# zhiyuns/REHRSeg

Hardware: AMD Instinct MI355X
Metric: 3D patches/sec (fwd+bwd, 128^3 fp32) (higher is better)
Workload: dtype f32; 1 GPU; FLAVR UNet_3D_3D(1,'unet_18',128,4) fwd+bwd+Adam, 1x1x128^3 patch per GPU, random-init weights; patches_per_gpu=1, global_batch=1, parallelism=dp1 (patch-parallel, flat-bucket RCCL all-reduce), wgrad_stream=True

## Files before the change

include/rehrseg_hip.h:

```cpp
#ifndef REHRSEG_HIP_H
#define REHRSEG_HIP_H

#include <stdint.h>

#ifdef __cplusplus
extern "C" {
#endif

#define REHR_OK 0
#define REHR_EINVAL -1
#define REHR_ENOSUP -2
#define REHR_EHIP -3

#define REHR_ACT_NONE 0
#define REHR_ACT_RELU 1
#define REHR_ACT_LRELU 2

typedef struct {
  int32_t count, off0, offs, k0, ks;
} rehr_axis_taps;

typedef struct {
  const float* x1;
  const float* x2;
  int32_t c1, ldx1, ldx2;
  int32_t N, Di, Hi, Wi, Cin;
  int32_t Ld, Lh, Lw;
  int32_t sd, sh, sw, bd, bh, bw;
  rehr_axis_taps td, th, tw;
  int32_t KH, KW;
  const float* wp;
  int32_t Npad;
  float* y;
  int32_t Dy, Hy, Wy, Cout, ldy;
  int32_t osd, osh, osw, obd, obh, obw;
  const float* bias;
  int32_t act;
  float slope;
  double* stats;
  int32_t stats_mode;
  int32_t tile_d, tile_h, tile_w;
  float* wino_ws;
  int64_t wino_ws_bytes;
  int32_t flags;
  int32_t debug_flags;
} rehr_gather_gemm_desc;

#define REHR_GG_Y_F32 1
#define REHR_GG_WS_READY 2
#define REHR_GG_WS_ONLY 4

#define REHR_DBG_GG_NO_HALO 1
#define REHR_DBG_GG_NO_FLAT8 2
#define REHR_DBG_GG_FLAT8_HALF 4
#define REHR_DBG_GG_FLAT8_FULL 8
#define REHR_DBG_GG_W32P_TWO_PER_CU 16
#define REHR_DBG_GG_W32P_ONE_PER_CU 32
#define REHR_DBG_GG_INTERLEAVE 64
#define REHR_DBG_GG_NO_TCONV_KS 128
#define REHR_DBG_GG_SLICE_MAJOR 256

int64_t rehr_gather_gemm_wino_bytes(const rehr_gather_gemm_desc* d);
#define REHR_GG_ROUTE_NONE 0
#define REHR_GG_ROUTE_FLAT8 1
#define REHR_GG_ROUTE_W32P 2
#define REHR_GG_ROUTE_BIG8 3
#define REHR_GG_ROUTE_SMALL 4
#define REHR_GG_ROUTE_FLAT22 5
#define REHR_GG_ROUTE_REGION22 6
int rehr_gather_gemm_wino_route(const rehr_gather_gemm_desc* d);
int rehr_gather_gemm_f32(const rehr_gather_gemm_desc* d, void* stream);
int rehr_gather_gemm_multi_f32(const rehr_gather_gemm_desc* descs, int32_t count,
                               void* stream);
int rehr_gather_gemm_bf16(const rehr_gather_gemm_desc* d, void* stream);
int rehr_gather_gemm_multi_bf16(const rehr_gather_gemm_desc* descs, int32_t count, void* stream);
int rehr_pack_weights_bf16(const float* in, void* out, int32_t A, int32_t Apad, int32_t B, int32_t T,
                           int32_t transpose_ab, void* stream);

int rehr_sum_slabs_bias_act_f32(const float* slabs, int32_t S, int64_t slab_stride,
                                const float* bias, float* y, int64_t rows, int32_t C,
                                int32_t act, float slope, void* stream);

int rehr_sum_slabs_stats_f32(const float* slabs, int32_t S, int64_t slab_stride, const float* bias,
                             float* y, int32_t N, int64_t SV, int32_t C, int32_t act, float slope,
                             double* stats, void* stream);

int rehr_sum_slabs_bias_act_bf16(const float* slabs, int32_t S, int64_t slab_stride, const float* bias, void* y,
                                 int64_t rows, int32_t C, int32_t act, float slope, void* stream);
int rehr_sum_slabs_stats_bf16(const float* slabs, int32_t S, int64_t slab_stride, const float* bias, void* y,
                              int32_t N, int64_t SV, int32_t C, int32_t act, float slope, double* stats,
                              void* stream);

typedef struct {
  const float* l;
  int32_t ldl, Ca;
  const float* g;
  int32_t ldg, Cg;
  int32_t N, Ld, Lh, Lw;
  int32_t Dg, Hg, Wg;
  int32_t sd, sh, sw, bd, bh, bw;
  rehr_axis_taps td, th, tw;
  int32_t KH, KW;
  float* dst;
  int64_t dst_sa, dst_sc, dst_st;
  int32_t accumulate;
  float* workspace;
  int64_t workspace_bytes;
  float* dbias;
  int32_t flags;
  int32_t debug_flags;
} rehr_wgrad_desc;

#define REHR_DBG_WGRAD_DIRECT 1
#define REHR_DBG_WGRAD_NO_TAP_SKIP 2
#define REHR_DBG_WGRAD_NO_TAP_COLOCATE 4

int64_t rehr_wgrad_bf16_workspace_bytes(const rehr_wgrad_desc* d);
int rehr_wgrad_bf16(const rehr_wgrad_desc* d, void* stream);
int64_t rehr_wgrad_workspace_bytes(const rehr_wgrad_desc* d);
int rehr_wgrad_uses_winograd(const rehr_wgrad_desc* d);
int rehr_wgrad_f32(const rehr_wgrad_desc* d, void* stream);

int rehr_pack_weights_f32(const float* in, float* out, int32_t A, int32_t Apad,
                          int32_t B, int32_t T, int32_t transpose_ab,
                          void* stream);

typedef struct {
  const float* x;
  int32_t ldx, N, Di, Hi, Wi, Cin;
  const float* w;
  const float* bias;
  float* y;
  int32_t ldy, Do, Ho, Wo, Cout;
  int32_t KD, KH, KW, sd, sh, sw, pd, ph, pw;
  int32_t act;
  float slope;
  double* stats;
  int32_t stats_mode;
} rehr_direct_conv_desc;

int rehr_conv_small_cin_fwd_f32(const rehr_direct_conv_desc* d, void* stream);
int rehr_im2col_f32(const rehr_direct_conv_desc* d, float* out, int32_t Kpad,
                    void* stream);
int64_t rehr_conv_small_cin_wgrad_workspace_bytes(const rehr_direct_conv_desc* d);
int rehr_conv_small_cin_wgrad_on_mfma(const rehr_direct_conv_desc* d);
int rehr_conv_small_cin_fwd_on_mfma(const rehr_direct_conv_desc* d);
int rehr_conv_small_cin_fwd_ybf16(const rehr_direct_conv_desc* d, void* stream);
int rehr_conv_small_cin_wgrad_dybf16(const rehr_direct_conv_desc* d, float* dw, float* dbias, float* workspace,
                                     int64_t workspace_bytes, void* stream);
int rehr_conv_small_cin_wgrad_f32(const rehr_direct_conv_desc* d, float* dw,
                                  float* dbias, float* workspace,
                                  int64_t workspace_bytes, void* stream);

int rehr_conv_small_cout_fwd_f32(const rehr_direct_conv_desc* d, void* stream);
int rehr_conv_small_cout_dgrad_f32(const rehr_direct_conv_desc* d, float* dx,
                                   void* stream);
int64_t rehr_conv_small_cout_wgrad_workspace_bytes(const rehr_direct_conv_desc* d);
int rehr_conv_small_cout_wgrad_f32(const rehr_direct_conv_desc* d, float* dw,
                                   float* dbias, float* workspace,
                                   int64_t workspace_bytes, void* stream);

int rehr_se_gate_fwd_f32(const double* stats, const float* w, const float* b,
                         float* gate, float* mean, int32_t N, int32_t C,
                         int64_t S, void* stream);
int rehr_scale_res_act_fwd_f32(const float* x, int32_t ldx, const float* gate,
                               const float* res, int32_t ldr, float* y,
                               int32_t ldy, int32_t N, int64_t S, int32_t C,
                               int32_t act, float slope, void* stream);
int rehr_scale_res_act_bwd_f32(const float* dy, int32_t lddy, const float* y,
                               int32_t ldy, const float* x, int32_t ldx,
                               const float* gate, float* dx, int32_t lddx,
                               float* dres, int32_t lddr, double* dgate_acc,
                               int32_t N, int64_t S, int32_t C, int32_t act,
                               float slope, void* stream);
int rehr_se_gate_bwd_f32(const double* dgate_acc, const float* gate,
                         const float* mean, const float* w, float* dw,
                         float* db, float* kconst, int32_t N, int32_t C,
                         int64_t S, void* stream);
int rehr_add_channel_const_f32(float* x, int32_t ldx, const float* k, int32_t N,
                               int64_t S, int32_t C, void* stream);

int rehr_instnorm_act_fwd_f32(const float* x, int32_t ldx, const double* stats,
                              const float* gamma, const float* beta, float* y,
                              int32_t ldy, float* mean_rstd ,
                              int32_t N, int64_t S, int32_t C, float eps,
                              int32_t act, float slope, void* stream);
int rehr_instnorm_act_bwd_f32(const float* dy, int32_t lddy, const float* x,
                              int32_t ldx, const float* mean_rstd,
                              const float* gamma, const float* beta, float* dx,
                              int32_t lddx, float* dgamma, float* dbeta,
                              double* red, int32_t N, int64_t S, int32_t C,
                              int32_t act, float slope, void* stream);

int rehr_upsample_depth_fwd_f32(const float* x, float* y, int32_t N, int32_t Di,
                                int32_t Do, int64_t HW, int32_t C, void* stream);
int rehr_upsample_depth_bwd_f32(const float* dy, float* dx, int32_t N,
                                int32_t Di, int32_t Do, int64_t HW, int32_t C,
                                void* stream);

int rehr_upmix_depth_fwd_f32(const float* g, const float* bias, float* y, int32_t N,
                             int32_t Di, int32_t Do, int64_t HW, int32_t C, int32_t KD,
                             int32_t pd, int32_t act, float slope, void* stream);
int rehr_upmix_depth_bwd_f32(const float* dy, const float* y, float* dg, int32_t N,
                             int32_t Di, int32_t Do, int64_t HW, int32_t C, int32_t KD,
                             int32_t pd, int32_t act, float slope, void* stream);
int rehr_channel_sum_actgrad_f32(const float* dy, const float* y, int32_t ld, int64_t rows,
                                 int32_t C, int32_t act, float slope, float* out,
                                 double* scratch, void* stream);

int rehr_cosdist_stats_f32(const float* x1, const float* x2, double* stats, int32_t N,
                           int64_t S, int32_t C, void* stream);
int rehr_cosdist_bwd_f32(const float* x1, const float* x2, const double* stats, float* dx1,
                         int32_t N, int64_t S, int32_t C, float scale, void* stream);

int32_t rehr_uasr_mix_blocks(int32_t N, int32_t D, int64_t HW);
int rehr_uasr_mix_fwd_f32(const float* om, const float* ue, const float* wu, const float* bu, float* out,
                          float* unc, int32_t N, int32_t K, int32_t D, int64_t HW, void* stream);
int rehr_uasr_mix_bwd_f32(const float* om, const float* ue, const float* wu, const float* bu,
                          const float* gout, const float* gunc, float* dom, float* due, double* partial,
                          int32_t N, int32_t K, int32_t D, int64_t HW, void* stream);

int rehr_quad_maxpool_fwd_f32(const float* x, float* y, int32_t* idx, int64_t slices,
                              int32_t H, int32_t W, int32_t C, void* stream);
int rehr_quad_maxpool_bwd_f32(const float* dy, const int32_t* idx, float* dx, int64_t slices,
// ... 166 lines not shown
```

rehrseg_amd/csrc/gather_gemm.hip:

```cpp
#include "common.h"
#include "halo_conv.h"
#include "wino_shared.h"

namespace {

constexpr int BK = 32;
constexpr int LDS_LD = 36;
constexpr int NTHREADS = 256;

template <int BM, int BN, int WGM, int WGN, int LDSBUF>
__device__ __forceinline__ void gather_gemm_body(const GGParams& p, const int nblocks, const int logical_in = -1) {
  constexpr int WTM = BM / WGM, WTN = BN / WGN;
  constexpr int FM = WTM / 32, FN = WTN / 32;
  constexpr int AROWS = BM / 32, BROWS = BN / 32;
  static_assert(WGM * WGN == 4, "4 waves");
  const rehr_gather_gemm_desc& d = p.d;

  extern __shared__ __attribute__((aligned(16))) float smem[];
  float* As = smem;
  float* Bs = smem + LDSBUF * BM * LDS_LD;
  int* row_out = (int*)(Bs + LDSBUF * BN * LDS_LD);

  const int tid = threadIdx.x;
  const int lane = tid & 63, wave = tid >> 6;
// ... 152 lines not shown
  };
  auto commit_loads = [&](int buf, const f32x4 (&ra)[AROWS], const f32x4 (&rb)[BROWS]) {
    float* a = As + buf * BM * LDS_LD;
    float* b = Bs + buf * BN * LDS_LD;
#pragma unroll
    for (int i = 0; i < AROWS; ++i)
      *reinterpret_cast<f32x4*>(a + (r0 + 32 * i) * LDS_LD + q * 4) = ra[i];
#pragma unroll
    for (int i = 0; i < BROWS; ++i)
      *reinterpret_cast<f32x4*>(b + (r0 + 32 * i) * LDS_LD + q * 4) = rb[i];
  };

  const int arow = wm * WTM + (lane & 31);
  const int brow = wn * WTN + (lane & 31);
  const int koff = 4 * (lane >> 5);
  auto compute = [&](int buf) {
    const float* a = As + buf * BM * LDS_LD;
    const float* b = Bs + buf * BN * LDS_LD;
#pragma unroll
    for (int kk = 0; kk < BK / 8; ++kk) {
      f32x4 fa[FM], fb[FN];
#pragma unroll
      for (int i = 0; i < FM; ++i)
        fa[i] = *reinterpret_cast<const f32x4*>(a + (arow + 32 * i) * LDS_LD + kk * 8 + koff);
#pragma unroll
      for (int j = 0; j < FN; ++j)
        fb[j] = *reinterpret_cast<const f32x4*>(b + (brow + 32 * j) * LDS_LD + kk * 8 + koff);
#pragma unroll
      for (int e = 0; e < 4; ++e)
#pragma unroll
        for (int i = 0; i < FM; ++i)
#pragma unroll
          for (int j = 0; j < FN; ++j)
            acc[i][j] = __builtin_amdgcn_mfma_f32_32x32x2f32(fa[i][e], fb[j][e], acc[i][j], 0, 0, 0);
      if (kk == 0) __builtin_amdgcn_sched_barrier(0);
    }
  };

  if (nsteps > 0) {
    issue_loads(ra0, rb0);
    issue_loads(ra1, rb1);
    commit_loads(0, ra0, rb0);
  }
  __syncthreads();

  if (LDSBUF == 2) {
    for (int s = 0; s < nsteps; s += 2) {
      issue_loads(ra0, rb0);
      compute(0);
      commit_loads(1, ra1, rb1);
      __syncthreads();
      if (s + 1 >= nsteps) break;
      issue_loads(ra1, rb1);
      compute(1);
      commit_loads(0, ra0, rb0);
      __syncthreads();
    }
  } else {
    for (int s = 0; s < nsteps; s += 2) {
      issue_loads(ra0, rb0);
      compute(0);
      __syncthreads();
      commit_loads(0, ra1, rb1);
      __syncthreads();
      if (s + 1 >= nsteps) break;
      issue_loads(ra1, rb1);
      compute(0);
      __syncthreads();
      commit_loads(0, ra0, rb0);
      __syncthreads();
    }
  }

  const int chalf = lane >> 5;
#pragma unroll
  for (int j = 0; j < FN; ++j) {
    const int col = n0 + wn * WTN + j * 32 + (lane & 31);
    const bool colok = col < d.Cout;
    const float bv = (d.bias != nullptr && colok) ? d.bias[col] : 0.f;
    float s1 = 0.f, s2 = 0.f;
#pragma unroll
    for (int i = 0; i < FM; ++i) {
#pragma unroll
      for (int r = 0; r < 16; ++r) {
        const int row = wm * WTM + i * 32 + (r & 3) + 8 * (r >> 2) + 4 * chalf;
        const int off = row_out[row];
        float v = apply_act(acc[i][j][r] + bv, d.act, d.slope);
        if (off >= 0 && colok) {
          d.y[(int64_t)off * d.ldy + col] = v;
          s1 += v;
          s2 += v * v;
        }
      }
    }
    if (d.stats_mode != 0) {
      s1 += __shfl_xor(s1, 32, 64);
      s2 += __shfl_xor(s2, 32, 64);
      if (chalf == 0 && colok) {
        double* st = d.stats + ((int64_t)n_img * d.Cout + col) * 2;
        atomicAdd(st, (double)s1);
        if (d.stats_mode == 2) atomicAdd(st + 1, (double)s2);
      }
    }
  }
}

template <int BM, int BN, int WGM, int WGN, int LDSBUF>
__global__ __launch_bounds__(NTHREADS, (LDSBUF == 1 ? 3 : 2)) void gather_gemm_multi_kernel(const GGMulti pm) {
  int phase, logical;
  if (pm.interleave) {
    if (!interleaved_block((int)blockIdx.x, pm.ph[0].m_tiles, pm.ph[0].n_tiles, pm.count, phase, logical)) return;
  } else {
    phase = blockIdx.z;
    const int nb = pm.ph[phase].m_tiles * pm.ph[phase].n_tiles;
    if ((int)blockIdx.x >= nb) return;
    logical = xcd_remap(blockIdx.x, nb);
  }
  phase = __builtin_amdgcn_readfirstlane(phase);
  logical = __builtin_amdgcn_readfirstlane(logical);
  gather_gemm_body<BM, BN, WGM, WGN, LDSBUF>(pm.ph[phase], 0, logical);
}
template <int BM, int BN, int WGM, int WGN, int LDSBUF>
__global__ __launch_bounds__(NTHREADS, (LDSBUF == 1 ? 3 : 2)) void gather_gemm_kernel(const GGParams p) {
  gather_gemm_body<BM, BN, WGM, WGN, LDSBUF>(p, (int)gridDim.x);
}

template <int BM, int BN, int WGM, int WGN, int LDSBUF>
int launch_gg(const GGMulti& pm, int count, hipStream_t stream) {
  constexpr size_t smem = (size_t)LDSBUF * (BM + BN) * LDS_LD * sizeof(float) + BM * sizeof(int);
  return gg_launch<gather_gemm_kernel<BM, BN, WGM, WGN, LDSBUF>, gather_gemm_multi_kernel<BM, BN, WGM, WGN, LDSBUF>,
                   NTHREADS, smem>(pm, count, stream);
}

int validate(const rehr_gather_gemm_desc& d) { return gg_validate(d, 4); }

int launch_generic(const GGMulti& pm, int count, hipStream_t st) {
  const int npad = pm.ph[0].d.Npad;
  if (npad % 128 == 0) return launch_gg<128, 128, 2, 2, 2>(pm, count, st);
  if (npad % 64 == 0) return launch_gg<128, 64, 2, 2, 1>(pm, count, st);
  return launch_gg<128, 32, 4, 1, 1>(pm, count, st);
}

}

WinoRoute wino_route(const rehr_gather_gemm_desc& d, WinoPlan& plan) {
  if (!(d.debug_flags & REHR_DBG_GG_NO_FLAT8) && wino_flat8_plan(d, plan)) return WINO_FLAT8;
  if (const WinoRoute r = wino_region_plan(d, plan)) return r;
  if (wino22_flat_plan(d, plan, 1)) return WINO_FLAT22;
  if (wino22_region_plan(d, plan)) return WINO_REGION22;
  plan.bytes = 0;
  return WINO_NONE;
}

static int wino_run(WinoRoute r, const rehr_gather_gemm_desc* ds, int count, const WinoPlan& plan, hipStream_t st) {
  for (int i = 0; i < count; ++i) {
    const int rc = r >= WINO_FLAT22 ? wino22_weights_launch(ds[i], plan, st) : wino_weights_launch(r, ds[i], plan, st);
    if (rc != REHR_OK) return rc;
  }
  if (ds[0].flags & REHR_GG_WS_ONLY) return REHR_OK;
  switch (r) {
    case WINO_FLAT8: return wino_flat8_launch(ds[0], plan, st);
    case WINO_W32P: case WINO_BIG8: case WINO_SMALL: return wino_region_launch(r, ds, count, plan, st);
    default: return wino22_launch(r, ds, count, plan, st);
  }
}

extern "C" int rehr_gather_gemm_multi_f32(const rehr_gather_gemm_desc* descs, int32_t count, void* stream) {
  if (descs == nullptr || count < 1 || count > MAX_PHASES) return REHR_EINVAL;
  for (int i = 0; i < count; ++i) {
    const int rc = validate(descs[i]);
    if (rc != REHR_OK) return rc;
    if (descs[i].Npad != descs[0].Npad || descs[i].N != descs[0].N || descs[i].wp != descs[0].wp ||
        descs[i].x1 != descs[0].x1)
      return REHR_EINVAL;
  }
  hipStream_t st = (hipStream_t)stream;
  const bool ws_only = (descs[0].flags & REHR_GG_WS_ONLY) != 0;
  for (int i = 1; i < count; ++i)
    if ((descs[i].flags ^ descs[0].flags) & (REHR_GG_WS_ONLY | REHR_GG_WS_READY)) return REHR_EINVAL;
  if (count > 1 && !ws_only) {
    const int trc = tconv_ks_try(descs, count, false, st);
    if (trc != REHR_ENOSUP) return trc;
  }
  WinoPlan plan{};
  if (count > 1 && descs[0].wino_ws != nullptr) {
    const int taps = descs[0].td.count;
    if ((taps > 3 || taps == 1) && wino_split_plan(descs, count, plan)) return wino_run(WINO_BIG8, descs, count, plan, st);
    if (taps <= 3 && wino22_flat_multi_plan(descs, count, plan)) return wino_run(WINO_FLAT22, descs, count, plan, st);
  }
  GGMulti pm;
  pm.interleave = 0;
  pm.count = 0;
  pm.no_interleave = (descs[0].debug_flags & REHR_DBG_GG_INTERLEAVE) ? 0 : 1;
  int n = 0;
  for (int i = 0; i < count; ++i) {
    if (descs[i].wino_ws != nullptr && !(count > 1 && descs[i].td.count > 3)) {
      const WinoRoute r = wino_route(descs[i], plan);
      if (r != WINO_NONE && wino_ws_ok(descs[i], plan.bytes)) {
        const int wrc = wino_run(r, &descs[i], 1, plan, st);
        if (wrc != REHR_OK) return wrc;
        continue;
      }
    }
    if (ws_only) continue;
    if (descs[i].tile_d >= 0) {
      const int hrc = halo_conv_try(descs[i], st);
      if (hrc == REHR_OK) continue;
      if (hrc != REHR_ENOSUP) return hrc;
    }
    const int rc = gg_plan(descs[i], pm.ph[n], 4, BK);
    if (rc != REHR_OK) return rc;
    ++n;
  }
  if (n == 0) return REHR_OK;
  return launch_generic(pm, n, st);
}

extern "C" int64_t rehr_gather_gemm_wino_bytes(const rehr_gather_gemm_desc* dp) {
  WinoPlan plan{};
  if (dp == nullptr || validate(*dp) != REHR_OK || wino_route(*dp, plan) == WINO_NONE) return 0;
  return plan.bytes;
}

extern "C" int rehr_gather_gemm_wino_route(const rehr_gather_gemm_desc* dp) {
  WinoPlan plan{};
  if (dp == nullptr || validate(*dp) != REHR_OK) return REHR_GG_ROUTE_NONE;
  const WinoRoute r = wino_route(*dp, plan);
  return r == WINO_NONE ? REHR_GG_ROUTE_NONE : (int)r | (plan.variant << 8);
}

extern "C" int rehr_gather_gemm_f32(const rehr_gather_gemm_desc* dp, void* stream) {
  if (dp == nullptr) return REHR_EINVAL;
  return rehr_gather_gemm_multi_f32(dp, 1, stream);
}
```

rehrseg_amd/csrc/gg_shared.h:

```cpp
#pragma once
#include "common.h"
#include "taps.h"

struct GGParams {
  rehr_gather_gemm_desc d;
  int tiles_d, tiles_h, tiles_w, m_tiles, n_tiles;
  int kchunks;
  int64_t wp_bytes;
};

constexpr int MAX_PHASES = 8;
struct GGMulti {
  GGParams ph[MAX_PHASES];
  int interleave, count, no_interleave;
};

__device__ __forceinline__ bool interleaved_block(int b, int m_tiles, int n_tiles, int count, int& phase, int& logical) {
  const int xcd = b & 7, j = b >> 3, per = count * n_tiles;
  const int mt = (j / per) * 8 + xcd, rem = j % per;
  phase = rem / n_tiles;
  logical = mt * n_tiles + (rem - phase * n_tiles);
  return mt < m_tiles;
}

constexpr int64_t GG_BUF_LIMIT = BUF_LIMIT;

inline int64_t gg_wp_bytes(const rehr_gather_gemm_desc& d, int es) {
  const int64_t kd_max = d.td.k0 + (int64_t)d.td.ks * (d.td.count - 1);
  const int64_t kh_max = d.th.k0 + (int64_t)d.th.ks * (d.th.count - 1);
  const int64_t kw_max = d.tw.k0 + (int64_t)d.tw.ks * (d.tw.count - 1);
  return (((kd_max * d.KH) + kh_max) * d.KW + kw_max + 1) * d.Npad * d.Cin * es;
}

inline bool gg_src_fits(const rehr_gather_gemm_desc& d, int64_t vox, int es) {
  const int64_t b = vox * es;
  return b * d.ldx1 < GG_BUF_LIMIT && (!d.x2 || b * d.ldx2 < GG_BUF_LIMIT);
}

inline int gg_validate(const rehr_gather_gemm_desc& d, int es) {
  const int row = 16 / es;
  if (!d.x1 || !d.wp || !d.y) return REHR_EINVAL;
  if (d.N < 1 || d.Cin < 16 || d.Cin % 16 || d.c1 < 1 || d.c1 > d.Cin) return REHR_EINVAL;
  if (d.c1 < d.Cin && (d.c1 % 32 || !d.x2)) return REHR_EINVAL;
  if (d.ldx1 % row || (d.x2 && d.ldx2 % row)) return REHR_EINVAL;
  if (((uintptr_t)d.x1 | (uintptr_t)d.wp | (uintptr_t)(d.x2 ? d.x2 : d.x1)) & 15) return REHR_EINVAL;
  if (d.Npad % 32 || d.Npad < d.Cout || d.Cout < 1) return REHR_EINVAL;
  if (d.Ld < 1 || d.Lh < 1 || d.Lw < 1) return REHR_EINVAL;
  if (d.td.count < 1 || d.th.count < 1 || d.tw.count < 1) return REHR_EINVAL;
  if (d.tile_d != 0 && (d.tile_d < 1 || d.tile_h < 1 || d.tile_w < 1 || d.tile_d * d.tile_h * d.tile_w != 128))
    return REHR_EINVAL;
  if (d.stats_mode != 0 && !d.stats) return REHR_EINVAL;
  if (d.N > 65535) return REHR_EINVAL;
  const int64_t yd = (int64_t)(d.Ld - 1) * d.osd + d.obd, yh = (int64_t)(d.Lh - 1) * d.osh + d.obh,
                yw = (int64_t)(d.Lw - 1) * d.osw + d.obw;
  if (d.obd < 0 || d.obh < 0 || d.obw < 0 || yd >= d.Dy || yh >= d.Hy || yw >= d.Wy) return REHR_EINVAL;
  if (d.ldy < d.Cout) return REHR_EINVAL;
  if ((int64_t)d.N * d.Dy * d.Hy * d.Wy >= (1ll << 31)) return REHR_EINVAL;
  return REHR_OK;
}

inline int gg_plan(const rehr_gather_gemm_desc& d, GGParams& p, int es, int bk) {
  p.d = d;
  if (d.tile_d == 0) {
    p.tiles_d = p.tiles_h = 1;
    p.tiles_w = (int)(((int64_t)d.Ld * d.Lh * d.Lw + 127) / 128);
    p.m_tiles = p.tiles_w;
  } else {
    p.tiles_d = (d.Ld + d.tile_d - 1) / d.tile_d;
    p.tiles_h = (d.Lh + d.tile_h - 1) / d.tile_h;
    p.tiles_w = (d.Lw + d.tile_w - 1) / d.tile_w;
    p.m_tiles = p.tiles_d * p.tiles_h * p.tiles_w;
  }
  p.kchunks = (d.Cin + bk - 1) / bk;
  p.wp_bytes = gg_wp_bytes(d, es);
  if (p.wp_bytes >= GG_BUF_LIMIT || !gg_src_fits(d, (int64_t)d.Di * d.Hi * d.Wi, es)) return REHR_ENOSUP;
  p.n_tiles = d.Npad / (d.Npad % 128 == 0 ? 128 : (d.Npad % 64 == 0 ? 64 : 32));
  return REHR_OK;
}

template <void (*KERN1)(GGParams), void (*KERNM)(GGMulti), int NT, size_t SMEM>
int gg_launch(const GGMulti& pm, int count, hipStream_t stream) {
  static bool attr_set = false;
  if (!attr_set) {
    if (hipFuncSetAttribute(reinterpret_cast<const void*>(KERN1), hipFuncAttributeMaxDynamicSharedMemorySize,
                            (int)SMEM) != hipSuccess ||
        hipFuncSetAttribute(reinterpret_cast<const void*>(KERNM), hipFuncAttributeMaxDynamicSharedMemorySize,
                            (int)SMEM) != hipSuccess)
      return REHR_EHIP;
    attr_set = true;
  }
  if (count == 1) {
    const GGParams& p = pm.ph[0];
    hipLaunchKernelGGL(KERN1, dim3(p.m_tiles * p.n_tiles, p.d.N, 1), dim3(NT), SMEM, stream, p);
  } else {
    int nb = 0;
    bool uniform = true;
    for (int i = 0; i < count; ++i) {
      const int n = pm.ph[i].m_tiles * pm.ph[i].n_tiles;
      nb = n > nb ? n : nb;
      uniform = uniform && pm.ph[i].m_tiles == pm.ph[0].m_tiles && pm.ph[i].n_tiles == pm.ph[0].n_tiles;
    }
    GGMulti pmi = pm;
    pmi.count = count;
    const int64_t gx = (int64_t)((pm.ph[0].m_tiles + 7) / 8) * 8 * count * pm.ph[0].n_tiles;
    pmi.interleave = (uniform && !pm.no_interleave && gx < (1ll << 31)) ? 1 : 0;
    if (pmi.interleave) hipLaunchKernelGGL(KERNM, dim3((unsigned)gx, pm.ph[0].d.N, 1), dim3(NT), SMEM, stream, pmi);
    else hipLaunchKernelGGL(KERNM, dim3(nb, pm.ph[0].d.N, count), dim3(NT), SMEM, stream, pmi);
  }
  REHR_LAUNCH_CHECK();
  return REHR_OK;
}

int tconv_ks_try(const rehr_gather_gemm_desc* ds, int count, bool bf16, hipStream_t stream);
```

rehrseg_amd/csrc/tconv_ks.hip:

```cpp
#include "common.h"

namespace {

constexpr int TK_BM = 128, TK_BK = 32, TK_LD = 36, TK_THREADS = 256, TK_MAXPH = 8;

struct TconvKsParams {
  const void* x;
  const void* wp;
  const float* bias;
  void* y;
  int ldx, ldy, Cin, Cout, Npad;
  int N, Di, Hi, Wi, Do, Ho, Wo;
  int sd, sh, sw;
  int nph;
  int tap[TK_MAXPH];
  int yoff[TK_MAXPH];
  int64_t vox_total;
  int lda;
};

template <int NT>
__global__ __launch_bounds__(TK_THREADS, 2) void tconv_ks_f32_kernel(const TconvKsParams p) {
  extern __shared__ __attribute__((aligned(16))) float smem[];
  float* As = smem;
// ... 132 lines not shown
      const int row = r0 + 64 * i;
      const int64_t v = v0 + row;
      tk_bf16x8 a;
#pragma unroll
      for (int e = 0; e < 8; ++e) a[e] = (__bf16)0.f;
      if (v < p.vox_total) a = *reinterpret_cast<const tk_bf16x8*>(x + v * p.ldx + c * TK_BK + q * 8);
      *reinterpret_cast<tk_bf16x8*>(As + row * p.lda + c * TK_BK + q * 8) = a;
    }

  constexpr int NBR = (NT * 32 + 63) / 64;
  tk_bf16x8 rb[NBR];
  auto fetch_b = [&](int ph, int c) {
    const __bf16* w = wp + ((int64_t)p.tap[ph] * p.Npad) * p.Cin + c * TK_BK + q * 8;
#pragma unroll
    for (int j = 0; j < NBR; ++j) {
      const int row = r0 + 64 * j;
      if (row < NT * 32) rb[j] = *reinterpret_cast<const tk_bf16x8*>(w + (int64_t)row * p.Cin);
    }
  };
  auto commit_b = [&](int buf) {
    __bf16* b = Bs + buf * NT * 32 * TK_LDH;
#pragma unroll
    for (int j = 0; j < NBR; ++j) {
      const int row = r0 + 64 * j;
      if (row < NT * 32) *reinterpret_cast<tk_bf16x8*>(b + row * TK_LDH + q * 8) = rb[j];
    }
  };

  const int arow = wave * 32 + (lane & 31), koff = 8 * (lane >> 5), chalf = lane >> 5;
  const int steps = p.nph * kchunks;
  fetch_b(0, 0);
  commit_b(0);
  __syncthreads();

  f32x16 acc[NT];
  int ph = 0, c = 0;
  for (int s = 0; s < steps; ++s) {
    if (c == 0) {
#pragma unroll
      for (int j = 0; j < NT; ++j)
#pragma unroll
        for (int r = 0; r < 16; ++r) acc[j][r] = 0.f;
    }
    int nph_ = ph, nc = c + 1;
    if (nc == kchunks) { nc = 0; ++nph_; }
    const bool more = s + 1 < steps;
    if (more) fetch_b(nph_, nc);
    const __bf16* a = As + arow * p.lda + c * TK_BK + koff;
    const __bf16* b = Bs + (s & 1) * NT * 32 * TK_LDH + (lane & 31) * TK_LDH + koff;
#pragma unroll
    for (int kk = 0; kk < TK_BK / 16; ++kk) {
      const tk_bf16x8 fa = *reinterpret_cast<const tk_bf16x8*>(a + kk * 16);
#pragma unroll
      for (int j = 0; j < NT; ++j) {
        const tk_bf16x8 fb = *reinterpret_cast<const tk_bf16x8*>(b + j * 32 * TK_LDH + kk * 16);
        acc[j] = __builtin_amdgcn_mfma_f32_32x32x16_bf16(fa, fb, acc[j], 0, 0, 0);
      }
    }
    if (more) commit_b((s + 1) & 1);
    if (c == kchunks - 1) {
      const int yo = p.yoff[ph];
#pragma unroll
      for (int j = 0; j < NT; ++j) {
        const int col = j * 32 + (lane & 31);
        const bool colok = col < p.Cout;
        const float bv = (p.bias != nullptr && colok) ? p.bias[col] : 0.f;
#pragma unroll
        for (int r = 0; r < 16; ++r) {
          const int row = wave * 32 + (r & 3) + 8 * (r >> 2) + 4 * chalf;
          const int off = row_out[row];
          if (off >= 0 && colok) y[(int64_t)(off + yo) * p.ldy + col] = (__bf16)(acc[j][r] + bv);
        }
      }
    }
    __syncthreads();
    ph = nph_;
    c = nc;
  }
}


bool tconv_ks_match(const rehr_gather_gemm_desc* ds, int count, bool bf16, TconvKsParams& p) {
  if (count < 2 || count > TK_MAXPH) return false;
  const rehr_gather_gemm_desc& d0 = ds[0];
  if (d0.x2 != nullptr || d0.c1 != d0.Cin || d0.Cin % TK_BK || d0.Cin > 128 || d0.Npad % 32 || d0.Npad > 128) return false;
  if (d0.act != REHR_ACT_NONE || d0.stats_mode != 0 || (d0.flags & REHR_GG_Y_F32)) return false;
  if (d0.osd * d0.osh * d0.osw != count) return false;
  if (d0.Dy != d0.Di * d0.osd || d0.Hy != d0.Hi * d0.osh || d0.Wy != d0.Wi * d0.osw) return false;
  if ((int64_t)d0.N * d0.Dy * d0.Hy * d0.Wy >= (1ll << 31)) return false;
  if (d0.KH != d0.osh || d0.KW != d0.osw) return false;
  unsigned seen = 0;
  for (int i = 0; i < count; ++i) {
    const rehr_gather_gemm_desc& d = ds[i];
    if (d.x1 != d0.x1 || d.wp != d0.wp || d.y != d0.y || d.bias != d0.bias || d.x2 != nullptr || d.Cin != d0.Cin ||
        d.ldx1 != d0.ldx1 || d.ldy != d0.ldy || d.Cout != d0.Cout || d.Npad != d0.Npad || d.N != d0.N)
      return false;
    if (d.td.count != 1 || d.th.count != 1 || d.tw.count != 1 || d.td.off0 || d.th.off0 || d.tw.off0) return false;
    if (d.sd != 1 || d.sh != 1 || d.sw != 1 || d.bd || d.bh || d.bw) return false;
    if (d.Ld != d0.Di || d.Lh != d0.Hi || d.Lw != d0.Wi || d.Di != d0.Di || d.Hi != d0.Hi || d.Wi != d0.Wi) return false;
    if (d.osd != d0.osd || d.osh != d0.osh || d.osw != d0.osw || d.Dy != d0.Dy || d.Hy != d0.Hy || d.Wy != d0.Wy) return false;
    if (d.obd != d.td.k0 || d.obh != d.th.k0 || d.obw != d.tw.k0) return false;
    if (d.obd < 0 || d.obd >= d.osd || d.obh < 0 || d.obh >= d.osh || d.obw < 0 || d.obw >= d.osw) return false;
    if (d.act != REHR_ACT_NONE || d.stats_mode != 0 || d.flags != d0.flags) return false;
    const int id = (d.obd * d.osh + d.obh) * d.osw + d.obw;
    if (seen & (1u << id)) return false;
    seen |= 1u << id;
    p.tap[i] = (d.td.k0 * d.KH + d.th.k0) * d.KW + d.tw.k0;
    p.yoff[i] = (d.obd * d.Hy + d.obh) * d.Wy + d.obw;
  }
  const int align = bf16 ? 15 : 15;
  if (((uintptr_t)d0.x1 | (uintptr_t)d0.wp) & align) return false;
  if (bf16 ? (d0.ldx1 % 8 || d0.ldy % 2) : (d0.ldx1 % 4)) return false;
  p.x = d0.x1; p.wp = d0.wp; p.bias = d0.bias; p.y = d0.y;
  p.ldx = d0.ldx1; p.ldy = d0.ldy; p.Cin = d0.Cin; p.Cout = d0.Cout; p.Npad = d0.Npad;
  p.N = d0.N; p.Di = d0.Di; p.Hi = d0.Hi; p.Wi = d0.Wi; p.Do = d0.Dy; p.Ho = d0.Hy; p.Wo = d0.Wy;
  p.sd = d0.osd; p.sh = d0.osh; p.sw = d0.osw;
  p.nph = count;
  p.vox_total = (int64_t)d0.N * d0.Di * d0.Hi * d0.Wi;
  p.lda = bf16 ? d0.Cin + 8 : d0.Cin + 4;
  return true;
}

template <int NT>
int tconv_launch(const TconvKsParams& p, bool bf16, hipStream_t stream) {
  const int64_t blocks = (p.vox_total + TK_BM - 1) / TK_BM;
  if (blocks >= (1ll << 31)) return REHR_ENOSUP;
  if (!bf16 && p.Cin > 64) return REHR_ENOSUP;
  if (bf16) {
    const size_t smem = ((size_t)TK_BM * p.lda + 2 * NT * 32 * TK_LDH) * 2 + TK_BM * sizeof(int);
    static bool attr = false;
    if (!attr) {
      if (hipFuncSetAttribute((const void*)tconv_ks_bf16_kernel<NT>, hipFuncAttributeMaxDynamicSharedMemorySize, 72 * 1024) !=
          hipSuccess)
        return REHR_EHIP;
      attr = true;
    }
    hipLaunchKernelGGL(tconv_ks_bf16_kernel<NT>, dim3((unsigned)blocks), dim3(TK_THREADS), smem, stream, p);
  } else {
    const size_t smem = ((size_t)TK_BM * p.lda + 2 * NT * 32 * TK_LD) * sizeof(float) + TK_BM * sizeof(int);
    static bool attr = false;
    if (!attr) {
      if (hipFuncSetAttribute((const void*)tconv_ks_f32_kernel<NT>, hipFuncAttributeMaxDynamicSharedMemorySize, 112 * 1024) !=
          hipSuccess)
        return REHR_EHIP;
      attr = true;
    }
    hipLaunchKernelGGL(tconv_ks_f32_kernel<NT>, dim3((unsigned)blocks), dim3(TK_THREADS), smem, stream, p);
  }
  return REHR_OK;
}

}

int tconv_ks_try(const rehr_gather_gemm_desc* ds, int count, bool bf16, hipStream_t stream) {
  if (ds[0].debug_flags & REHR_DBG_GG_NO_TCONV_KS) return REHR_ENOSUP;
  TconvKsParams p;
  if (!tconv_ks_match(ds, count, bf16, p)) return REHR_ENOSUP;
  int rc;
  switch (p.Npad / 32) {
    case 1: rc = tconv_launch<1>(p, bf16, stream); break;
    case 2: rc = tconv_launch<2>(p, bf16, stream); break;
    case 3: rc = tconv_launch<3>(p, bf16, stream); break;
    default: rc = tconv_launch<4>(p, bf16, stream); break;
  }
  if (rc != REHR_OK) return rc;
  REHR_LAUNCH_CHECK();
  return REHR_OK;
}
```

rehrseg_amd/csrc/wino22_conv.hip:

```cpp
#include "common.h"
#include "wino_shared.h"
#include <cstdlib>

namespace {

constexpr int LD = WINO_LDX;
constexpr int PW = 17;
constexpr int RP = PW * LD + 12;
constexpr int BUF = PW * RP;
constexpr int PVOX = PW * PW;
constexpr int NT_ = 768;
constexpr int NX = (PVOX * 8 + NT_ - 1) / NT_;
constexpr int MAXPH = WINO_MAXPH;

struct W22Params {
  rehr_gather_gemm_desc d;
  int nb_h, nb_w, kchunks, nphase;
  Phase phase[MAXPH];
  const float* up;
  uint32_t up_bytes;
};

__global__ void w22_weights_kernel(const rehr_gather_gemm_desc d, float* __restrict__ up, int kchunks) {
  AxisPlan ah, aw;
  plan_axis(d.th, d.sh, d.bh, ah);
  plan_axis(d.tw, d.sw, d.bw, aw);
  const int nphase = ah.nph * aw.nph;
  const int cpad = kchunks * 32;
  const int64_t per = (int64_t)d.Npad * cpad;
  const int64_t per_src = (int64_t)d.Npad * d.Cin;
  const int64_t total = (int64_t)nphase * d.td.count * per;
  const int NT = d.Npad / 32;
  for (int64_t i = (int64_t)blockIdx.x * blockDim.x + threadIdx.x; i < total; i += (int64_t)gridDim.x * blockDim.x) {
    const int pj = (int)(i / per);
    const int p = pj / d.td.count, jd = pj - p * d.td.count;
    const int p_h = p / aw.nph, p_w = p - p_h * aw.nph;
    const int64_t rem = i - (int64_t)pj * per;
    const int n = (int)(rem / cpad), ci = (int)(rem - (int64_t)n * cpad);
    float g[2][2];
#pragma unroll
    for (int a = 0; a < 2; ++a)
#pragma unroll
      for (int b = 0; b < 2; ++b) {
        const int wt = ((d.td.k0 + d.td.ks * jd) * d.KH + ah.kidx[p_h][a]) * d.KW + aw.kidx[p_w][b];
        g[a][b] = ci < d.Cin ? d.wp[(int64_t)wt * per_src + (int64_t)n * d.Cin + ci] : 0.f;
      }
    float u[9];
    u[0] = g[0][0];              u[1] = g[0][0] + g[0][1];                     u[2] = g[0][1];
    u[3] = g[0][0] + g[1][0];    u[4] = g[0][0] + g[0][1] + g[1][0] + g[1][1]; u[5] = g[0][1] + g[1][1];
    u[6] = g[1][0];              u[7] = g[1][0] + g[1][1];                     u[8] = g[1][1];
    const int nt = n >> 5, col = n & 31, chunk = ci >> 5, kk = (ci >> 3) & 3, half = (ci >> 2) & 1, e = ci & 3;
#pragma unroll
    for (int x = 0; x < 9; ++x) {
      const int64_t o = (((((int64_t)pj * 9 + x) * NT + nt) * kchunks + chunk) * 4 + kk) * 256 + (half * 32 + col) * 4 + e;
      up[o] = u[x];
    }
  }
}

__global__ __launch_bounds__(NT_) void wino22_conv_kernel(const W22Params p) {
  const rehr_gather_gemm_desc& d = p.d;
  extern __shared__ __attribute__((aligned(16))) float smem[];
  float* Xs = smem;

  const int tid = threadIdx.x, lane = tid & 63;
  const int wv = __builtin_amdgcn_readfirstlane(tid >> 6);
  const int r = wv % 3, fm = (wv / 3) & 1, fn = wv / 6;
  const int half = lane >> 5, col = lane & 31;
  const int n_img = blockIdx.z;
  const int nt0 = blockIdx.y * 2 + fn, n0 = blockIdx.y * 64;
  int b = xcd_remap(blockIdx.x, gridDim.x);
  const int bw_ = b % p.nb_w; b /= p.nb_w;
  const int bh_ = b % p.nb_h;
  const int od = b / p.nb_h;
  const int oh0 = bh_ * 16, ow0 = bw_ * 16;

  const int ia = r;
  const int th_ = fm * 4 + (col >> 3), tw_ = col & 7;
  const float* xa = Xs + (2 * th_ + ia) * RP + tw_ * LD + 4 * half;
  const float* xb = Xs + (2 * th_ + 1) * RP + tw_ * LD + 4 * half;

  int prow[NX], pcol[NX];
#pragma unroll
  for (int i = 0; i < NX; ++i) {
    const int piece = tid + NT_ * i;
    const int v = piece >> 3;
    const int ph = (v * 3856) >> 16;
    const int slot = v - ph * PW;
    prow[i] = ph;
    pcol[i] = slot < 9 ? 2 * slot : 2 * (slot - 9) + 1;
  }
  const int pq = tid & 7;
  const uint32_t img_elems = (uint32_t)d.Di * d.Hi * d.Wi;
  int jd_lo = d.td.count, jd_hi = -1;
  for (int j = 0; j < d.td.count; ++j) {
    const int id = od + d.bd + d.td.off0 + d.td.offs * j;
    if ((unsigned)id < (unsigned)d.Di) { jd_lo = min(jd_lo, j); jd_hi = max(jd_hi, j); }
  }
  const int items = p.nphase * p.kchunks * max(0, jd_hi - jd_lo + 1);
  f32x4 rx[NX];
  struct Item { int ph, chunk, jd; };
  auto advance = [&](Item& t) {
    if (++t.jd > jd_hi) {
      t.jd = jd_lo;
      if (++t.chunk == p.kchunks) { t.chunk = 0; ++t.ph; }
    }
  };
  auto fetch = [&](const Item& t) {
    const bool live = t.ph < p.nphase;
    const int ph_i = live ? t.ph : 0;
    const int jd = t.jd;
    const int cc = t.chunk * 32;
    const Phase& P = p.phase[ph_i];
    const int id = od + d.bd + d.td.off0 + d.td.offs * jd;
    const bool first = cc < d.c1;
    const float* src = first ? d.x1 : d.x2;
    const uint32_t ld = (uint32_t)(first ? d.ldx1 : d.ldx2);
    const int coff = first ? cc : cc - d.c1;
    const uint32_t nrec = img_elems * ld * 4u;
    const __amdgpu_buffer_rsrc_t rs = __builtin_amdgcn_make_buffer_rsrc(
        const_cast<float*>(src) + (int64_t)n_img * img_elems * ld, 0, nrec, 0x00020000);
    const bool dok = live & ((unsigned)id < (unsigned)d.Di) & ((cc + pq * 4) < d.Cin);
    const uint32_t base = (uint32_t)(id * d.Hi * d.Wi) * ld * 4u + (uint32_t)(coff + pq * 4) * 4u;
#pragma unroll
    for (int i = 0; i < NX; ++i) {
      const int piece = tid + NT_ * i;
      const int ih = (oh0 + P.dh0 + prow[i]) * P.sh + P.ph, iw = (ow0 + P.dw0 + pcol[i]) * P.sw + P.pw;
      const bool ok = dok & (piece < PVOX * 8) & ((unsigned)ih < (unsigned)d.Hi) & ((unsigned)iw < (unsigned)d.Wi);
      const uint32_t off = base + (uint32_t)(ih * d.Wi + iw) * ld * 4u;
      rx[i] = __builtin_bit_cast(f32x4, __builtin_amdgcn_raw_buffer_load_b128(rs, ok ? off : nrec, 0, 0));
    }
  };
  auto stage = [&](int buf) {
#pragma unroll
    for (int i = 0; i < NX; ++i) {
      const int piece = tid + NT_ * i;
      const int v = piece >> 3;
      if (piece < PVOX * 8) *reinterpret_cast<f32x4*>(Xs + buf + v * LD + prow[i] * 12 + pq * 4) = rx[i];
    }
  };

  const __amdgpu_buffer_rsrc_t rsu =
      __builtin_amdgcn_make_buffer_rsrc(const_cast<float*>(p.up), 0, p.up_bytes, 0x00020000);
  const int NT = d.Npad / 32;
  const uint32_t xi_stride = (uint32_t)NT * p.kchunks * 4096u, nt_stride = (uint32_t)p.kchunks * 4096u;
  const uint32_t ulane = (uint32_t)(r * 3) * xi_stride + (uint32_t)nt0 * nt_stride + (uint32_t)lane * 16u;
  auto load_u = [&](const Item& t, int kk, f32x4 (&ub)[3]) {
    const int ph_i = t.ph < p.nphase ? t.ph : 0;
#ifdef W22_DBG_SAMEW
    const uint32_t base = ulane + 0u * (uint32_t)(ph_i + kk);
#else
    const uint32_t base = (uint32_t)((ph_i * d.td.count + t.jd) * 9) * xi_stride + (uint32_t)(t.chunk * 4 + kk) * 1024u + ulane;
#endif
#pragma unroll
    for (int c = 0; c < 3; ++c)
      ub[c] = __builtin_bit_cast(f32x4, __builtin_amdgcn_raw_buffer_load_b128(rsu, base + c * xi_stride, 0, 0));
  };

  f32x16 acc[3];
#pragma unroll
  for (int c = 0; c < 3; ++c)
#pragma unroll
    for (int q = 0; q < 16; ++q) acc[c][q] = 0.f;

  auto read_a = [&](int buf, const int kk, f32x4 (&v)[3]) {
    f32x4 R[3];
#ifdef W22_DBG_NOLDS
    R[0] = R[1] = R[2] = f32x4{1.f, 2.f, 3.f, 4.f};
#else
#pragma unroll
    for (int j = 0; j < 3; ++j) R[j] = *reinterpret_cast<const f32x4*>(xa + buf + ((j & 1) * 9 + (j >> 1)) * LD + kk * 8);
    if (r != 1) {
#pragma unroll
      for (int j = 0; j < 3; ++j) R[j] -= *reinterpret_cast<const f32x4*>(xb + buf + ((j & 1) * 9 + (j >> 1)) * LD + kk * 8);
    }
#endif
    v[0] = R[0] - R[1];
    v[1] = R[1];
    v[2] = R[2] - R[1];
  };
  auto mma = [&](const f32x4 (&v)[3], const f32x4 (&ub)[3]) {
#pragma unroll
    for (int e = 0; e < 4; ++e)
#pragma unroll
      for (int c = 0; c < 3; ++c) acc[c] = __builtin_amdgcn_mfma_f32_32x32x2f32(v[c][e], ub[c][e], acc[c], 0, 0, 0);
  };

#ifdef W22_STAMPS
  const long long st0 = __builtin_readcyclecounter();
#endif
  f32x4 u0[3], u1[3], va[3], vb[3];
  Item cur_i = {0, 0, min(jd_lo, d.td.count - 1)}, nxt_i = cur_i, fet_i;
  fetch(cur_i);
  load_u(cur_i, 0, u0);
  stage(0);
  advance(nxt_i);
  fetch(nxt_i);
  fet_i = nxt_i;
  __syncthreads();
  read_a(0, 0, va);
#ifdef W22_STAMPS
  const long long st1 = __builtin_readcyclecounter();
  long long st_stage = 0, st_bar = 0;
#endif
  for (int it = 0; it < items; ++it) {
    const int cur = (it & 1) * BUF, nxt = cur ^ BUF;
    load_u(cur_i, 1, u1);
    read_a(cur, 1, vb);
    __builtin_amdgcn_s_setprio(2);
// ... 284 lines not shown
  Item cur_i = {0, 0, min(jd_lo, d.td.count - 1)}, nxt_i = cur_i;
  fetch(cur_i);
  load_u(cur_i, 0, u0);
  stage(0);
  __syncthreads();
  for (int it = 0; it < items; ++it) {
    const int cur = (it & 1) * FBUF, nxt = cur ^ FBUF;
    advance(nxt_i);
    fetch(nxt_i);
    load_u(cur_i, 1, u1);
    kstep(cur, 0, u0);
    load_u(cur_i, 2, u0);
    kstep(cur, 1, u1);
    load_u(cur_i, 3, u1);
    kstep(cur, 2, u0);
    load_u(nxt_i, 0, u0);
    kstep(cur, 3, u1);
    stage(nxt);
    cur_i = nxt_i;
    __syncthreads();
  }

  float* ex = smem;
  {
    const f32x16 T0v = acc[0] + acc[1];
    const f32x16 T1v = acc[1] + acc[2];
    float* e0 = ex + (((fm * 2 + fn) * 3 + r) * 2) * 16 * 64 + lane;
#pragma unroll
    for (int q = 0; q < 16; ++q) {
      e0[q * 64] = T0v[q];
      e0[(16 + q) * 64] = T1v[q];
    }
  }
  __syncthreads();
  const float neg_slope = d.act == REHR_ACT_NONE ? 1.f : (d.act == REHR_ACT_RELU ? 0.f : d.slope);
  const int col_n = n0 + fn * 32 + col;
  const bool colok = col_n < d.Cout;
  const float bv = (d.bias != nullptr && colok) ? d.bias[col_n] : 0.f;
  float ssum[F22_MAXSLOT][2];
#pragma unroll
  for (int s = 0; s < F22_MAXSLOT; ++s) ssum[s][0] = ssum[s][1] = 0.f;
  for (int pos = r; pos < 4; pos += 3) {
    const int ro = pos >> 1, co = pos & 1;
    const float k0 = ro == 0 ? 1.f : 0.f, k2 = ro == 0 ? 0.f : 1.f;
    const float* e0 = ex + ((fm * 2 + fn) * 3 * 2 + co) * 16 * 64 + lane;
    float t[3][16];
#pragma unroll
    for (int rr = 0; rr < 3; ++rr)
#pragma unroll
      for (int q = 0; q < 16; ++q) t[rr][q] = e0[(rr * 32 + q) * 64];
#pragma unroll
    for (int q = 0; q < 16; ++q) {
      const float yv = k0 * t[0][q] + t[1][q] + k2 * t[2][q] + bv;
      const float v = fmaxf(yv, 0.f) + neg_slope * fminf(yv, 0.f);
      const int m = fm * 32 + 8 * (q >> 2) + 4 * half + (q & 3);
      const int tv = tab[m], hwp = tab[2 * TB + m], sl = tab[TB + m];
      const int oh = 2 * (hwp >> 16) + ro, ow = 2 * (hwp & 0xffff) + co;
      const bool ok = colok & (tv >= 0) & (oh < d.Lh) & (ow < d.Lw);
      if (ok) d.y[((int64_t)tv + (int64_t)ro * d.osh * d.Wy + co * d.osw) * d.ldy + col_n] = v;
      if (d.stats_mode != 0) {
        const float vs = ok ? v : 0.f;
#pragma unroll
        for (int s = 0; s < F22_MAXSLOT; ++s) {
          ssum[s][0] += (s == sl) ? vs : 0.f;
          ssum[s][1] += (s == sl) ? vs * vs : 0.f;
        }
      }
    }
  }
  if (d.stats_mode != 0) {
    __syncthreads();
    float* red = smem;
    const int nslot = min(sl_ - s0 + 1, F22_MAXSLOT);
#pragma unroll
    for (int s = 0; s < F22_MAXSLOT; ++s)
      if (s < nslot) {
        float* rp = red + (((s * 12 + wv) * 2 + half) * 2) * 32 + col;
        rp[0] = ssum[s][0];
        rp[32] = ssum[s][1];
      }
    __syncthreads();
    for (int task = tid; task < nslot * 64; task += NT_) {
      const int s = task >> 6, fq = (task >> 5) & 1, c = task & 31;
      const int cn = n0 + fq * 32 + c;
      const int slice = s0 + s, od = slice / d.N, n = slice - od * d.N;
      if (cn < d.Cout && od < d.Ld) {
        float a1 = 0.f, a2 = 0.f;
        for (int w6 = 0; w6 < 6; ++w6)
          for (int h = 0; h < 2; ++h) {
            const float* rp = red + (((s * 12 + fq * 6 + w6) * 2 + h) * 2) * 32 + c;
            a1 += rp[0];
            a2 += rp[32];
          }
        double* st = d.stats + ((int64_t)n * d.Cout + cn) * 2;
        atomicAdd(st, (double)a1);
        if (d.stats_mode == 2) atomicAdd(st + 1, (double)a2);
      }
    }
  }
}

constexpr FlatConsts F22_CONSTS = {1, 64, F22_NX * NT_, 256, (int64_t)4 * 3 * 2 * 16 * 64,
                                   (int64_t)F22_MAXSLOT * 12 * 2 * 2 * 32, 160 * 1024};

bool plan22_taps(const rehr_gather_gemm_desc& d, WinoPlan& plan) {
  if (d.sd != 1) return false;
  AxisPlan ah, aw;
  if (!plan_axis(d.th, d.sh, d.bh, ah) || !plan_axis(d.tw, d.sw, d.bw, aw)) return false;
  if (ah.nph != aw.nph) return false;
  if (ah.nph == 2 && (d.osh != 1 || d.osw != 1 || d.obh || d.obw)) return false;
  if (d.td.count < 1 || d.td.count > 3 || d.Npad % 64) return false;
  plan.variant = 0;
  plan.kchunks = (d.Cin + 31) / 32;
  plan.nphase = fill_phases(ah, aw, plan.phase);
  plan.bytes = wino_scratch_bytes(d, 9 * plan.nphase);
  return plan.bytes != 0;
}

}

bool wino22_flat_plan(const rehr_gather_gemm_desc& d, WinoPlan& plan, int parts) {
  if (d.debug_flags & REHR_DBG_GG_NO_FLAT8) return false;
  if (!plan22_taps(d, plan) || d.Lh > 2048 || d.Ld > 127) return false;
  return plan_flat_geom(d, F22_CONSTS, parts, plan.flat);
}

bool wino22_region_plan(const rehr_gather_gemm_desc& d, WinoPlan& plan) {
  if (!plan22_taps(d, plan) || d.Lh < 12 || d.Lw < 12) return false;
  plan.nb_h = (d.Lh + 15) / 16;
  plan.nb_w = (d.Lw + 15) / 16;
  const int64_t padded = (int64_t)plan.nb_h * 16 * plan.nb_w * 16, exact = (int64_t)d.Lh * d.Lw;
  if (padded * 10 > exact * 13) {
    if (padded * 100 > exact * 178 || (int64_t)plan.nb_h * plan.nb_w * d.Ld * d.N * (d.Npad / 64) < 256) return false;
  }
  if (!gg_src_fits(d, (int64_t)d.Di * d.Hi * d.Wi, 4)) return false;
  return (int64_t)plan.nb_h * plan.nb_w * d.Ld < (1ll << 31) && d.Npad / 64 <= 65535 && d.N <= 65535;
}

bool wino22_flat_multi_plan(const rehr_gather_gemm_desc* ds, int count, WinoPlan& plan) {
  if (count < 2 || count > WINO_MAXPH) return false;
  if (!wino22_flat_plan(ds[0], plan, count) || plan.nphase != 1) return false;
  for (int i = 0; i < count; ++i) {
    WinoPlan q;
    if (!wino22_flat_plan(ds[i], q, count) || q.nphase != 1 || q.bytes != plan.bytes || !wino_ws_ok(ds[i], q.bytes))
      return false;
    if (!gg_same_layer(ds[i], ds[0], SAME_DEPTH_TAPS | SAME_DEST) || q.phase[0].sh != plan.phase[0].sh ||
        q.phase[0].sw != plan.phase[0].sw)
      return false;
    plan.phase[i] = q.phase[0];
  }
  return true;
}

int wino22_weights_launch(const rehr_gather_gemm_desc& d, const WinoPlan& plan, hipStream_t stream) {
  const int64_t total = (int64_t)plan.nphase * d.td.count * d.Npad * plan.kchunks * 32;
  return wino_transform_launch<w22_weights_kernel>(d, total, 8192, stream, plan.kchunks);
}

int wino22_launch(WinoRoute r, const rehr_gather_gemm_desc* ds, int count, const WinoPlan& plan, hipStream_t stream) {
  const rehr_gather_gemm_desc& d = ds[0];
  if (r == WINO_FLAT22) {
    F22Params p;
    p.d = d;
    flat_fill(p, plan.flat);
    p.kchunks = plan.kchunks;
    p.nphase = plan.nphase;
    for (int i = 0; i < WINO_MAXPH; ++i) p.phase[i] = plan.phase[i];
    p.up_bytes = (uint32_t)plan.bytes;
    p.parts = count;
    p.up = count == 1 ? d.wino_ws : nullptr;
    for (int i = 0; i < count; ++i) {
      p.s_up[i] = ds[i].wino_ws;
      p.s_obh[i] = ds[i].obh;
      p.s_obw[i] = ds[i].obw;
    }
    const size_t smem = flat_lds_bytes(plan.flat, 64);
    const int rc = grow_dyn_lds<wino22_flat_conv_kernel>(smem);
    if (rc != REHR_OK) return rc;
    dim3 grid((unsigned)((p.ntiles + 63) / 64), d.Npad / 64, count);
    hipLaunchKernelGGL(wino22_flat_conv_kernel, grid, dim3(NT_), smem, stream, p);
  } else {
    W22Params p;
    p.d = d;
    p.nb_h = plan.nb_h;
    p.nb_w = plan.nb_w;
    p.kchunks = plan.kchunks;
    p.nphase = plan.nphase;
    for (int i = 0; i < WINO_MAXPH; ++i) p.phase[i] = plan.phase[i];
    p.up = d.wino_ws;
    p.up_bytes = (uint32_t)plan.bytes;
    constexpr size_t smem_x = (size_t)2 * BUF * sizeof(float), smem_e = (size_t)4 * 3 * 2 * 16 * 64 * sizeof(float);
    constexpr size_t smem = smem_x > smem_e ? smem_x : smem_e;
    const int rc = set_dyn_lds_once<wino22_conv_kernel>((int)smem);
    if (rc != REHR_OK) return rc;
    dim3 grid((unsigned)((int64_t)p.nb_h * p.nb_w * d.Ld), d.Npad / 64, d.N);
    hipLaunchKernelGGL(wino22_conv_kernel, grid, dim3(NT_), smem, stream, p);
  }
  REHR_LAUNCH_CHECK();
  return REHR_OK;
}
```

rehrseg_amd/csrc/wino_conv.hip:

```cpp
#include "common.h"
#include "wino_shared.h"
#include <cstdlib>

namespace {

constexpr int TH = 4, TW = 8;
constexpr int PH = 2 * TH + 2, PW = 2 * TW + 2;
constexpr int PVOX = PH * PW;
constexpr int LDX = 36;
constexpr int NX = (PVOX * 8 + 255) / 256;

struct WinoParams {
  rehr_gather_gemm_desc d;
  int nb_h, nb_w;
  int band_major;
  int kchunks;
  int dh0, dw0;
  const float* up;
  uint32_t up_bytes;
  int nsplit;
  rehr_axis_taps s_td[8];
  const float* s_up[8];
  uint32_t s_up_bytes[8];
  float* s_y[8];
// ... 119 lines not shown
    }
  };
  auto load_u = [&](int it, int kk, f32x4 (&ub)[4]) {
    const int jd = it % d.td.count;
    const int cc = (it / d.td.count) * 32;
    const uint32_t base = (uint32_t)(jd * 16 + r * 4) * per_b + (uint32_t)(cc + kk * 8) * 4u + ulane;
#pragma unroll
    for (int c = 0; c < 4; ++c)
      ub[c] = __builtin_bit_cast(f32x4, __builtin_amdgcn_raw_buffer_load_b128(rsu, base + c * per_b, 0, 0));
  };
  auto compute = [&](const f32x4 (&R)[4], const f32x4 (&ub)[4]) {
    f32x4 v[4];
    v[0] = R[0] - R[2];
    v[1] = R[1] + R[2];
    v[2] = R[1] - R[2];
    v[3] = R[1] - R[3];
#pragma unroll
    for (int e = 0; e < 4; ++e)
#pragma unroll
      for (int c = 0; c < 4; ++c)
        acc[c] = __builtin_amdgcn_mfma_f32_32x32x2f32(v[c][e], ub[c][e], acc[c], 0, 0, 0);
  };

  fetch(0);
  stage(0);
  fetch(1);
  f32x4 Ra[4], Rb[4], ua[4], ubb[4];
  load_u(0, 0, ua);
  __syncthreads();

  for (int it = 0; it < items; ++it) {
    const int cur = (it & 1) * (PVOX * LDX);
    read_r(cur, 0, Ra);
    read_r(cur, 1, Rb);
    load_u(it, 1, ubb);
    stage(cur ^ (PVOX * LDX));
    __builtin_amdgcn_sched_barrier(0);
    compute(Ra, ua);
    __builtin_amdgcn_sched_barrier(0);
    read_r(cur, 2, Ra);
    load_u(it, 2, ua);
    fetch(it + 2);
    __builtin_amdgcn_sched_barrier(0);
    compute(Rb, ubb);
    __builtin_amdgcn_sched_barrier(0);
    read_r(cur, 3, Rb);
    load_u(it, 3, ubb);
    __builtin_amdgcn_sched_barrier(0);
    compute(Ra, ua);
    __builtin_amdgcn_sched_barrier(0);
    load_u(it + 1 < items ? it + 1 : it, 0, ua);
    __builtin_amdgcn_sched_barrier(0);
    compute(Rb, ubb);
    __builtin_amdgcn_sched_barrier(0);
    __syncthreads();
  }

  f32x16 T0 = (acc[0] + acc[1] - acc[2]) * rsign;
  f32x16 T1 = (acc[1] + acc[2] - acc[3]) * rsign;
  float* ex = smem;
#pragma unroll
  for (int q = 0; q < 16; ++q) {
    ex[((r * 2 + 0) * 16 + q) * 64 + lane] = T0[q];
    ex[((r * 2 + 1) * 16 + q) * 64 + lane] = T1[q];
  }
  __syncthreads();
  const int ro = r >> 1, co = r & 1;
  const float k0 = ro == 0 ? 1.f : 0.f, k2 = ro == 0 ? 1.f : -1.f, k3 = ro == 0 ? 0.f : -1.f;
  const float neg_slope = d.act == REHR_ACT_NONE ? 1.f : (d.act == REHR_ACT_RELU ? 0.f : d.slope);
  const int col_n = n0 + col;
  const bool colok = col_n < d.Cout;
  const float bv = (d.bias != nullptr && colok) ? d.bias[col_n] : 0.f;
  float s1_ = 0.f, s2_ = 0.f;
  float t[4][16];
#pragma unroll
  for (int rr = 0; rr < 4; ++rr)
#pragma unroll
    for (int q = 0; q < 16; ++q) t[rr][q] = ex[((rr * 2 + co) * 16 + q) * 64 + lane];
#pragma unroll
  for (int q = 0; q < 16; ++q) {
    const float yv = k0 * t[0][q] + t[1][q] + k2 * t[2][q] + k3 * t[3][q] + bv;
    const float v = fmaxf(yv, 0.f) + neg_slope * fminf(yv, 0.f);
    const int tile = (q & 3) + 8 * (q >> 2) + 4 * half;
    const int oh = oh0 + 2 * (tile / TW) + ro, ow = ow0 + 2 * (tile % TW) + co;
    const bool ok = colok & (oh < d.Lh) & (ow < d.Lw);
    if (ok) d.y[((((int64_t)n_img * d.Dy + od) * d.Hy + oh) * d.Wy + ow) * d.ldy + col_n] = v;
    s1_ += ok ? v : 0.f;
    s2_ += ok ? v * v : 0.f;
  }
  if (d.stats_mode != 0) {
    s1_ += __shfl_xor(s1_, 32, 64);
    s2_ += __shfl_xor(s2_, 32, 64);
    __syncthreads();
    float* red = smem;
    if (half == 0) {
      red[(r * 2 + 0) * 32 + col] = s1_;
      red[(r * 2 + 1) * 32 + col] = s2_;
    }
    __syncthreads();
    if (r == 0 && half == 0 && colok) {
      const float a1 = red[col] + red[64 + col] + red[128 + col] + red[192 + col];
      const float a2 = red[32 + col] + red[96 + col] + red[160 + col] + red[224 + col];
      double* st = d.stats + ((int64_t)n_img * d.Cout + col_n) * 2;
      atomicAdd(st, (double)a1);
      if (d.stats_mode == 2) atomicAdd(st + 1, (double)a2);
    }
  }
}

constexpr int PW2 = 18, PVOX2 = 18 * 18;
constexpr int RP2 = PW2 * LDX + 8;
constexpr int BUF2 = PW2 * RP2;

__global__ void wino_weights_frag_kernel(const rehr_gather_gemm_desc d, float* __restrict__ up, int kchunks) {
  const float G[4][3] = {{1.f, 0.f, 0.f}, {.5f, .5f, .5f}, {.5f, -.5f, .5f}, {0.f, 0.f, 1.f}};
  const int cpad = kchunks * 32;
  const int64_t per = (int64_t)d.Npad * cpad;
  const int64_t per_src = (int64_t)d.Npad * d.Cin;
  const int64_t total = (int64_t)d.td.count * per;
  const int NT = d.Npad / 32;
  for (int64_t i = (int64_t)blockIdx.x * blockDim.x + threadIdx.x; i < total; i += (int64_t)gridDim.x * blockDim.x) {
    const int jd = (int)(i / per);
    const int64_t rem = i - (int64_t)jd * per;
    const int n = (int)(rem / cpad), ci = (int)(rem - (int64_t)n * cpad);
    float g[3][3];
#pragma unroll
    for (int jh = 0; jh < 3; ++jh)
#pragma unroll
      for (int jw = 0; jw < 3; ++jw) {
        const int a = d.bh + d.th.off0 + d.th.offs * jh + 1;
        const int b = d.bw + d.tw.off0 + d.tw.offs * jw + 1;
        const int wt = ((d.td.k0 + d.td.ks * jd) * d.KH + (d.th.k0 + d.th.ks * jh)) * d.KW + (d.tw.k0 + d.tw.ks * jw);
        const float v = ci < d.Cin ? d.wp[(int64_t)wt * per_src + (int64_t)n * d.Cin + ci] : 0.f;
#pragma unroll
        for (int aa = 0; aa < 3; ++aa)
#pragma unroll
          for (int bb = 0; bb < 3; ++bb)
            if (aa == a && bb == b) g[aa][bb] = v;
      }
    float t[4][3];
#pragma unroll
    for (int r = 0; r < 4; ++r)
#pragma unroll
      for (int b = 0; b < 3; ++b) t[r][b] = G[r][0] * g[0][b] + G[r][1] * g[1][b] + G[r][2] * g[2][b];
    const int nt = n >> 5, col = n & 31, chunk = ci >> 5, kk = (ci >> 3) & 3, half = (ci >> 2) & 1, e = ci & 3;
#pragma unroll
    for (int r = 0; r < 4; ++r)
#pragma unroll
      for (int c = 0; c < 4; ++c) {
        const int64_t o = (((((int64_t)jd * 16 + r * 4 + c) * NT + nt) * kchunks + chunk) * 4 + kk) * 256 +
                          (half * 32 + col) * 4 + e;
        up[o] = t[r][0] * G[c][0] + t[r][1] * G[c][1] + t[r][2] * G[c][2];
      }
  }
}

constexpr int NX8 = (PVOX2 * 8 + 511) / 512;

__global__ __launch_bounds__(512) void wino_conv_big8_kernel(const WinoParams p) {
  const rehr_gather_gemm_desc& d = p.d;
  extern __shared__ __attribute__((aligned(16))) float smem[];
  float* Xs = smem;
  constexpr int BUF = BUF2;

  const int tid = threadIdx.x, lane = tid & 63;
  const int wv = __builtin_amdgcn_readfirstlane(tid >> 6);
  const int r = wv & 3, fm = wv >> 2;
  const int half = lane >> 5, col = lane & 31;
  const int part = (p.nsplit > 1) ? (int)(blockIdx.z % p.nsplit) : 0;
  const int n_img = (p.nsplit > 1) ? (int)(blockIdx.z / p.nsplit) : (int)blockIdx.z;
  const rehr_axis_taps td = (p.nsplit > 1) ? p.s_td[part] : p.d.td;
  const float* const up = (p.nsplit > 1) ? p.s_up[part] : p.up;
  const uint32_t up_bytes = (p.nsplit > 1) ? p.s_up_bytes[part] : p.up_bytes;
  float* const yout = (p.nsplit > 1) ? p.s_y[part] : p.d.y;
  const int nt0 = blockIdx.y * 2, n0 = blockIdx.y * 64;
  int b = xcd_remap(blockIdx.x, gridDim.x);
  const int bw_ = b % p.nb_w; b /= p.nb_w;
  const int bh_ = p.band_major ? b / p.d.Ld : b % p.nb_h;
  const int od = p.band_major ? b % p.d.Ld : b / p.nb_h;
  const int oh0 = bh_ * 16, ow0 = bw_ * 16;

  const int i1 = (r == 0) ? 0 : 1, i2 = (r == 3) ? 3 : 2;
  const float s2 = (r == 1) ? 1.f : -1.f;
  const float rsign = (r == 2) ? -1.f : 1.f;
  const int th_ = fm * 4 + (col >> 3), tw_ = col & 7;
  const float* xa = Xs + (2 * th_ + i1) * RP2 + tw_ * LDX + 4 * half;
  const float* xb = Xs + (2 * th_ + i2) * RP2 + tw_ * LDX + 4 * half;

  int pvx[NX8];
  uint32_t pok = 0;
#pragma unroll
  for (int i = 0; i < NX8; ++i) {
    const int piece = tid + 512 * i;
    const int v = piece >> 3;
    const int ph = v / PW2, slot = v - ph * PW2;
    const int pw_ = slot < 9 ? 2 * slot : 2 * (slot - 9) + 1;
    const int ih = oh0 + p.dh0 + ph, iw = ow0 + p.dw0 + pw_;
    const bool ok = (piece < PVOX2 * 8) & ((unsigned)ih < (unsigned)d.Hi) & ((unsigned)iw < (unsigned)d.Wi);
    pvx[i] = ok ? ih * d.Wi + iw : 0;
    pok |= (ok ? 1u : 0u) << i;
  }
  const int pq = tid & 7;
  const uint32_t img_elems = (uint32_t)d.Di * d.Hi * d.Wi;
  constexpr int NXH = NX8 / 2;
  f32x4 rx[NXH];
  int jd_lo = td.count, jd_hi = -1;
  for (int j = 0; j < td.count; ++j) {
    const int id = od + d.bd + td.off0 + td.offs * j;
    if ((unsigned)id < (unsigned)d.Di) { jd_lo = min(jd_lo, j); jd_hi = max(jd_hi, j); }
  }
  const int items = p.kchunks * max(0, jd_hi - jd_lo + 1);
  struct Item { int chunk, jd; };
  auto advance = [&](Item& t) {
    if (++t.jd > jd_hi) { t.jd = jd_lo; ++t.chunk; }
  };
  auto fetch_to = [&](f32x4 (&rx)[NXH], const Item& t, const int lo) {
    const bool live = (t.chunk < p.kchunks) & (items > 0);
    const int jd = t.jd;
    const int cc = (live ? t.chunk : 0) * 32;
    const int id = od + d.bd + td.off0 + td.offs * jd;
    const bool first = cc < d.c1;
    const float* src = first ? d.x1 : d.x2;
    const uint32_t ld = (uint32_t)(first ? d.ldx1 : d.ldx2);
    const int coff = first ? cc : cc - d.c1;
    const uint32_t nrec = img_elems * ld * 4u;
    const __amdgpu_buffer_rsrc_t rs = __builtin_amdgcn_make_buffer_rsrc(
        const_cast<float*>(src) + (int64_t)n_img * img_elems * ld, 0, nrec, 0x00020000);
    const bool dok = live & ((unsigned)id < (unsigned)d.Di) & ((cc + pq * 4) < d.Cin);
    const uint32_t base = (uint32_t)(id * d.Hi * d.Wi) * ld * 4u + (uint32_t)(coff + pq * 4) * 4u;
#pragma unroll
    for (int i = 0; i < NXH; ++i) {
      const bool ok = dok & ((pok >> (lo + i)) & 1u);
      const uint32_t off = base + (uint32_t)pvx[lo + i] * ld * 4u;
      rx[i] = __builtin_bit_cast(f32x4, __builtin_amdgcn_raw_buffer_load_b128(rs, ok ? off : nrec, 0, 0));
    }
  };
  auto stage_from = [&](const f32x4 (&rx)[NXH], int buf, const int lo) {
#pragma unroll
    for (int i = 0; i < NXH; ++i) {
      const int piece = tid + 512 * (lo + i);
      const int v = piece >> 3, row = (v * 3641) >> 16;
      if (piece < PVOX2 * 8) *reinterpret_cast<f32x4*>(Xs + buf + v * LDX + row * 8 + pq * 4) = rx[i];
    }
  };
  auto fetch = [&](const Item& t, const int lo) { fetch_to(rx, t, lo); };
  auto stage = [&](int buf, const int lo) { stage_from(rx, buf, lo); };

  const __amdgpu_buffer_rsrc_t rsu =
      __builtin_amdgcn_make_buffer_rsrc(const_cast<float*>(up), 0, up_bytes, 0x00020000);
  const int NT = d.Npad / 32;
  const uint32_t xi_stride = (uint32_t)NT * p.kchunks * 4096u, nt_stride = (uint32_t)p.kchunks * 4096u;
  const uint32_t ulane = (uint32_t)lane * 16u;
  const uint32_t ubase = (uint32_t)(r * 4) * xi_stride + (uint32_t)nt0 * nt_stride;
  auto load_u = [&](const Item& t, const int kk, const int fn, f32x4 (&ub)[4]) {
    const int chunk = t.chunk < p.kchunks ? t.chunk : 0;
    const uint32_t base = ubase + (uint32_t)(t.jd * 16) * xi_stride + (uint32_t)(chunk * 4 + kk) * 1024u + fn * nt_stride;
#pragma unroll
    for (int c = 0; c < 4; ++c)
      ub[c] = __builtin_bit_cast(f32x4, __builtin_amdgcn_raw_buffer_load_b128(rsu, ulane, base + c * xi_stride, 0));
  };

  f32x16 acc[2][4];
#pragma unroll
  for (int fn = 0; fn < 2; ++fn)
#pragma unroll
    for (int c = 0; c < 4; ++c)
#pragma unroll
      for (int q = 0; q < 16; ++q) acc[fn][c][q] = 0.f;

  f32x4 ra[4], rb[4];
  auto issue_reads = [&](int buf, const int kk) {
#pragma unroll
    for (int j = 0; j < 4; ++j) {
      ra[j] = *reinterpret_cast<const f32x4*>(xa + buf + ((j & 1) * 9 + (j >> 1)) * LDX + kk * 8);
      rb[j] = *reinterpret_cast<const f32x4*>(xb + buf + ((j & 1) * 9 + (j >> 1)) * LDX + kk * 8);
    }
  };
  typedef float f32x2 __attribute__((ext_vector_type(2)));
  struct VFrag { f32x2 p[4][2]; };
  const f32x2 s2v = {s2, s2};
  auto combine = [&](VFrag& v) {
#pragma unroll
    for (int h = 0; h < 2; ++h) {
      f32x2 R[4];
#pragma unroll
      for (int j = 0; j < 4; ++j) {
        const f32x2 a = h ? ra[j].hi : ra[j].lo, bq = h ? rb[j].hi : rb[j].lo;
        R[j] = __builtin_elementwise_fma(bq, s2v, a);
      }
      v.p[0][h] = R[0] - R[2];
      v.p[1][h] = R[1] + R[2];
      v.p[2][h] = R[1] - R[2];
      v.p[3][h] = R[1] - R[3];
    }
  };
  auto mfmas = [&](const int fn, const VFrag& v, const f32x4 (&ub)[4]) {
#pragma unroll
    for (int e = 0; e < 4; ++e)
#pragma unroll
      for (int c = 0; c < 4; ++c)
        acc[fn][c] = __builtin_amdgcn_mfma_f32_32x32x2f32(v.p[c][e >> 1][e & 1], ub[c][e], acc[fn][c], 0, 0, 0);
  };

  VFrag VA, VB;
  f32x4 u0[4], u1[4];
  Item ci = {0, min(jd_lo, td.count - 1)}, ni = ci;
// ... 356 lines not shown
    W3P_FENCE();
    load_u(ni, 1, u1);
    ci = ni;
  }
#undef W3P_FENCE
  __syncthreads();

  float* ex = smem;
#pragma unroll
  for (int m = 0; m < 2; ++m) {
    const f32x16 T0 = (acc[m][0] + acc[m][1] - acc[m][2]) * rsign;
    const f32x16 T1 = (acc[m][1] + acc[m][2] - acc[m][3]) * rsign;
    float* e0 = ex + (((2 * g + m) * 4 + r) * 2) * 16 * 64 + lane;
#pragma unroll
    for (int q = 0; q < 16; ++q) {
      e0[q * 64] = T0[q];
      e0[(16 + q) * 64] = T1[q];
    }
  }
  __syncthreads();
  const int ro = r >> 1, co = r & 1;
  const float k0 = ro == 0 ? 1.f : 0.f, k2 = ro == 0 ? 1.f : -1.f, k3 = ro == 0 ? 0.f : -1.f;
  const float neg_slope = d.act == REHR_ACT_NONE ? 1.f : (d.act == REHR_ACT_RELU ? 0.f : d.slope);
  float* ybase = d.y + ((((int64_t)n_img * d.Dy + od) * d.Hy + (oh0 + ro)) * d.Wy + (ow0 + co + 8 * half)) * d.ldy +
                 n0 + col;
  const int64_t rowstep = 2 * (int64_t)d.Wy * d.ldy, colstep = 2 * (int64_t)d.ldy;
  const bool interior = (oh0 + 16 * G <= d.Lh) & (ow0 + 16 <= d.Lw) & (n0 + 32 <= d.Cout);
  const int col_n = n0 + col;
  const bool colok = col_n < d.Cout;
  const float bv = (d.bias != nullptr && colok) ? d.bias[col_n] : 0.f;
  double s1_ = 0.0, s2_ = 0.0;
#pragma unroll
  for (int m = 0; m < 2; ++m) {
    const int fm = 2 * g + m;
    const float* e0 = ex + (fm * 4 * 2 + co) * 16 * 64 + lane;
    float t[4][16];
#pragma unroll
    for (int rr = 0; rr < 4; ++rr)
#pragma unroll
      for (int q = 0; q < 16; ++q) t[rr][q] = e0[(rr * 32 + q) * 64];
    float v[16];
#pragma unroll
    for (int q = 0; q < 16; ++q) {
      const float yv = k0 * t[0][q] + t[1][q] + k2 * t[2][q] + k3 * t[3][q] + bv;
      v[q] = fmaxf(yv, 0.f) + neg_slope * fminf(yv, 0.f);
    }
    float* yb = ybase + (fm * 4) * rowstep;
    if (interior) {
#pragma unroll
      for (int q = 0; q < 16; ++q) {
        yb[(q >> 2) * rowstep + (q & 3) * colstep] = v[q];
        s1_ += (double)v[q];
        s2_ += (double)v[q] * (double)v[q];
      }
    } else {
#pragma unroll
      for (int q = 0; q < 16; ++q) {
        const int oh = oh0 + 2 * (fm * 4 + (q >> 2)) + ro, ow = ow0 + 2 * ((q & 3) + 4 * half) + co;
        const bool ok = colok & (oh < d.Lh) & (ow < d.Lw);
        if (ok) yb[(q >> 2) * rowstep + (q & 3) * colstep] = v[q];
        s1_ += ok ? (double)v[q] : 0.0;
        s2_ += ok ? (double)v[q] * (double)v[q] : 0.0;
      }
    }
  }
  if (d.stats_mode != 0) {
    s1_ += __shfl_xor(s1_, 32, 64);
    s2_ += __shfl_xor(s2_, 32, 64);
    __syncthreads();
    double* red = reinterpret_cast<double*>(smem);
    if (half == 0) {
      red[(wv * 2 + 0) * 32 + col] = s1_;
      red[(wv * 2 + 1) * 32 + col] = s2_;
    }
    __syncthreads();
    if (wv == 0 && half == 0 && colok) {
      double a1 = 0.0, a2 = 0.0;
#pragma unroll
      for (int w = 0; w < 4 * G; ++w) {
        a1 += red[(w * 2 + 0) * 32 + col];
        a2 += red[(w * 2 + 1) * 32 + col];
      }
      double* st = d.stats + ((int64_t)n_img * d.Cout + col_n) * 2;
      atomicAdd(st, a1);
      if (d.stats_mode == 2) atomicAdd(st + 1, a2);
    }
  }
}

bool regions16_ok(const rehr_gather_gemm_desc& d) {
  if (d.Lh < 16 || d.Lw < 16) return false;
  const int64_t nb_h = (d.Lh + 15) / 16, nb_w = (d.Lw + 15) / 16;
  return nb_h * 16 * nb_w * 16 * 10 <= (int64_t)d.Lh * d.Lw * 13;
}
int w32_groups(const rehr_gather_gemm_desc& d) {
  const int64_t nb_h = (d.Lh + 31) / 32, nb_w = (d.Lw + 15) / 16;
  if (d.Lh >= 32 && nb_h * 32 * nb_w * 16 * 10 <= (int64_t)d.Lh * d.Lw * 13) return 4;
  return 2;
}

template <int G>
int launch_w32p(const WinoParams& p, hipStream_t stream) {
  constexpr size_t smem_x = (size_t)2 * (W3<2 * G>::BUF + 32) * sizeof(float);
  constexpr size_t smem_e = (size_t)2 * G * 4 * 2 * 16 * 64 * sizeof(float);
  constexpr size_t smem = smem_x > smem_e ? smem_x : smem_e;
  const int rc = set_dyn_lds_once<wino_conv_w32p_kernel<G>>((int)smem);
  if (rc != REHR_OK) return rc;
  dim3 grid((unsigned)((int64_t)p.nb_h * p.nb_w * p.d.Ld), p.d.Npad / 32, p.d.N);
  hipLaunchKernelGGL(wino_conv_w32p_kernel<G>, grid, dim3(256 * G), smem, stream, p);
  return REHR_OK;
}

}

WinoRoute wino_region_plan(const rehr_gather_gemm_desc& d, WinoPlan& plan) {
  if (d.sd != 1 || d.sh != 1 || d.sw != 1) return WINO_NONE;
  if (d.osd != 1 || d.osh != 1 || d.osw != 1 || d.obd || d.obh || d.obw) return WINO_NONE;
  if (d.Ld != d.Dy || d.Lh != d.Hy || d.Lw != d.Wy) return WINO_NONE;
  if (!three_taps(d.th, d.bh) || !three_taps(d.tw, d.bw)) return WINO_NONE;
  if (d.td.count < 1 || d.td.count > 256) return WINO_NONE;
  if (d.Lh < 8 || d.Lw < 8) return WINO_NONE;
  const WinoRoute r = !regions16_ok(d) ? WINO_SMALL : d.Npad % 64 ? WINO_W32P : WINO_BIG8;
  const int64_t nb_h = (d.Lh + 2 * TH - 1) / (2 * TH), nb_w = (d.Lw + 2 * TW - 1) / (2 * TW);
  if (r == WINO_SMALL && nb_h * 2 * TH * nb_w * 2 * TW * 100 > (int64_t)d.Lh * d.Lw * 134) return WINO_NONE;
  plan.bytes = wino_scratch_bytes(d, 16);
  if (plan.bytes == 0) return WINO_NONE;
  if (!gg_src_fits(d, (int64_t)d.Di * d.Hi * d.Wi, 4)) return WINO_NONE;
  if (nb_h * nb_w * d.Ld >= (1ll << 31) || d.Npad / 32 > 65535 || d.N > 65535) return WINO_NONE;
  plan.kchunks = (d.Cin + 31) / 32;
  plan.variant = 0;
  plan.nb_h = r == WINO_SMALL ? (int)nb_h : (d.Lh + 15) / 16;
  plan.nb_w = r == WINO_SMALL ? (int)nb_w : (d.Lw + 15) / 16;
  if (r == WINO_W32P) {
    const bool two = (d.debug_flags & REHR_DBG_GG_W32P_TWO_PER_CU) ? true
                     : (d.debug_flags & REHR_DBG_GG_W32P_ONE_PER_CU) ? false : d.Cin * d.td.count <= 96;
    plan.variant = (w32_groups(d) == 4 && !two) ? 2 : 1;
    plan.nb_h = (d.Lh + 16 * plan.variant - 1) / (16 * plan.variant);
  }
  return r;
}

bool wino_split_plan(const rehr_gather_gemm_desc* ds, int count, WinoPlan& plan) {
  if (count < 2 || count > 8 || (int64_t)ds[0].N * count > 65535) return false;
  if (wino_region_plan(ds[0], plan) != WINO_BIG8) return false;
  for (int i = 0; i < count; ++i) {
    const rehr_gather_gemm_desc& d = ds[i];
    WinoPlan q{};
    if (wino_region_plan(d, q) == WINO_NONE || !wino_ws_ok(d, q.bytes)) return false;
    if (d.bias || d.stats_mode || d.act != REHR_ACT_NONE || !gg_same_layer(d, ds[0], SAME_HW_TAPS)) return false;
  }
  return true;
}

int wino_weights_launch(WinoRoute r, const rehr_gather_gemm_desc& d, const WinoPlan& plan, hipStream_t stream) {
  if (r == WINO_SMALL)
    return wino_transform_launch<wino_weights_kernel>(d, (int64_t)d.td.count * d.Npad * d.Cin, 4096, stream);
  return wino_transform_launch<wino_weights_frag_kernel>(d, (int64_t)d.td.count * d.Npad * plan.kchunks * 32, 8192, stream,
                                                         plan.kchunks);
}

int wino_region_launch(WinoRoute r, const rehr_gather_gemm_desc* ds, int count, const WinoPlan& plan, hipStream_t stream) {
  const rehr_gather_gemm_desc& d = ds[0];
  WinoParams p;
  p.d = d;
  p.kchunks = plan.kchunks;
  p.dh0 = -1;
  p.dw0 = -1;
  p.nb_h = plan.nb_h;
  p.nb_w = plan.nb_w;
  p.band_major = (d.debug_flags & REHR_DBG_GG_SLICE_MAJOR) ? 0 : 1;
  p.nsplit = count > 1 ? count : 0;
  p.up = count > 1 ? nullptr : d.wino_ws;
  p.up_bytes = count > 1 ? 0 : (uint32_t)plan.bytes;
  for (int i = 0; count > 1 && i < count; ++i) {
    p.s_td[i] = ds[i].td;
    p.s_up[i] = ds[i].wino_ws;
    p.s_up_bytes[i] = (uint32_t)wino_scratch_bytes(ds[i], 16);
    p.s_y[i] = ds[i].y;
  }
  if (r == WINO_W32P) {
    const int rc = plan.variant == 2 ? launch_w32p<2>(p, stream) : launch_w32p<1>(p, stream);
    if (rc != REHR_OK) return rc;
  } else if (r == WINO_BIG8) {
    constexpr size_t smem_x = (size_t)2 * BUF2 * sizeof(float), smem_e = (size_t)4 * 4 * 2 * 16 * 64 * sizeof(float);
    constexpr size_t smem = smem_x > smem_e ? smem_x : smem_e;
    const int rc = set_dyn_lds_once<wino_conv_big8_kernel>((int)smem);
    if (rc != REHR_OK) return rc;
    dim3 grid((unsigned)((int64_t)p.nb_h * p.nb_w * d.Ld), d.Npad / 64, d.N * count);
    hipLaunchKernelGGL(wino_conv_big8_kernel, grid, dim3(512), smem, stream, p);
  } else {
    constexpr size_t smem_x = (size_t)2 * PVOX * LDX * sizeof(float), smem_e = (size_t)4 * 2 * 16 * 64 * sizeof(float);
    constexpr size_t smem = smem_x > smem_e ? smem_x : smem_e;
    static_assert(smem <= 64 * 1024, "wino_conv_kernel: dynamic LDS beyond the default limit");
    dim3 grid((unsigned)((int64_t)p.nb_h * p.nb_w * d.Ld), d.Npad / 32, d.N);
    hipLaunchKernelGGL(wino_conv_kernel, grid, dim3(256), smem, stream, p);
  }
  REHR_LAUNCH_CHECK();
  return REHR_OK;
}
```

rehrseg_amd/csrc/wino_shared.h:

```cpp
#pragma once
#include "common.h"
#include "gg_shared.h"
#include "wino22_shared.h"

enum WinoRoute {
  WINO_NONE = REHR_GG_ROUTE_NONE,
  WINO_FLAT8 = REHR_GG_ROUTE_FLAT8,
  WINO_W32P = REHR_GG_ROUTE_W32P,
  WINO_BIG8 = REHR_GG_ROUTE_BIG8,
  WINO_SMALL = REHR_GG_ROUTE_SMALL,
  WINO_FLAT22 = REHR_GG_ROUTE_FLAT22,
  WINO_REGION22 = REHR_GG_ROUTE_REGION22,
};

constexpr int WINO_LDX = 36;
constexpr int WINO_MAXPH = 4;

struct Phase {
  int sh, sw;
  int ph, pw;
  int dh0, dw0;
};

struct FlatGeom {
  int nth, ntw, tps;
  int ntiles;
  int PH;
  int PWs, nev;
  int RP, rowpad;
  int rows;
  int rowmagic;
  int tab_off;
};
struct FlatConsts {
  int border;
  int tiles;
  int pieces;
  int fill_min;
  int64_t efl, rfl;
  int lds_cap;
};
constexpr int FLAT_MAXSLOT = 8;

struct WinoPlan {
  int64_t bytes;
  int variant;
  int kchunks;
  int nb_h, nb_w;
  FlatGeom flat;
  int nphase;
  Phase phase[WINO_MAXPH];
};

inline int64_t wino_scratch_bytes(const rehr_gather_gemm_desc& d, int xforms) {
  const int64_t need = (int64_t)xforms * d.td.count * d.Npad * ((d.Cin + 31) / 32) * 32 * (int64_t)sizeof(float);
  return need >= (1ll << 32) - 64 ? 0 : need;
}
inline bool wino_ws_ok(const rehr_gather_gemm_desc& d, int64_t need) {
  return d.wino_ws && d.wino_ws_bytes >= need && !((uintptr_t)d.wino_ws & 15);
}

inline int flat_conflicts(int ntw, int RP) {
  int worst = 0;
  for (int a = 0; a < ntw; ++a) {
    int cnt[16] = {0};
    for (int l = 0; l < 16; ++l) {
      const int t = a + l, th = t / ntw, tw = t - th * ntw;
      const int unit = ((tw * WINO_LDX + th * 2 * RP) / 4) & 15;
      if (++cnt[unit] > worst) worst = cnt[unit];
    }
  }
  return worst;
}

inline bool plan_flat_geom(const rehr_gather_gemm_desc& d, const FlatConsts& c, int parts, FlatGeom& g) {
  if (d.td.count < 1 || d.td.count > 3) return false;
  if (d.Npad % 64 || d.Lh < 6 || d.Lw < 6 || d.Lw > 64) return false;
  if (d.Lh % 16 == 0 && d.Lw % 16 == 0) return false;
  g.nth = (d.Lh + 1) / 2;
  g.ntw = (d.Lw + 1) / 2;
  g.tps = g.nth * g.ntw;
  if ((int64_t)g.nth * 2 * g.ntw * 2 * 10 > (int64_t)d.Lh * d.Lw * 13) return false;
  const int64_t ntiles = (int64_t)d.N * d.Ld * g.tps;
  if (ntiles >= (1ll << 30) || ntiles < c.tiles) return false;
  g.ntiles = (int)ntiles;
  if ((ntiles + 63) / 64 * (d.Npad / 64) * parts < c.fill_min) return false;
  if ((c.tiles - 2) / g.tps + 2 > FLAT_MAXSLOT) return false;
  g.PH = 2 * g.nth + c.border;
  g.nev = g.ntw + 1;
  g.PWs = 2 * g.ntw + c.border;
  const int trr = (c.tiles - 2) / g.ntw + 2, sdiff = (c.tiles - 2) / g.tps + 1;
  g.rows = 2 * (trr - 1) + c.border * (sdiff + 1) + 2;
  if ((int64_t)g.rows * g.PWs * 8 > c.pieces) return false;
  g.rowmagic = 65536 / g.PWs + 1;
  for (int v = 0; v <= g.rows * g.PWs; ++v)
    if (((v * g.rowmagic) >> 16) != v / g.PWs) return false;
  int best = 1 << 30;
  for (int pad = 4; pad <= 64; pad += 4) {
    const int cf = flat_conflicts(g.ntw, g.PWs * WINO_LDX + pad);
    if (cf < best) { best = cf; g.rowpad = pad; }
  }
  g.RP = g.PWs * WINO_LDX + g.rowpad;
  if (!gg_src_fits(d, (int64_t)d.N * d.Di * d.Hi * d.Wi, 4)) return false;
  if ((int64_t)d.N * d.Dy * d.Hy * d.Wy >= (1ll << 31) || d.Npad / 64 > 65535) return false;
  int64_t fl = (int64_t)2 * (g.rows * g.RP + WINO_LDX + 4);
  if (c.efl > fl) fl = c.efl;
  if (c.rfl > fl) fl = c.rfl;
  g.tab_off = (int)fl;
  return (fl + 3 * c.tiles) * 4 <= c.lds_cap;
}
template <typename P>
inline void flat_fill(P& p, const FlatGeom& g) {
  p.nth = g.nth; p.ntw = g.ntw; p.tps = g.tps; p.ntiles = g.ntiles;
  p.PH = g.PH; p.PWs = g.PWs; p.nev = g.nev; p.RP = g.RP; p.rowpad = g.rowpad;
  p.rows = g.rows; p.rowmagic = g.rowmagic; p.tab_off = g.tab_off;
}
inline size_t flat_lds_bytes(const FlatGeom& g, int tiles) { return (size_t)(g.tab_off + 3 * tiles) * sizeof(float); }

inline int fill_phases(const AxisPlan& ah, const AxisPlan& aw, Phase* phase) {
  for (int i = 0; i < ah.nph; ++i)
    for (int j = 0; j < aw.nph; ++j) {
      Phase& P = phase[i * aw.nph + j];
      P.sh = ah.stride; P.sw = aw.stride;
      P.ph = ah.par[i]; P.pw = aw.par[j];
      P.dh0 = ah.dmin[i]; P.dw0 = aw.dmin[j];
    }
  return ah.nph * aw.nph;
}

enum { SAME_HW_TAPS = 1, SAME_DEPTH_TAPS = 2, SAME_DEST = 4 };
inline bool gg_same_layer(const rehr_gather_gemm_desc& d, const rehr_gather_gemm_desc& d0, unsigned groups) {
  if (d.x2 != d0.x2 || d.Cin != d0.Cin || d.c1 != d0.c1 || d.ldx1 != d0.ldx1 || d.ldx2 != d0.ldx2 || d.Cout != d0.Cout ||
      d.ldy != d0.ldy || d.Ld != d0.Ld || d.Lh != d0.Lh || d.Lw != d0.Lw || d.Di != d0.Di || d.Hi != d0.Hi ||
      d.Wi != d0.Wi || d.bd != d0.bd)
    return false;
  auto same_axis = [](const rehr_axis_taps& a, const rehr_axis_taps& b) {
    return a.count == b.count && a.off0 == b.off0 && a.offs == b.offs && a.k0 == b.k0 && a.ks == b.ks;
  };
  if ((groups & SAME_HW_TAPS) && (d.bh != d0.bh || d.bw != d0.bw || d.KH != d0.KH || d.KW != d0.KW ||
                                  !same_axis(d.th, d0.th) || !same_axis(d.tw, d0.tw)))
    return false;
  if ((groups & SAME_DEPTH_TAPS) && (d.td.count != d0.td.count || d.td.off0 != d0.td.off0 || d.td.offs != d0.td.offs))
    return false;
  if ((groups & SAME_DEST) &&
      (d.y != d0.y || d.Dy != d0.Dy || d.Hy != d0.Hy || d.Wy != d0.Wy || d.osd != d0.osd || d.osh != d0.osh ||
       d.osw != d0.osw || d.obd != d0.obd || d.bias != d0.bias || d.act != d0.act || d.slope != d0.slope ||
       d.stats != d0.stats || d.stats_mode != d0.stats_mode))
    return false;
  return true;
}

template <auto KERN, typename... Args>
static int wino_transform_launch(const rehr_gather_gemm_desc& d, int64_t total, int cap, hipStream_t stream, Args... args) {
  if (d.flags & REHR_GG_WS_READY) return REHR_OK;
  int64_t blocks = (total + 255) / 256;
  if (blocks > cap) blocks = cap;
  hipLaunchKernelGGL(KERN, dim3((unsigned)blocks), dim3(256), 0, stream, d, d.wino_ws, args...);
  REHR_LAUNCH_CHECK();
  return REHR_OK;
}

WinoRoute wino_region_plan(const rehr_gather_gemm_desc& d, WinoPlan& plan);
bool wino_split_plan(const rehr_gather_gemm_desc* ds, int count, WinoPlan& plan);
int wino_weights_launch(WinoRoute r, const rehr_gather_gemm_desc& d, const WinoPlan& plan, hipStream_t stream);
int wino_region_launch(WinoRoute r, const rehr_gather_gemm_desc* ds, int count, const WinoPlan& plan, hipStream_t stream);
bool wino_flat8_plan(const rehr_gather_gemm_desc& d, WinoPlan& plan);
int wino_flat8_launch(const rehr_gather_gemm_desc& d, const WinoPlan& plan, hipStream_t stream);
bool wino22_flat_plan(const rehr_gather_gemm_desc& d, WinoPlan& plan, int parts);
bool wino22_region_plan(const rehr_gather_gemm_desc& d, WinoPlan& plan);
bool wino22_flat_multi_plan(const rehr_gather_gemm_desc* ds, int count, WinoPlan& plan);
int wino22_weights_launch(const rehr_gather_gemm_desc& d, const WinoPlan& plan, hipStream_t stream);
int wino22_launch(WinoRoute r, const rehr_gather_gemm_desc* ds, int count, const WinoPlan& plan, hipStream_t stream);
```

rehrseg_amd/hip_backend.py:

```python
from __future__ import annotations

import ctypes as C
import os
import functools
import weakref

import torch
from torch.optim.optimizer import register_optimizer_step_post_hook as _register_step_hook

from . import lib as L

name = "hip"


def _stream():
    return C.c_void_p(torch.cuda.current_stream().cuda_stream)


_prof = None


def profile_start():
    global _prof
    _prof = []
# ... 65 lines not shown
            continue
        if not t.is_cuda:
            raise L.RehrsegHipError("librehrseg_hip.so needs device tensors (no CPU fallback)")
        if t.dtype not in (torch.float32, torch.bfloat16):
            raise L.RehrsegHipError(f"unsupported dtype {t.dtype} (the kernels read float32, the mixed-precision "
                                    "variants bfloat16)")
    for t in f64:
        if t is None:
            continue
        if not t.is_cuda or t.dtype != torch.float64:
            raise L.RehrsegHipError("statistics buffers are float64 device tensors")


def _fn(base, t):
    name = base + ("_bf16" if t.dtype == torch.bfloat16 else "_f32")
    return getattr(L.load(), name), name


def _same_dtype(*ts):
    dts = {t.dtype for t in ts if t is not None}
    if len(dts) > 1:
        raise L.RehrsegHipError(f"activation operands of one call must share a dtype, got {sorted(map(str, dts))}")


_zero_pool = {}
_ZERO_CHUNK = 1 << 16


def zeros_f64(shape, device):
    n = 1
    for s in shape:
        n *= int(s)
    n_al = (n + 1) & ~1
    if n_al > _ZERO_CHUNK // 4:
        return torch.zeros(shape, dtype=torch.float64, device=device)
    key = (device.type, device.index, torch.cuda.current_stream(device).cuda_stream if device.type == "cuda" else 0)
    ent = _zero_pool.get(key)
    if ent is None or ent[1] + n_al > _ZERO_CHUNK:
        ent = [torch.zeros(_ZERO_CHUNK, dtype=torch.float64, device=device), 0]
        _zero_pool[key] = ent
    out = ent[0][ent[1]:ent[1] + n].view(shape)
    ent[1] += n_al
    return out


def new_act(N, Cc, D, H, W, like, zero=False, dtype=None):
    dt = dtype if dtype is not None else (like.dtype if like.dtype == torch.bfloat16 else torch.float32)
    t = torch.empty((N, Cc, D, H, W), dtype=dt, device=like.device, memory_format=torch.channels_last_3d)
    return t.zero_() if zero else t


WEIGHT_FORM_CACHE = True


def _after_optimizer_step(opt, args, kwargs):
    for g in opt.param_groups:
        for p in g["params"]:
            p._rehr_stamp = getattr(p, "_rehr_stamp", 0) + 1


_register_step_hook(_after_optimizer_step)


def _ver(p):
    return (p._version, getattr(p, "_rehr_stamp", 0))


keep_forms = False


def _keeps_forms(w):
    return WEIGHT_FORM_CACHE and keep_forms and isinstance(w, torch.nn.Parameter)


class _Form:
    __slots__ = ("param", "version", "out", "make", "stream", "readers", "dep", "__weakref__")

    def __init__(self, key, param, make, dep=None):
        self.param = weakref.ref(param, lambda _r, k=key: _drop_form(k))
        self.version = None
        self.out = None
        self.make = make
        self.stream = None
        self.readers = set()
        self.dep = dep


_forms = {}
_form_of_panel = {}
form_rebuilds = 0


def _drop_form(key):
    f = _forms.pop(key, None)
    if f is not None and key[0] == "pack":
        _form_of_panel.pop(id(f.out), None)


def invalidate_weight_forms():
    _forms.clear()
    _form_of_panel.clear()


def _form_ready(f, p):
    global form_rebuilds
    cur = torch.cuda.current_stream(p.device)
    v = _ver(p)
    if f.version != v:
        if f.dep is not None:
            _form_ready(f.dep, p)
        for r in f.readers:
            if r != cur:
                cur.wait_stream(r)
        if f.stream is not None and f.stream != cur:
            cur.wait_stream(f.stream)
        f.make(p)
        form_rebuilds += 1
        f.version, f.stream, f.readers = v, cur, set()
    if f.stream != cur and cur not in f.readers:
        cur.wait_stream(f.stream)
    f.readers.add(cur)


def _pack_launch(src, out, A, Apad, B, T, transpose):
    if out.dtype == torch.bfloat16:
        L.check(L.load().rehr_pack_weights_bf16(_ptr(src), _ptr(out), A, Apad, B, T, int(transpose), _stream()),
                "rehr_pack_weights_bf16")
    else:
        L.check(L.load().rehr_pack_weights_f32(_ptr(src), _ptr(out), A, Apad, B, T, int(transpose), _stream()),
                "rehr_pack_weights_f32")


def pack_weights(w, A, Apad, B, T, transpose, dtype=torch.float32, part=None):
    _chk_dev(w)
    if w.dtype != torch.float32:
        raise L.RehrsegHipError("master weights are float32")

    def src(p):
        return (p if part is None else p.narrow(*part)).contiguous()

    if not _keeps_forms(w):
        out = torch.empty((T, Apad, B), dtype=dtype, device=w.device)
        _pack_launch(src(w), out, A, Apad, B, T, transpose)
        return out
    key = ("pack", id(w), tuple(w.shape), part, A, Apad, B, T, bool(transpose), dtype)
    f = _forms.get(key)
    if f is None or f.param() is not w:
        out = torch.empty((T, Apad, B), dtype=dtype, device=w.device)
        f = _forms[key] = _Form(key, w, lambda p: _pack_launch(src(p), out, A, Apad, B, T, transpose))
        f.out = out
        _form_of_panel[id(out)] = f
    _form_ready(f, w)
    return f.out


USE_WINOGRAD = True
USE_WINOGRAD_WGRAD = True
USE_HALO_BF16 = True
WGRAD_TAP_COLOCATE = True
USE_WGRAD_TAP_SKIP = True
W32P_BLOCKS = 0
PHASE_INTERLEAVE = False
WINO_BAND_MAJOR = True
USE_TCONV_KS = True
USE_WINO_FLAT8 = True
WINO_FLAT8_TILES = 0
wino_wgrad_launches = 0
wino_launches = 0


def _gg_desc(d, x1, x2, c1, src_dims, Cin, lattice, s, b, taps, KH, KW, wp, Npad, y, y_dims, Cout,
             os_, ob, bias, act, slope, stats, stats_mode, tile):
    _chk_dev(x1, x2, wp, y, bias, f64=(stats,))
    d.x1, d.x2, d.c1 = _ptr(x1), _ptr(x2), c1
    d.ldx1 = x1.shape[1]
    d.ldx2 = x2.shape[1] if x2 is not None else 0
    d.N = x1.shape[0]
    d.Di, d.Hi, d.Wi = src_dims
    d.Cin = Cin
    d.Ld, d.Lh, d.Lw = lattice
    d.sd, d.sh, d.sw = s
    d.bd, d.bh, d.bw = b
    d.td, d.th, d.tw = _taps(taps[0]), _taps(taps[1]), _taps(taps[2])
    d.KH, d.KW = KH, KW
    d.wp, d.Npad = _ptr(wp), Npad
    d.y = _ptr(y)
    d.Dy, d.Hy, d.Wy = y_dims
    d.Cout, d.ldy = Cout, y.shape[1]
    d.osd, d.osh, d.osw = os_
    d.obd, d.obh, d.obw = ob
    d.bias, d.act, d.slope = _ptr(bias), act, slope
    d.stats, d.stats_mode = _ptr(stats), stats_mode
    d.tile_d, d.tile_h, d.tile_w = tile
    d.wino_ws, d.wino_ws_bytes = None, 0
    d.flags = 0
    d.debug_flags = 0
    need = 0
    if x1.dtype == torch.bfloat16:
        if wp.dtype != torch.bfloat16 or (x2 is not None and x2.dtype != torch.bfloat16):
            raise L.RehrsegHipError("mixed-precision gather-GEMM: x1, x2 and the packed weights must all be bfloat16")
        if bias is not None and bias.dtype != torch.float32:
            raise L.RehrsegHipError("bias stays float32")
        d.flags = L.GG_Y_F32 if y.dtype == torch.float32 else 0
        d.debug_flags = (0 if USE_HALO_BF16 else L.DBG_GG_NO_HALO)
    elif wp.dtype != torch.float32 or y.dtype != torch.float32 or (x2 is not None and x2.dtype != torch.float32):
        raise L.RehrsegHipError("fp32 gather-GEMM: every operand must be float32")
    elif USE_WINOGRAD and tile[0] >= 0:
        d.debug_flags = ((0 if USE_WINO_FLAT8 else L.DBG_GG_NO_FLAT8) |
                         {1: L.DBG_GG_W32P_TWO_PER_CU, 2: L.DBG_GG_W32P_ONE_PER_CU}.get(W32P_BLOCKS, 0) |
                         {1: L.DBG_GG_FLAT8_HALF, 2: L.DBG_GG_FLAT8_FULL}.get(WINO_FLAT8_TILES, 0))
        need = L.load().rehr_gather_gemm_wino_bytes(C.byref(d))
    if PHASE_INTERLEAVE:
        d.debug_flags |= L.DBG_GG_INTERLEAVE
    if not USE_TCONV_KS:
        d.debug_flags |= L.DBG_GG_NO_TCONV_KS
    if not WINO_BAND_MAJOR:
        d.debug_flags |= L.DBG_GG_SLICE_MAJOR
    _gg_desc.need = need
    _gg_desc.sig = (c1, x1.shape[1], x2.shape[1] if x2 is not None else 0, x1.shape[0], tuple(src_dims), Cin,
                    tuple(lattice), tuple(s), tuple(b), tuple(tuple(t) for t in taps), KH, KW, Npad, tuple(y_dims), Cout,
                    y.shape[1], tuple(os_), tuple(ob), bias is not None, act, stats_mode, tuple(tile), d.debug_flags)
    return _algo_flops(d.N, lattice, s, b, taps, src_dims, Cin, Cout) if _prof is not None else 0.0


def _attach_ws(descs, n, needs, sigs, wp):
    if not any(needs):
        return None
    global wino_launches
    wino_launches += sum(1 for nb in needs if nb)
    dev = wp.device
    pf = _form_of_panel.get(id(wp)) if WEIGHT_FORM_CACHE else None
    p = pf.param() if pf is not None else None
    if p is None or not _keeps_forms(p):
        keeps = [torch.empty(nb // 4, dtype=torch.float32, device=dev) if nb else None for nb in needs]
        for i in range(n):
            if needs[i]:
                descs[i].wino_ws, descs[i].wino_ws_bytes = _ptr(keeps[i]), needs[i]
        return keeps
    key = ("ws", id(p), id(pf), tuple(sigs))
    f = _forms.get(key)
    if f is None or f.param() is not p or f.dep is not pf:
        outs = [torch.empty(nb // 4, dtype=torch.float32, device=dev) if nb else None for nb in needs]
        cp = (L.GatherGemmDesc * n)()
        for i in range(n):
            C.memmove(C.byref(cp[i]), C.byref(descs[i]), C.sizeof(L.GatherGemmDesc))
            if needs[i]:
                cp[i].wino_ws, cp[i].wino_ws_bytes = _ptr(outs[i]), needs[i]
            cp[i].flags |= L.GG_WS_ONLY

        def make(_p, cp=cp, n=n):
            L.check(L.load().rehr_gather_gemm_multi_f32(cp, n, _stream()), "rehr_gather_gemm_multi_f32 (weight forms)")

        f = _forms[key] = _Form(key, p, make, dep=pf)
        f.out = outs
    _form_ready(f, p)
    for i in range(n):
        if needs[i]:
            descs[i].wino_ws, descs[i].wino_ws_bytes = _ptr(f.out[i]), needs[i]
        descs[i].flags |= L.GG_WS_READY
    return f.out


def _gg_tag(d):
    return (f"N{d.N} {d.Cin}->{d.Cout} lattice {d.Ld}x{d.Lh}x{d.Lw} stride {d.sd}{d.sh}{d.sw} "
            f"taps {d.td.count}x{d.th.count}x{d.tw.count}" + (" +x2" if d.x2 else "") +
            (" [" + _ROUTE_NAMES.get(wino_route(d)[0], "direct") + "]" if d.wino_ws else ""))


_ROUTE_NAMES = {L.GG_ROUTE_FLAT8: "flat8", L.GG_ROUTE_W32P: "w32p", L.GG_ROUTE_BIG8: "big8", L.GG_ROUTE_SMALL: "small",
                L.GG_ROUTE_FLAT22: "flat22", L.GG_ROUTE_REGION22: "region22"}


def wino_route(d):
    r = int(L.load().rehr_gather_gemm_wino_route(C.byref(d)))
    return r & 255, (r >> 8) & 255


def _gg_family(d):
    if _prof is None:
        return None
    if not d.wino_ws:
        return "gather_gemm"
    route = wino_route(d)[0]
    if route == L.GG_ROUTE_NONE:
        return "gather_gemm"
    return "wino22_conv" if route in (L.GG_ROUTE_FLAT22, L.GG_ROUTE_REGION22) else "wino_conv"


def gather_gemm(*args):
    d = L.GatherGemmDesc()
    flops = _gg_desc(d, *args)
    if args[0].dtype == torch.bfloat16:
        with _timed("gather_gemm_bf16", flops, lambda: _gg_tag(d)):
            L.check(L.load().rehr_gather_gemm_bf16(C.byref(d), _stream()), "rehr_gather_gemm_bf16")
        return
    arr = (L.GatherGemmDesc * 1)(d)
    keep = _attach_ws(arr, 1, [_gg_desc.need], [_gg_desc.sig], args[11])
    with _timed(_gg_family(arr[0]), flops, lambda: _gg_tag(arr[0])):
        L.check(L.load().rehr_gather_gemm_multi_f32(arr, 1, _stream()), "rehr_gather_gemm_f32")
    del keep


def gather_gemm_multi(calls):
    if len(calls) == 1:
        return gather_gemm(*calls[0])
    arr = (L.GatherGemmDesc * len(calls))()
    flops, needs, sigs = 0.0, [], []
    for i, a in enumerate(calls):
        flops += _gg_desc(arr[i], *a)
        needs.append(_gg_desc.need)
        sigs.append(_gg_desc.sig)
    if calls[0][0].dtype == torch.bfloat16:
        with _timed("gather_gemm_bf16", flops, lambda: f"{len(calls)} parts of " + _gg_tag(arr[0])):
            L.check(L.load().rehr_gather_gemm_multi_bf16(arr, len(calls), _stream()), "rehr_gather_gemm_multi_bf16")
        return
    keep = _attach_ws(arr, len(calls), needs, sigs, calls[0][11])
    with _timed(_gg_family(arr[0]) if all(arr[i].wino_ws for i in range(len(calls))) else "gather_gemm", flops,
                lambda: f"{len(calls)} parts of " + _gg_tag(arr[0])):
        L.check(L.load().rehr_gather_gemm_multi_f32(arr, len(calls), _stream()), "rehr_gather_gemm_multi_f32")
    del keep


def sum_slabs_bias_act(slabs, S, bias, act, slope, stats=None, out_dtype=None):
    _chk_dev(slabs, bias, f64=(stats,))
    if slabs.dtype != torch.float32:
        raise L.RehrsegHipError("split-K slabs are float32")
    SN, Cc, D, H, W = slabs.shape
    N = SN // S
    bf = out_dtype == torch.bfloat16
    y = new_act(N, Cc, D, H, W, like=slabs, dtype=torch.bfloat16 if bf else torch.float32)
    rows = N * D * H * W
    lib = L.load()
    if stats is not None:
        fn = lib.rehr_sum_slabs_stats_bf16 if bf else lib.rehr_sum_slabs_stats_f32
        L.check(fn(_ptr(slabs), S, rows * Cc, _ptr(bias), _ptr(y), N, D * H * W, Cc, act, slope, _ptr(stats), _stream()),
                "rehr_sum_slabs_stats")
        return y
    fn = lib.rehr_sum_slabs_bias_act_bf16 if bf else lib.rehr_sum_slabs_bias_act_f32
    L.check(fn(_ptr(slabs), S, rows * Cc, _ptr(bias), _ptr(y), rows, Cc, act, slope, _stream()), "rehr_sum_slabs_bias_act")
    return y


def wgrad(l, Ca, g, Cg, N, lattice, g_dims, s, b, taps, KH, KW, dst, dst_off, dst_strides, accumulate, dbias):
    _chk_dev(l, g, dst, dbias)
    bf16 = l.dtype == torch.bfloat16
    if (g.dtype == torch.bfloat16) != bf16 or dst.dtype != torch.float32:
        raise L.RehrsegHipError("weight gradient: l and g share one dtype (fp32 or bf16), dst is float32")
    d = L.WgradDesc()
    d.l, d.ldl, d.Ca = _ptr(l), l.shape[1], Ca
    d.g, d.ldg, d.Cg = _ptr(g), g.shape[1], Cg
    d.N = N
    d.Ld, d.Lh, d.Lw = lattice
    d.Dg, d.Hg, d.Wg = g_dims
    d.sd, d.sh, d.sw = s
    d.bd, d.bh, d.bw = b
    d.td, d.th, d.tw = _taps(taps[0]), _taps(taps[1]), _taps(taps[2])
    d.KH, d.KW = KH, KW
    d.dst = C.c_void_p(dst.data_ptr() + 4 * dst_off)
    d.dst_sa, d.dst_sc, d.dst_st = dst_strides
    d.accumulate = int(accumulate)
    d.dbias = _ptr(dbias)
    d.flags = 0
    d.debug_flags = ((0 if USE_WINOGRAD_WGRAD else L.DBG_WGRAD_DIRECT) | (0 if USE_WGRAD_TAP_SKIP else L.DBG_WGRAD_NO_TAP_SKIP) |
                     (0 if WGRAD_TAP_COLOCATE else L.DBG_WGRAD_NO_TAP_COLOCATE))
    lib = L.load()
    flops = _algo_flops(N, lattice, s, b, taps, g_dims, Ca, Cg) if _prof is not None else 0.0
    if bf16:
        if dbias is not None:
            raise L.RehrsegHipError("mixed-precision weight gradient has no fused bias gradient (use channel_sum)")
        nbytes = lib.rehr_wgrad_bf16_workspace_bytes(C.byref(d))
        if nbytes < 0:
            L.check(int(nbytes), "rehr_wgrad_bf16_workspace_bytes")
        ws = torch.empty((nbytes + 3) // 4, dtype=torch.float32, device=l.device)
        d.workspace, d.workspace_bytes = _ptr(ws), nbytes
        with _timed("wgrad_bf16", flops, lambda: f"N{N} {Ca}x{Cg} lattice {tuple(lattice)} stride {tuple(s)} "
                                             f"taps {taps[0][0]}x{taps[1][0]}x{taps[2][0]}"):
            L.check(lib.rehr_wgrad_bf16(C.byref(d), _stream()), "rehr_wgrad_bf16")
        return
    nbytes = lib.rehr_wgrad_workspace_bytes(C.byref(d))
    if nbytes < 0:
        L.check(int(nbytes), "rehr_wgrad_workspace_bytes")
    global wino_wgrad_launches
    wino = int(lib.rehr_wgrad_uses_winograd(C.byref(d)))
    wino_wgrad_launches += wino
    ws = torch.empty((nbytes + 3) // 4, dtype=torch.float32, device=l.device)
    d.workspace, d.workspace_bytes = _ptr(ws), nbytes
    with _timed(("wino_wgrad" if d.th.count == 3 else "wino22_wgrad") if wino else "wgrad", flops,
                lambda: f"N{N} {Ca}x{Cg} lattice {tuple(lattice)} stride {tuple(s)} taps {taps[0][0]}x{taps[1][0]}x{taps[2][0]}"):
        L.check(lib.rehr_wgrad_f32(C.byref(d), _stream()), "rehr_wgrad_f32")


def _direct_desc(x, w, bias, y, stride, pad, act, slope, stats, stats_mode):
    d = L.DirectConvDesc()
    N, Cin, Di, Hi, Wi = x.shape
    Cout, _, KD, KH, KW = w.shape
    _, _, Do, Ho, Wo = y.shape
    d.x, d.ldx, d.N, d.Di, d.Hi, d.Wi, d.Cin = _ptr(x), Cin, N, Di, Hi, Wi, Cin
    d.w, d.bias = _ptr(w), _ptr(bias)
    d.y, d.ldy, d.Do, d.Ho, d.Wo, d.Cout = _ptr(y), Cout, Do, Ho, Wo, Cout
    d.KD, d.KH, d.KW = KD, KH, KW
    d.sd, d.sh, d.sw = stride
    d.pd, d.ph, d.pw = pad
    d.act, d.slope = act, slope
    d.stats, d.stats_mode = _ptr(stats), stats_mode
    return d


def _shape_desc(x_shape, w_shape, stride, pad):
    d = L.DirectConvDesc()
    d.N, d.Cin, d.Di, d.Hi, d.Wi = x_shape
    d.Cout, _, d.KD, d.KH, d.KW = w_shape
    d.ldx, d.ldy = d.Cin, d.Cout
    d.sd, d.sh, d.sw = stride
    d.pd, d.ph, d.pw = pad
    d.Do, d.Ho, d.Wo = ((i + 2 * p - k) // s + 1 for i, k, s, p in zip(x_shape[2:], w_shape[2:], stride, pad))
    return d


@functools.lru_cache(maxsize=None)
def small_cin_bf16_out_ok(x_shape, w_shape, stride, pad):
    return bool(L.load().rehr_conv_small_cin_fwd_on_mfma(C.byref(_shape_desc(x_shape, w_shape, stride, pad))))


def small_cin_fwd(x, w, bias, y, stride, pad, act, slope, stats, stats_mode):
    _chk_dev(x, w, bias, y, f64=(stats,))
    if x.dtype != torch.float32:
        raise L.RehrsegHipError("thin-input conv: the input stays float32")
    d = _direct_desc(x, w.contiguous(), bias, y, stride, pad, act, slope, stats, stats_mode)
    if y.dtype == torch.bfloat16:
        L.check(L.load().rehr_conv_small_cin_fwd_ybf16(C.byref(d), _stream()), "rehr_conv_small_cin_fwd_ybf16")
        return
    L.check(L.load().rehr_conv_small_cin_fwd_f32(C.byref(d), _stream()), "rehr_conv_small_cin_fwd_f32")


def im2col(x, w, out_dims, stride, pad, Kpad):
    _chk_dev(x, w)
    N = x.shape[0]
    col = new_act(N, Kpad, *out_dims, like=x)
    d = _direct_desc(x, w, None, col, stride, pad, 0, 0.0, None, 0)
    d.Cout, d.ldy = w.shape[0], Kpad
    L.check(L.load().rehr_im2col_f32(C.byref(d), _ptr(col), Kpad, _stream()), "rehr_im2col_f32")
    return col


def small_cin_wgrad_on_mfma(x, w, dy, stride, pad):
    d = _direct_desc(x, w.contiguous(), None, dy, stride, pad, 0, 0.0, None, 0)
    return bool(L.load().rehr_conv_small_cin_wgrad_on_mfma(C.byref(d)))


def small_cin_wgrad(x, w, dy, stride, pad, want_bias):
    _chk_dev(x, w, dy)
    lib = L.load()
    d = _direct_desc(x, w.contiguous(), None, dy, stride, pad, 0, 0.0, None, 0)
    if dy.dtype == torch.bfloat16 and not lib.rehr_conv_small_cin_wgrad_on_mfma(C.byref(d)):
        dy = dy.float()
        d.y = _ptr(dy)
    nbytes = lib.rehr_conv_small_cin_wgrad_workspace_bytes(C.byref(d))
    ws = torch.empty((nbytes + 3) // 4, dtype=torch.float32, device=x.device)
    dw = torch.empty_like(w, memory_format=torch.contiguous_format)
    db = torch.empty(w.shape[0], dtype=torch.float32, device=x.device) if want_bias else None
    fn = lib.rehr_conv_small_cin_wgrad_dybf16 if dy.dtype == torch.bfloat16 else lib.rehr_conv_small_cin_wgrad_f32
    L.check(fn(C.byref(d), _ptr(dw), _ptr(db), _ptr(ws), nbytes, _stream()), "rehr_conv_small_cin_wgrad")
    return dw, db


def small_cout_fwd(x, w, bias, y, pad, act, slope):
    _chk_dev(x, w, bias, y)
    d = _direct_desc(x, w.contiguous(), bias, y, (1, 1, 1), pad, act, slope, None, 0)
    L.check(L.load().rehr_conv_small_cout_fwd_f32(C.byref(d), _stream()), "rehr_conv_small_cout_fwd_f32")


# ... 715 lines not shown
```

rehrseg_amd/lib.py:

```python
from __future__ import annotations

import ctypes as C
import os
import re
from typing import Optional

_HERE = os.path.dirname(os.path.abspath(__file__))
LIB_PATH = os.environ.get("REHRSEG_HIP_LIB") or os.path.join(_HERE, "librehrseg_hip.so")
HEADER_PATH = os.path.join(os.path.dirname(_HERE), "include", "rehrseg_hip.h")

ACT_NONE, ACT_RELU, ACT_LRELU = 0, 1, 2
ABI_VERSION = 6
GG_Y_F32 = 1
GG_WS_READY = 2
GG_WS_ONLY = 4
DBG_WGRAD_DIRECT = 1
DBG_WGRAD_NO_TAP_SKIP = 2
DBG_WGRAD_NO_TAP_COLOCATE = 4
DBG_GG_NO_HALO = 1
DBG_GG_NO_FLAT8 = 2
DBG_GG_FLAT8_HALF = 4
DBG_GG_FLAT8_FULL = 8
DBG_GG_W32P_TWO_PER_CU = 16
DBG_GG_W32P_ONE_PER_CU = 32
DBG_GG_INTERLEAVE = 64
DBG_GG_NO_TCONV_KS = 128
DBG_GG_SLICE_MAJOR = 256
GG_ROUTE_NONE, GG_ROUTE_FLAT8, GG_ROUTE_W32P, GG_ROUTE_BIG8 = 0, 1, 2, 3
GG_ROUTE_SMALL, GG_ROUTE_FLAT22, GG_ROUTE_REGION22 = 4, 5, 6

_i32, _i64, _f32 = C.c_int32, C.c_int64, C.c_float
_vp = C.c_void_p


class AxisTaps(C.Structure):
    _fields_ = [("count", _i32), ("off0", _i32), ("offs", _i32), ("k0", _i32), ("ks", _i32)]

    def __init__(self, count=1, off0=0, offs=1, k0=0, ks=1):
        super().__init__(count, off0, offs, k0, ks)

    def astuple(self):
        return (self.count, self.off0, self.offs, self.k0, self.ks)


class GatherGemmDesc(C.Structure):
    _fields_ = [
        ("x1", _vp), ("x2", _vp), ("c1", _i32), ("ldx1", _i32), ("ldx2", _i32),
        ("N", _i32), ("Di", _i32), ("Hi", _i32), ("Wi", _i32), ("Cin", _i32),
        ("Ld", _i32), ("Lh", _i32), ("Lw", _i32),
        ("sd", _i32), ("sh", _i32), ("sw", _i32), ("bd", _i32), ("bh", _i32), ("bw", _i32),
        ("td", AxisTaps), ("th", AxisTaps), ("tw", AxisTaps), ("KH", _i32), ("KW", _i32),
        ("wp", _vp), ("Npad", _i32),
        ("y", _vp), ("Dy", _i32), ("Hy", _i32), ("Wy", _i32), ("Cout", _i32), ("ldy", _i32),
        ("osd", _i32), ("osh", _i32), ("osw", _i32), ("obd", _i32), ("obh", _i32), ("obw", _i32),
        ("bias", _vp), ("act", _i32), ("slope", _f32),
        ("stats", _vp), ("stats_mode", _i32),
        ("tile_d", _i32), ("tile_h", _i32), ("tile_w", _i32),
        ("wino_ws", _vp), ("wino_ws_bytes", _i64),
        ("flags", _i32), ("debug_flags", _i32),
    ]


class WgradDesc(C.Structure):
    _fields_ = [
        ("l", _vp), ("ldl", _i32), ("Ca", _i32),
        ("g", _vp), ("ldg", _i32), ("Cg", _i32),
        ("N", _i32), ("Ld", _i32), ("Lh", _i32), ("Lw", _i32),
        ("Dg", _i32), ("Hg", _i32), ("Wg", _i32),
        ("sd", _i32), ("sh", _i32), ("sw", _i32), ("bd", _i32), ("bh", _i32), ("bw", _i32),
        ("td", AxisTaps), ("th", AxisTaps), ("tw", AxisTaps), ("KH", _i32), ("KW", _i32),
        ("dst", _vp), ("dst_sa", _i64), ("dst_sc", _i64), ("dst_st", _i64),
        ("accumulate", _i32),
        ("workspace", _vp), ("workspace_bytes", _i64),
        ("dbias", _vp),
        ("flags", _i32), ("debug_flags", _i32),
    ]


class DirectConvDesc(C.Structure):
    _fields_ = [
        ("x", _vp), ("ldx", _i32), ("N", _i32), ("Di", _i32), ("Hi", _i32), ("Wi", _i32), ("Cin", _i32),
        ("w", _vp), ("bias", _vp),
        ("y", _vp), ("ldy", _i32), ("Do", _i32), ("Ho", _i32), ("Wo", _i32), ("Cout", _i32),
        ("KD", _i32), ("KH", _i32), ("KW", _i32), ("sd", _i32), ("sh", _i32), ("sw", _i32),
        ("pd", _i32), ("ph", _i32), ("pw", _i32),
        ("act", _i32), ("slope", _f32), ("stats", _vp), ("stats_mode", _i32),
    ]


PATCH_F32, PATCH_U8, PATCH_MAX_ITEMS = 0, 1, 16


class PatchItem(C.Structure):
    _fields_ = [("src", _vp), ("base", _i64), ("stride", _i64 * 4), ("lo", _i32 * 4), ("hi", _i32 * 4)]


class PatchGatherDesc(C.Structure):
    _fields_ = [("n_items", _i32), ("dims", _i32 * 4), ("src_dtype", _i32), ("scale", _f32), ("bias", _f32),
                ("dst", _vp), ("dst_item_stride", _i64)]


_P_GG, _P_WG, _P_DC = C.POINTER(GatherGemmDesc), C.POINTER(WgradDesc), C.POINTER(DirectConvDesc)

PROTOTYPES = {
    "rehr_gather_gemm_wino_bytes": (_i64, [_P_GG]),
    "rehr_gather_gemm_wino_route": (C.c_int, [_P_GG]),
    "rehr_gather_gemm_f32": (C.c_int, [_P_GG, _vp]),
    "rehr_gather_gemm_multi_f32": (C.c_int, [_P_GG, _i32, _vp]),
    "rehr_gather_gemm_bf16": (C.c_int, [_P_GG, _vp]),
    "rehr_gather_gemm_multi_bf16": (C.c_int, [_P_GG, _i32, _vp]),
    "rehr_pack_weights_bf16": (C.c_int, [_vp, _vp, _i32, _i32, _i32, _i32, _i32, _vp]),
    "rehr_sum_slabs_bias_act_f32": (C.c_int, [_vp, _i32, _i64, _vp, _vp, _i64, _i32, _i32, _f32, _vp]),
    "rehr_sum_slabs_stats_f32": (C.c_int, [_vp, _i32, _i64, _vp, _vp, _i32, _i64, _i32, _i32, _f32, _vp, _vp]),
    "rehr_sum_slabs_bias_act_bf16": (C.c_int, [_vp, _i32, _i64, _vp, _vp, _i64, _i32, _i32, _f32, _vp]),
    "rehr_sum_slabs_stats_bf16": (C.c_int, [_vp, _i32, _i64, _vp, _vp, _i32, _i64, _i32, _i32, _f32, _vp, _vp]),
    "rehr_wgrad_workspace_bytes": (_i64, [_P_WG]),
    "rehr_wgrad_uses_winograd": (C.c_int, [_P_WG]),
    "rehr_wgrad_f32": (C.c_int, [_P_WG, _vp]),
    "rehr_wgrad_bf16_workspace_bytes": (_i64, [_P_WG]),
    "rehr_wgrad_bf16": (C.c_int, [_P_WG, _vp]),
    "rehr_pack_weights_f32": (C.c_int, [_vp, _vp, _i32, _i32, _i32, _i32, _i32, _vp]),
    "rehr_conv_small_cin_fwd_f32": (C.c_int, [_P_DC, _vp]),
    "rehr_im2col_f32": (C.c_int, [_P_DC, _vp, _i32, _vp]),
    "rehr_conv_small_cin_wgrad_workspace_bytes": (_i64, [_P_DC]),
    "rehr_conv_small_cin_wgrad_on_mfma": (C.c_int, [_P_DC]),
    "rehr_conv_small_cin_fwd_on_mfma": (C.c_int, [_P_DC]),
    "rehr_conv_small_cin_fwd_ybf16": (C.c_int, [_P_DC, _vp]),
    "rehr_conv_small_cin_wgrad_dybf16": (C.c_int, [_P_DC, _vp, _vp, _vp, _i64, _vp]),
    "rehr_conv_small_cin_wgrad_f32": (C.c_int, [_P_DC, _vp, _vp, _vp, _i64, _vp]),
    "rehr_conv_small_cout_fwd_f32": (C.c_int, [_P_DC, _vp]),
    "rehr_conv_small_cout_dgrad_f32": (C.c_int, [_P_DC, _vp, _vp]),
    "rehr_conv_small_cout_wgrad_workspace_bytes": (_i64, [_P_DC]),
    "rehr_conv_small_cout_wgrad_f32": (C.c_int, [_P_DC, _vp, _vp, _vp, _i64, _vp]),
    "rehr_se_gate_fwd_f32": (C.c_int, [_vp, _vp, _vp, _vp, _vp, _i32, _i32, _i64, _vp]),
    "rehr_scale_res_act_fwd_f32": (C.c_int, [_vp, _i32, _vp, _vp, _i32, _vp, _i32, _i32, _i64, _i32, _i32, _f32, _vp]),
    "rehr_scale_res_act_bwd_f32": (C.c_int, [_vp, _i32, _vp, _i32, _vp, _i32, _vp, _vp, _i32, _vp, _i32, _vp,
                                             _i32, _i64, _i32, _i32, _f32, _vp]),
    "rehr_se_gate_bwd_f32": (C.c_int, [_vp, _vp, _vp, _vp, _vp, _vp, _vp, _i32, _i32, _i64, _vp]),
    "rehr_add_channel_const_f32": (C.c_int, [_vp, _i32, _vp, _i32, _i64, _i32, _vp]),
    "rehr_instnorm_act_fwd_f32": (C.c_int, [_vp, _i32, _vp, _vp, _vp, _vp, _i32, _vp, _i32, _i64, _i32, _f32,
                                            _i32, _f32, _vp]),
    "rehr_instnorm_act_bwd_f32": (C.c_int, [_vp, _i32, _vp, _i32, _vp, _vp, _vp, _vp, _i32, _vp, _vp, _vp,
                                            _i32, _i64, _i32, _i32, _f32, _vp]),
    "rehr_upsample_depth_fwd_f32": (C.c_int, [_vp, _vp, _i32, _i32, _i32, _i64, _i32, _vp]),
    "rehr_upsample_depth_bwd_f32": (C.c_int, [_vp, _vp, _i32, _i32, _i32, _i64, _i32, _vp]),
    "rehr_upmix_depth_fwd_f32": (C.c_int, [_vp, _vp, _vp, _i32, _i32, _i32, _i64, _i32, _i32, _i32, _i32, C.c_float, _vp]),
    "rehr_upmix_depth_bwd_f32": (C.c_int, [_vp, _vp, _vp, _i32, _i32, _i32, _i64, _i32, _i32, _i32, _i32, C.c_float, _vp]),
    "rehr_channel_sum_actgrad_f32": (C.c_int, [_vp, _vp, _i32, _i64, _i32, _i32, C.c_float, _vp, _vp, _vp]),
    "rehr_cosdist_stats_f32": (C.c_int, [_vp, _vp, _vp, _i32, _i64, _i32, _vp]),
    "rehr_cosdist_bwd_f32": (C.c_int, [_vp, _vp, _vp, _vp, _i32, _i64, _i32, C.c_float, _vp]),
    "rehr_uasr_mix_blocks": (_i32, [_i32, _i32, _i64]),
    "rehr_uasr_mix_fwd_f32": (C.c_int, [_vp, _vp, _vp, _vp, _vp, _vp, _i32, _i32, _i32, _i64, _vp]),
    "rehr_uasr_mix_bwd_f32": (C.c_int, [_vp, _vp, _vp, _vp, _vp, _vp, _vp, _vp, _vp, _i32, _i32, _i32, _i64, _vp]),
    "rehr_quad_maxpool_fwd_f32": (C.c_int, [_vp, _vp, _vp, _i64, _i32, _i32, _i32, _vp]),
    "rehr_quad_maxpool_bwd_f32": (C.c_int, [_vp, _vp, _vp, _i64, _i32, _i32, _i32, _vp]),
    "rehr_window_stem_assemble_f32": (C.c_int, [_vp, _vp, _vp, _vp, _vp, _vp, _i32, _i32, _i32, _i64, _i32, _i32, C.c_float, _vp]),
    "rehr_window_stem_assemble_bf16": (C.c_int, [_vp, _vp, _vp, _vp, _vp, _vp, _i32, _i32, _i32, _i64, _i32, _i32, C.c_float, _vp]),
    "rehr_conv5_thin_f32_workspace_bytes": (_i64, [_P_DC]),
    "rehr_conv5_thin_f32_supported": (C.c_int, [_P_DC]),
    "rehr_conv5_thin_fwd_f32": (C.c_int, [_P_DC, _vp, _i64, _vp]),
    "rehr_conv5_thin_dgrad_f32": (C.c_int, [_P_DC, _vp, _i32, _vp, _i64, _vp]),
    "rehr_conv5_thin_wgrad_f32": (C.c_int, [_P_DC, _vp, _vp, _vp, _i64, _vp]),
    "rehr_conv5_thin_workspace_bytes": (_i64, [_P_DC]),
    "rehr_conv5_thin_dgrad_bf16": (C.c_int, [_P_DC, _vp, _i32, _vp, _i64, _vp]),
    "rehr_conv5_thin_wgrad_bf16": (C.c_int, [_P_DC, _vp, _vp, _vp, _i64, _vp]),
    "rehr_upmix_depth_fwd_bf16": (C.c_int, [_vp, _vp, _vp, _i32, _i32, _i32, _i64, _i32, _i32, _i32, _i32, C.c_float, _vp]),
    "rehr_upmix_depth_bwd_bf16": (C.c_int, [_vp, _vp, _vp, _i32, _i32, _i32, _i64, _i32, _i32, _i32, _i32, C.c_float, _vp]),
    "rehr_channel_sum_actgrad_bf16": (C.c_int, [_vp, _vp, _i32, _i64, _i32, _i32, C.c_float, _vp, _vp, _vp]),
    "rehr_conv5_thin_supported": (C.c_int, [_P_DC]),
    "rehr_conv5_thin_fwd_bf16": (C.c_int, [_P_DC, _vp, _i64, _vp]),
    "rehr_patch_gather": (C.c_int, [C.POINTER(PatchGatherDesc), C.POINTER(PatchItem), _vp]),
    "rehr_axis_resample_f32": (C.c_int, [_vp, _vp, _vp, _vp, _i64, _i32, _i32, _i64, _i32, _vp]),
    "rehr_aug_warp2d_f32": (C.c_int, [_vp, _vp, _vp, _i32, _i32, _i32, _i32, _i32, _i32, _i32, _vp]),
    "rehr_aug_stats_f32": (C.c_int, [_vp, _i32, _i64, _vp, _vp, _vp]),
    "rehr_aug_pointwise_f32": (C.c_int, [_vp, _i32, _i64, _i32, _vp, _vp, _vp, _vp]),
    "rehr_tta_gather_f32": (C.c_int, [_vp, _vp] + [_i32] * 12 + [_vp]),
    "rehr_tta_blend_f16acc": (C.c_int, [_vp, _vp, _i32, _i32, _i32, _i32, _vp, _vp, _vp] + [_i32] * 6 + [_vp]),
    "rehr_seg_eval_finalize_f16": (C.c_int, [_vp, _vp] + [_i32] * 9 + [_vp, _vp, _vp, _vp]),
    "rehr_minmax_f32": (C.c_int, [_vp, _i64, _vp, _vp]),
    "rehr_sr_window_gather_f32": (C.c_int, [_vp, _vp] + [_i32] * 8 + [_vp]),
    "rehr_sr_volume_scatter_f32": (C.c_int, [_vp, _vp] + [_i32] * 7 + [_vp, _vp, _vp, _vp, _vp]),
    "rehr_stage2_prep_f32": (C.c_int, [_vp, _vp, _vp, _i32, _vp, _i32, _i64, _vp]),
    "rehr_stage2_unc_u8_f32": (C.c_int, [_vp, _vp, _vp, _i64, _vp]),
    "rehr_zoom_depth_f32": (C.c_int, [_vp, _i64, _i32, _i32, _vp, _vp, _vp, _i32, _vp, _vp, _vp]),
    "rehr_bspline_prefilter_axis_f64acc_f32": (C.c_int, [_vp, _vp, _i64, _i32, _i64, _vp]),
    "rehr_blur_to_slices_f32": (C.c_int, [_vp, _vp, _i32, _vp, _i32, _i32, _i32, _i32, _vp]),
    "rehr_sr_metrics_workspace_bytes": (_i64, [_i32] * 4),
    "rehr_sr_metrics_f32": (C.c_int, [_vp] * 8 + [_i32] * 4 + [_f32, _vp, _vp, _i64, _vp]),
    "rehr_sr_metrics_bf16": (C.c_int, [_vp] * 8 + [_i32] * 4 + [_f32, _vp, _vp, _i64, _vp]),
    "rehr_seg_loss_fwd_f32": (C.c_int, [_vp, _i32, _vp, _vp, _i32, _i32, _i64, _vp, _vp]),
    "rehr_seg_loss_bwd_f32": (C.c_int, [_vp, _i32, _vp, _vp, _i32, _i32, _i64, _vp, _f32, _f32, _f32, _i32, _vp,
                                        _vp, _i32, _vp]),
    "rehr_bce_dice_fwd_f32": (C.c_int, [_vp, _vp, _i32, _i32, _i64, _vp, _vp]),
    "rehr_bce_dice_bwd_f32": (C.c_int, [_vp, _vp, _i32, _i32, _i64, _vp, _f32, _f32, _vp, _vp, _vp]),
    "rehr_act_fwd_f32": (C.c_int, [_vp, _vp, _i64, _i32, _f32, _vp]),
    "rehr_act_bwd_f32": (C.c_int, [_vp, _vp, _vp, _i64, _i32, _f32, _vp]),
    "rehr_channel_sum_f32": (C.c_int, [_vp, _i32, _i64, _i32, _vp, _i32, _vp, _vp]),
    "rehr_copy_channels_f32": (C.c_int, [_vp, _i32, _vp, _i32, _i64, _i32, _vp]),
    "rehr_nchw_to_nhwc_f32": (C.c_int, [_vp, _vp, _i32, _i32, _i64, _vp]),
    "rehr_nhwc_to_nchw_f32": (C.c_int, [_vp, _vp, _i32, _i32, _i64, _vp]),
    "rehr_scale_res_act_fwd_bf16": (C.c_int, [_vp, _i32, _vp, _vp, _i32, _vp, _i32, _i32, _i64, _i32, _i32, _f32, _vp]),
    "rehr_scale_res_act_bwd_bf16": (C.c_int, [_vp, _i32, _vp, _i32, _vp, _i32, _vp, _vp, _i32, _vp, _i32, _vp,
                                              _i32, _i64, _i32, _i32, _f32, _vp]),
    "rehr_add_channel_const_bf16": (C.c_int, [_vp, _i32, _vp, _i32, _i64, _i32, _vp]),
    "rehr_instnorm_act_fwd_bf16": (C.c_int, [_vp, _i32, _vp, _vp, _vp, _vp, _i32, _vp, _i32, _i64, _i32, _f32,
                                             _i32, _f32, _vp]),
    "rehr_instnorm_act_bwd_bf16": (C.c_int, [_vp, _i32, _vp, _i32, _vp, _vp, _vp, _vp, _i32, _vp, _vp, _vp,
                                             _i32, _i64, _i32, _i32, _f32, _vp]),
    "rehr_instnorm_act_bwd_dbias_bf16": (C.c_int, [_vp, _i32, _vp, _i32, _vp, _vp, _vp, _vp, _i32, _vp, _vp, _vp,
                                                   _i32, _i64, _i32, _i32, _f32, _vp, _vp, _vp]),
    "rehr_channel_sum_bf16": (C.c_int, [_vp, _i32, _i64, _i32, _vp, _i32, _vp, _vp]),
    "rehr_act_bwd_bf16": (C.c_int, [_vp, _vp, _vp, _i64, _i32, _f32, _vp]),
    "rehr_abi_version": (C.c_int, []),
    "rehr_last_hip_error": (C.c_char_p, []),
}

_ERR = {-1: "REHR_EINVAL (malformed descriptor)", -2: "REHR_ENOSUP (unsupported shape)",
        -3: "REHR_EHIP (hip launch error)"}


class RehrsegHipError(RuntimeError):
    pass


def declared_symbols(header_path: str = HEADER_PATH):
    text = open(header_path).read()
    text = re.sub(r"/\*.*?\*/", "", text, flags=re.S)
    return sorted(set(re.findall(r"\b(rehr_[a-z0-9_]+)\s*\(", text)))


_lib: Optional[C.CDLL] = None


def load() -> C.CDLL:
    global _lib
    if _lib is not None:
        return _lib
    if not os.path.exists(LIB_PATH):
        raise RehrsegHipError(
            f"{LIB_PATH} not found: build it with `python -c 'import __graft_entry__ as g; g.build()'` "
            "(hipcc --offload-arch=gfx950).  There is no CPU fallback for the product path.")
    import torch
    if torch.cuda.is_available():
        torch.cuda.init()
    lib = C.CDLL(LIB_PATH)
    for name, (res, args) in PROTOTYPES.items():
        fn = getattr(lib, name)
        fn.restype = res
        fn.argtypes = args
    ver = lib.rehr_abi_version()
    if ver != ABI_VERSION:
        raise RehrsegHipError(f"ABI version mismatch: library {ver}, binding {ABI_VERSION}")
    _lib = lib
    return lib


def check(rc: int, what: str):
    if rc != 0:
        detail = ""
        if rc == -3 and _lib is not None:
            detail = f": {_lib.rehr_last_hip_error().decode()}"
        raise RehrsegHipError(f"{what} failed: {_ERR.get(rc, rc)}{detail}")
```

rehrseg_amd/ops.py:

```python
from __future__ import annotations

import functools
import itertools
import weakref
from dataclasses import dataclass
from typing import Optional, Tuple

import torch

from . import hip_backend

ACT_NONE, ACT_RELU, ACT_LRELU = 0, 1, 2

_backend = hip_backend


def get_backend():
    return _backend


def set_backend(b):
    global _backend
    old = _backend
    _backend = b
    return old


_mixed = False


class mixed_precision:

    def __init__(self, enabled=True):
        self.enabled = bool(enabled)

    def __enter__(self):
        global _mixed
        self.prev, _mixed = _mixed, self.enabled
        return self

    def __exit__(self, *exc):
        global _mixed
        _mixed = self.prev
        return False


def is_mixed_precision():
    return _mixed


def to_cl(x: torch.Tensor) -> torch.Tensor:
    if x.dim() != 5:
        raise ValueError(f"expected a 5-D (N,C,D,H,W) tensor, got {tuple(x.shape)}")
    if x.dtype not in (torch.float32, torch.bfloat16, torch.float64):
        x = x.float()
    if x.permute(0, 2, 3, 4, 1).is_contiguous():
        return x
    return x.permute(0, 2, 3, 4, 1).contiguous().permute(0, 4, 1, 2, 3)


def _triple(v):
    if isinstance(v, int):
        return (v, v, v)
    v = tuple(int(a) for a in v)
    if len(v) != 3:
        raise ValueError(f"expected 3 values, got {v}")
    return v


def conv_out_dim(i, k, s, p):
    return (i + 2 * p - k) // s + 1


def phase_taps(K, s, p, phase):
    k0 = (phase + p) % s
    if k0 >= K:
        return None
    count = (K - k0 + s - 1) // s
    off0 = (phase + p - k0) // s
    return (count, off0, -1, k0, s)


def full_taps(K):
    return (K, 0, 1, 0, 1)


@functools.lru_cache(maxsize=None)
def choose_tile(lattice, thin=(False, False, False)):
    Ld, Lh, Lw = lattice
    best = None
    for td in (1, 2, 4, 8, 16, 32, 64, 128):
        for th in (1, 2, 4, 8, 16, 32, 64, 128):
            if 128 % (td * th):
                continue
            tw = 128 // (td * th)
            if (thin[0] and td > 1) or (thin[1] and th > 1) or (thin[2] and tw > 1):
                continue
            vol = (-(-Ld // td) * td) * (-(-Lh // th) * th) * (-(-Lw // tw) * tw)
            halo = (td + 2) * (th + 2) * (tw + 2)
            key = (vol, halo, -tw)
            if best is None or key < best[0]:
                best = (key, (td, th, tw))
    lin = -(-(Ld * Lh * Lw) // 128) * 128
    if best is None or (best[0][0] > 1.10 * lin and not any(thin)):
        return (0, 0, 0)
    return best[1]


def pad_rows(a):
    if a % 128 == 0 or a % 64 == 0:
        return a
    return -(-a // 32) * 32


@dataclass(frozen=True)
class ConvCfg:
    stride: Tuple[int, int, int]
    pad: Tuple[int, int, int]
    transposed: bool = False
    act: int = ACT_NONE
    slope: float = 0.0
    mode: str = "plain"
    eps: float = 1e-5
    y_fp32: bool = False


def _spatial(x):
    return tuple(x.shape[2:])


def _out_dims(in_dims, w_shape, cfg: ConvCfg):
    K = tuple(w_shape[2:])
    if cfg.transposed:
        return tuple((i - 1) * s - 2 * p + k for i, k, s, p in zip(in_dims, K, cfg.stride, cfg.pad))
    return tuple(conv_out_dim(i, k, s, p) for i, k, s, p in zip(in_dims, K, cfg.stride, cfg.pad))


def _pack(w, dest_dim, dtype=torch.float32, part=None):
    be = get_backend()
    T = w.shape[2] * w.shape[3] * w.shape[4]
    kw = {"dtype": torch.bfloat16} if dtype == torch.bfloat16 else {}
    shape = list(w.shape)
    if part is not None:
        if hasattr(be, "invalidate_weight_forms"):
            kw["part"] = part
        else:
            w = w.narrow(*part).contiguous()
        shape[part[0]] = part[2]
    if dest_dim == 0:
        A, B = shape[0], shape[1]
        return be.pack_weights(w, A, pad_rows(A), B, T, False, **kw), pad_rows(A)
    A, B = shape[1], shape[0]
    return be.pack_weights(w, A, pad_rows(A), B, T, True, **kw), pad_rows(A)


def _phased_gather(src1, src2, c1, Csrc, wp, Npad, dst, Cdst, K, stride, pad, bias, act, slope, stats, stats_mode):
    be = get_backend()
    src_dims, dst_dims = _spatial(src1), _spatial(dst)
    calls = []
    for ph in itertools.product(*(range(s) for s in stride)):
        taps = [phase_taps(K[a], stride[a], pad[a], ph[a]) for a in range(3)]
        lattice = tuple((dst_dims[a] - ph[a] + stride[a] - 1) // stride[a] for a in range(3))
        if min(lattice) <= 0:
            continue
        if any(t is None for t in taps):
            continue
        thin = tuple(src_dims[a] == 1 and taps[a][0] > 1 for a in range(3))
        calls.append((src1, src2, c1, src_dims, Csrc, lattice, (1, 1, 1), (0, 0, 0), taps, K[1], K[2], wp, Npad,
                      dst, dst_dims, Cdst, stride, ph, bias, act, slope, stats, stats_mode,
                      choose_tile(tuple(lattice), thin)))
    if calls:
        be.gather_gemm_multi(calls)


def _has_empty_phase(K, stride, pad):
    return any(phase_taps(K[a], stride[a], pad[a], ph) is None for a in range(3) for ph in range(stride[a]))


def _thin_out(w, cfg: ConvCfg, has_x2):
    return (not cfg.transposed and not has_x2 and w.shape[0] <= 4 and w.shape[1] % 16 == 0 and
            cfg.stride == (1, 1, 1) and w.shape[4] <= 7)


def _thin5_f32(be, x, w, cfg: ConvCfg, shape=None):
    return (x.dtype == torch.float32 and x.is_cuda and hasattr(be, "thin5_supported") and
            be.thin5_supported(tuple(shape if shape is not None else x.shape), tuple(w.shape), cfg.pad, torch.float32))


WINO_TAP_SPLIT = True


def _sub_taps(t, a, b):
    cnt, off0, offs, k0, ks = t
    return (b - a, off0 + offs * a, offs, k0 + ks * a, ks)


def _tap_split(lattice, N, Npad, taps, Cin, bf16=False):
    vox = lattice[0] * lattice[1] * lattice[2]
    blocks = -(-vox // 128) * (Npad // (128 if Npad % 128 == 0 else (64 if Npad % 64 == 0 else 32))) * N
    T = taps[0][0] * taps[1][0] * taps[2][0]
    if blocks > 160 or T * Cin < 2048 or taps[0][0] * taps[1][0] < 2:
        return None
    if not bf16 and taps[0][0] <= 3 and taps[1][0] == 3 and taps[2][0] == 3 and taps[1][2] in (1, -1) and taps[2][2] in (1, -1):
        Lh, Lw = lattice[1], lattice[2]
        if (WINO_TAP_SPLIT and taps[0][0] == 3 and lattice[0] >= 2 and Lh % 16 == 0 and Lw % 16 == 0 and Npad % 64 == 0 and
                (Lh // 16) * (Lw // 16) * lattice[0] * N * (Npad // 64) <= 160):
            return [[_sub_taps(taps[0], a, a + 1), taps[1], taps[2]] for a in range(3)]
        if Lh >= 8 and Lw >= 8 and (-(-Lh // 8) * 8) * (-(-Lw // 16) * 16) * 100 <= Lh * Lw * 134:
            return None
        tps = -(-Lh // 2) * -(-Lw // 2)
        if (6 <= Lh <= 16 and 6 <= Lw <= 16 and 16 <= tps < 64 and Npad % 64 == 0 and
                -(-(N * lattice[0] * tps) // 64) * (Npad // 64) >= 128):
            return None
    want = min(8, max(2, 512 // blocks))
    kd, kh = taps[0][0], taps[1][0]
    nd = min(kd, want)
    nh = 2 if (kh >= 2 and nd * 2 <= want) else 1
    dstep, hstep = -(-kd // nd), -(-kh // nh)
    parts = []
    for a in range(0, kd, dstep):
        for c in range(0, kh, hstep):
            parts.append([_sub_taps(taps[0], a, min(kd, a + dstep)), _sub_taps(taps[1], c, min(kh, c + hstep)), taps[2]])
    return parts if len(parts) > 1 else None


def conv_forward(x1, x2, w, bias, cfg: ConvCfg, act, slope, stats_mode):
    be = get_backend()
    N = x1.shape[0]
    c1 = x1.shape[1]
    Cin = c1 + (x2.shape[1] if x2 is not None else 0)
    K = tuple(w.shape[2:])
    in_dims = _spatial(x1)
    out_dims = _out_dims(in_dims, w.shape, cfg)
    Cout = w.shape[1] if cfg.transposed else w.shape[0]
    if (w.shape[0] if cfg.transposed else w.shape[1]) != Cin:
        raise ValueError(f"weight {tuple(w.shape)} does not match {Cin} input channels")
    stats = None
    if stats_mode:
        stats = (be.zeros_f64((N, Cout, 2), x1.device) if hasattr(be, "zeros_f64")
                 else torch.zeros((N, Cout, 2), dtype=torch.float64, device=x1.device))
    if Cin <= 2:
        if cfg.transposed or x2 is not None:
            raise ValueError("thin-input path handles plain Conv3d only")
        okw = {}
        if (_mixed and not cfg.y_fp32 and x1.dtype == torch.float32 and hasattr(be, "small_cin_bf16_out_ok") and
                be.small_cin_bf16_out_ok(tuple(x1.shape), tuple(w.shape), tuple(cfg.stride), tuple(cfg.pad))):
            okw["dtype"] = torch.bfloat16
        y = be.new_act(N, Cout, *out_dims, like=x1, **okw)
        be.small_cin_fwd(x1, w, bias, y, cfg.stride, cfg.pad, act, slope, stats, stats_mode)
        return y, stats
    if _thin_out(w, cfg, x2 is not None):
        if stats_mode:
            raise NotImplementedError("statistics epilogue on a thin-output conv")
        if x1.dtype == torch.bfloat16:
            if act != ACT_NONE:
                raise NotImplementedError("activation behind the bf16 thin-output conv")
            return be.thin5_fwd(x1, w, bias), None
        if act == ACT_NONE and _thin5_f32(be, x1, w, cfg):
            return be.thin5_fwd(x1, w, bias), None
        y = be.new_act(N, Cout, *out_dims, like=x1)
        be.small_cout_fwd(x1, w, bias, y, cfg.pad, act, slope)
        return y, None
    if cfg.transposed:
        empty = _has_empty_phase(K, cfg.stride, cfg.pad)
        if empty and bias is not None:
            raise NotImplementedError("ConvTranspose3d with unreachable output phases and a bias")
        y = be.new_act(N, Cout, *out_dims, like=x1, zero=empty)
        wp, Npad = _pack(w, 1, x1.dtype)
        _phased_gather(x1, x2, c1, Cin, wp, Npad, y, Cout, K, cfg.stride, cfg.pad, bias, act, slope, stats,
                       stats_mode)
        return y, stats
    wp, Npad = _pack(w, 0, x1.dtype)
    taps = [full_taps(k) for k in K]
    bf16 = x1.dtype == torch.bfloat16
    parts = _tap_split(out_dims, N, Npad, taps, Cin, bf16)
    if parts is not None and Cout % 4 == 0:
        S = len(parts)
        slabs = be.new_act(S * N, Cout, *out_dims, like=x1, **({"dtype": torch.float32} if bf16 else {}))
        calls = [(x1, x2, c1, in_dims, Cin, out_dims, cfg.stride, tuple(-p for p in cfg.pad), tp, K[1], K[2],
                  wp, Npad, slabs[s_i * N:(s_i + 1) * N], out_dims, Cout, (1, 1, 1), (0, 0, 0), None,
                  ACT_NONE, 0.0, None, 0, choose_tile(tuple(out_dims))) for s_i, tp in enumerate(parts)]
        be.gather_gemm_multi(calls)
        okw = {"out_dtype": torch.bfloat16} if bf16 else {}
        return be.sum_slabs_bias_act(slabs, S, bias, act, slope, stats if stats_mode else None, **okw), stats
    y = be.new_act(N, Cout, *out_dims, like=x1)
    be.gather_gemm(x1, x2, c1, in_dims, Cin, out_dims, cfg.stride, tuple(-p for p in cfg.pad), taps, K[1], K[2],
                   wp, Npad, y, out_dims, Cout, (1, 1, 1), (0, 0, 0), bias, act, slope, stats, stats_mode,
                   choose_tile(tuple(out_dims)))
    return y, stats


def conv_dgrad(dz, w, in_dims, c1, c2, cfg: ConvCfg, need1=True, need2=True, x_dtype=None):
    be = get_backend()
    N = dz.shape[0]
    K = tuple(w.shape[2:])
    Cz = dz.shape[1]
    if _thin_out(w, cfg, c2 > 0):
        if x_dtype == torch.bfloat16:
            return (be.thin5_dgrad(dz.float() if dz.dtype != torch.float32 else dz, w) if need1 else None), None
        if dz.dtype == torch.float32 and _thin5_f32(be, dz, w, cfg, (N, c1) + tuple(in_dims)):
            return (be.thin5_dgrad(dz, w, torch.float32) if need1 else None), None
        return (be.small_cout_dgrad(dz, w, (N, c1) + tuple(in_dims), cfg.pad) if need1 else None), None
    out = []
    for (lo, cnt, need) in ((0, c1, need1), (c1, c2, need2)):
        if cnt == 0 or not need:
            out.append(None)
# ... 368 lines not shown
```

Before: 16.88 patches/s.

## Build Winograd weight forms directly from master weights, skipping packed panels

Adds a weight-source path that computes Winograd-transformed weight forms straight from the strided fp32 master weight tensor. For convolutions that only read the Winograd forms it skips materialising the packed weight panel, removing one pack kernel and its intermediate buffer per conv call. The path uses new source and LDS-staged transform kernels. Shapes that still need the panel fall back to packing, which adds host-side planning checks and a second dispatch path.

Measured after the change: 16.93 patches/s (median of 6 runs). About the same (+0.3%).

```diff
diff --git a/include/rehrseg_hip.h b/include/rehrseg_hip.h
--- a/include/rehrseg_hip.h
+++ b/include/rehrseg_hip.h
@@ -70,6 +70,15 @@
 #define REHR_GG_ROUTE_REGION22 6
 int rehr_gather_gemm_wino_route(const rehr_gather_gemm_desc* d);
 int rehr_gather_gemm_f32(const rehr_gather_gemm_desc* d, void* stream);
+typedef struct {
+  const float* w;
+  int64_t sn, sc, st;
+  int32_t rows, cols;
+  int32_t taps;
+  int32_t reserved;
+} rehr_weight_src;
+int rehr_gather_gemm_weight_forms_f32(const rehr_gather_gemm_desc* descs, int32_t count, const rehr_weight_src* src,
+                                      void* stream);
 int rehr_gather_gemm_multi_f32(const rehr_gather_gemm_desc* descs, int32_t count,
                                void* stream);
 int rehr_gather_gemm_bf16(const rehr_gather_gemm_desc* d, void* stream);
diff --git a/rehrseg_amd/csrc/gather_gemm.hip b/rehrseg_amd/csrc/gather_gemm.hip
--- a/rehrseg_amd/csrc/gather_gemm.hip
+++ b/rehrseg_amd/csrc/gather_gemm.hip
@@ -328,12 +328,13 @@
   return WINO_NONE;
 }
 
-static int wino_run(WinoRoute r, const rehr_gather_gemm_desc* ds, int count, const WinoPlan& plan, hipStream_t st) {
+static int wino_run(WinoRoute r, const rehr_gather_gemm_desc* ds, int count, const WinoPlan& plan, hipStream_t st,
+                    const rehr_weight_src* src) {
   for (int i = 0; i < count; ++i) {
-    const int rc = r >= WINO_FLAT22 ? wino22_weights_launch(ds[i], plan, st) : wino_weights_launch(r, ds[i], plan, st);
+    const int rc = r >= WINO_FLAT22 ? wino22_weights_launch(ds[i], plan, st, src) : wino_weights_launch(r, ds[i], plan, st, src);
     if (rc != REHR_OK) return rc;
   }
-  if (ds[0].flags & REHR_GG_WS_ONLY) return REHR_OK;
+  if ((ds[0].flags & REHR_GG_WS_ONLY) || src != nullptr) return REHR_OK;
   switch (r) {
     case WINO_FLAT8: return wino_flat8_launch(ds[0], plan, st);
     case WINO_W32P: case WINO_BIG8: case WINO_SMALL: return wino_region_launch(r, ds, count, plan, st);
@@ -341,7 +342,22 @@
   }
 }
 
-extern "C" int rehr_gather_gemm_multi_f32(const rehr_gather_gemm_desc* descs, int32_t count, void* stream) {
+static bool gg_reads_panel(const rehr_gather_gemm_desc* descs, int count) {
+  if (count > 1 && tconv_ks_takes(descs, count, false)) return true;
+  WinoPlan plan{};
+  if (count > 1 && descs[0].wino_ws != nullptr) {
+    const int taps = descs[0].td.count;
+    if ((taps > 3 || taps == 1) && wino_split_plan(descs, count, plan)) return false;
+    if (taps <= 3 && wino22_flat_multi_plan(descs, count, plan)) return false;
+  }
+  for (int i = 0; i < count; ++i) {
+    if (descs[i].wino_ws == nullptr || (count > 1 && descs[i].td.count > 3)) return true;
+    if (wino_route(descs[i], plan) == WINO_NONE || !wino_ws_ok(descs[i], plan.bytes)) return true;
+  }
+  return false;
+}
+
+static int gg_multi_f32(const rehr_gather_gemm_desc* descs, int32_t count, void* stream, const rehr_weight_src* src) {
   if (descs == nullptr || count < 1 || count > MAX_PHASES) return REHR_EINVAL;
   for (int i = 0; i < count; ++i) {
     const int rc = validate(descs[i]);
@@ -351,9 +367,18 @@
       return REHR_EINVAL;
   }
   hipStream_t st = (hipStream_t)stream;
-  const bool ws_only = (descs[0].flags & REHR_GG_WS_ONLY) != 0;
+  const bool ws_only = (descs[0].flags & REHR_GG_WS_ONLY) != 0 || src != nullptr;
   for (int i = 1; i < count; ++i)
     if ((descs[i].flags ^ descs[0].flags) & (REHR_GG_WS_ONLY | REHR_GG_WS_READY)) return REHR_EINVAL;
+  if (src != nullptr) {
+    if (descs[0].flags & (REHR_GG_WS_ONLY | REHR_GG_WS_READY)) return REHR_EINVAL;
+    if (src->w == nullptr || ((uintptr_t)src->w & 3) || src->sn < 0 || src->sc < 0 || src->st < 0 ||
+        src->taps < 1)
+      return REHR_EINVAL;
+    for (int i = 0; i < count; ++i)
+      if (src->rows < 1 || src->rows > descs[i].Npad || src->cols < 1 || src->cols > descs[i].Cin) return REHR_EINVAL;
+    if (gg_reads_panel(descs, count)) return REHR_ENOSUP;
+  }
   if (count > 1 && !ws_only) {
     const int trc = tconv_ks_try(descs, count, false, st);
     if (trc != REHR_ENOSUP) return trc;
@@ -361,8 +386,8 @@
   WinoPlan plan{};
   if (count > 1 && descs[0].wino_ws != nullptr) {
     const int taps = descs[0].td.count;
-    if ((taps > 3 || taps == 1) && wino_split_plan(descs, count, plan)) return wino_run(WINO_BIG8, descs, count, plan, st);
-    if (taps <= 3 && wino22_flat_multi_plan(descs, count, plan)) return wino_run(WINO_FLAT22, descs, count, plan, st);
+    if ((taps > 3 || taps == 1) && wino_split_plan(descs, count, plan)) return wino_run(WINO_BIG8, descs, count, plan, st, src);
+    if (taps <= 3 && wino22_flat_multi_plan(descs, count, plan)) return wino_run(WINO_FLAT22, descs, count, plan, st, src);
   }
   GGMulti pm;
   pm.interleave = 0;
@@ -373,7 +398,7 @@
     if (descs[i].wino_ws != nullptr && !(count > 1 && descs[i].td.count > 3)) {
       const WinoRoute r = wino_route(descs[i], plan);
       if (r != WINO_NONE && wino_ws_ok(descs[i], plan.bytes)) {
-        const int wrc = wino_run(r, &descs[i], 1, plan, st);
+        const int wrc = wino_run(r, &descs[i], 1, plan, st, src);
         if (wrc != REHR_OK) return wrc;
         continue;
       }
@@ -392,6 +417,16 @@
   return launch_generic(pm, n, st);
 }
 
+extern "C" int rehr_gather_gemm_multi_f32(const rehr_gather_gemm_desc* descs, int32_t count, void* stream) {
+  return gg_multi_f32(descs, count, stream, nullptr);
+}
+
+extern "C" int rehr_gather_gemm_weight_forms_f32(const rehr_gather_gemm_desc* descs, int32_t count,
+                                                 const rehr_weight_src* src, void* stream) {
+  if (src == nullptr) return REHR_EINVAL;
+  return gg_multi_f32(descs, count, stream, src);
+}
+
 extern "C" int64_t rehr_gather_gemm_wino_bytes(const rehr_gather_gemm_desc* dp) {
   WinoPlan plan{};
   if (dp == nullptr || validate(*dp) != REHR_OK || wino_route(*dp, plan) == WINO_NONE) return 0;
diff --git a/rehrseg_amd/csrc/gg_shared.h b/rehrseg_amd/csrc/gg_shared.h
--- a/rehrseg_amd/csrc/gg_shared.h
+++ b/rehrseg_amd/csrc/gg_shared.h
@@ -112,3 +112,4 @@
 }
 
 int tconv_ks_try(const rehr_gather_gemm_desc* ds, int count, bool bf16, hipStream_t stream);
+bool tconv_ks_takes(const rehr_gather_gemm_desc* ds, int count, bool bf16);
diff --git a/rehrseg_amd/csrc/tconv_ks.hip b/rehrseg_amd/csrc/tconv_ks.hip
--- a/rehrseg_amd/csrc/tconv_ks.hip
+++ b/rehrseg_amd/csrc/tconv_ks.hip
@@ -308,6 +308,13 @@
 
 }
 
+bool tconv_ks_takes(const rehr_gather_gemm_desc* ds, int count, bool bf16) {
+  if (ds[0].debug_flags & REHR_DBG_GG_NO_TCONV_KS) return false;
+  TconvKsParams p;
+  if (!tconv_ks_match(ds, count, bf16, p)) return false;
+  return (p.vox_total + TK_BM - 1) / TK_BM < (1ll << 31) && (bf16 || p.Cin <= 64);
+}
+
 int tconv_ks_try(const rehr_gather_gemm_desc* ds, int count, bool bf16, hipStream_t stream) {
   if (ds[0].debug_flags & REHR_DBG_GG_NO_TCONV_KS) return REHR_ENOSUP;
   TconvKsParams p;
diff --git a/rehrseg_amd/csrc/wino22_conv.hip b/rehrseg_amd/csrc/wino22_conv.hip
--- a/rehrseg_amd/csrc/wino22_conv.hip
+++ b/rehrseg_amd/csrc/wino22_conv.hip
@@ -55,6 +55,99 @@
       const int64_t o = (((((int64_t)pj * 9 + x) * NT + nt) * kchunks + chunk) * 4 + kk) * 256 + (half * 32 + col) * 4 + e;
       up[o] = u[x];
     }
+  }
+}
+
+__global__ void w22_weights_src_kernel(const rehr_gather_gemm_desc d, const rehr_weight_src s, float* __restrict__ up,
+                                       int kchunks) {
+  AxisPlan ah, aw;
+  plan_axis(d.th, d.sh, d.bh, ah);
+  plan_axis(d.tw, d.sw, d.bw, aw);
+  const int nphase = ah.nph * aw.nph;
+  const int NT = d.Npad / 32;
+  const int64_t items = (int64_t)NT * kchunks * 256;
+  for (int64_t q = (int64_t)blockIdx.x * blockDim.x + threadIdx.x; q < items; q += (int64_t)gridDim.x * blockDim.x) {
+    const int lane = (int)(q & 63), kk = (int)(q >> 6) & 3;
+    const int64_t tc = q >> 8;
+    const int chunk = (int)(tc % kchunks), nt = (int)(tc / kchunks);
+    const int n = nt * 32 + (lane & 31), ci0 = chunk * 32 + kk * 8 + (lane >> 5) * 4;
+    for (int pj = 0; pj < nphase * d.td.count; ++pj) {
+      const int p = pj / d.td.count, jd = pj - p * d.td.count;
+      const int p_h = p / aw.nph, p_w = p - p_h * aw.nph;
+      f32x4 uu[9];
+#pragma unroll
+      for (int e = 0; e < 4; ++e) {
+        const int ci = ci0 + e;
+        float g[2][2];
+#pragma unroll
+        for (int a = 0; a < 2; ++a)
+#pragma unroll
+          for (int b = 0; b < 2; ++b) {
+            const int wt = ((d.td.k0 + d.td.ks * jd) * d.KH + ah.kidx[p_h][a]) * d.KW + aw.kidx[p_w][b];
+            g[a][b] = wsrc_tap(s, wt, n, ci);
+          }
+        float u[9];
+        u[0] = g[0][0];              u[1] = g[0][0] + g[0][1];                     u[2] = g[0][1];
+        u[3] = g[0][0] + g[1][0];    u[4] = g[0][0] + g[0][1] + g[1][0] + g[1][1]; u[5] = g[0][1] + g[1][1];
+        u[6] = g[1][0];              u[7] = g[1][0] + g[1][1];                     u[8] = g[1][1];
+#pragma unroll
+        for (int x = 0; x < 9; ++x) uu[x][e] = u[x];
+      }
+#pragma unroll
+      for (int x = 0; x < 9; ++x) *reinterpret_cast<f32x4*>(up + (((int64_t)pj * 9 + x) * items + q) * 4) = uu[x];
+    }
+  }
+}
+
+__global__ __launch_bounds__(64) void w22_weights_lds_kernel(const rehr_gather_gemm_desc d, const rehr_weight_src s,
+                                                             float* __restrict__ up, int kchunks, int mode) {
+  extern __shared__ __attribute__((aligned(16))) float wl[];
+  AxisPlan ah, aw;
+  plan_axis(d.th, d.sh, d.bh, ah);
+  plan_axis(d.tw, d.sw, d.bw, aw);
+  const int nphase = ah.nph * aw.nph;
+  const int NT = d.Npad / 32;
+  const int64_t items = (int64_t)NT * kchunks * 256;
+  const int lane = threadIdx.x, col = lane & 31, half = lane >> 5;
+  const int kk = blockIdx.x & 3, tc = blockIdx.x >> 2;
+  const int chunk = tc % kchunks, nt = tc / kchunks;
+  const int64_t q = (int64_t)blockIdx.x * 64 + lane;
+  const int n0 = nt * 32, c0 = chunk * 32 + kk * 8;
+  const WsrcLds g = wsrc_lds(s, mode);
+  wsrc_stage(s, mode, g, n0, c0, lane, wl);
+  __syncthreads();
+  const int n = n0 + col, ci0 = c0 + half * 4;
+  const int pj_lo = gridDim.y > 1 ? blockIdx.y : 0, pj_hi = gridDim.y > 1 ? blockIdx.y + 1 : nphase * d.td.count;
+  for (int pj = pj_lo; pj < pj_hi; ++pj) {
+    const int p = pj / d.td.count, jd = pj - p * d.td.count;
+    const int p_h = p / aw.nph, p_w = p - p_h * aw.nph;
+    int wt[2][2];
+#pragma unroll
+    for (int a = 0; a < 2; ++a)
+#pragma unroll
+      for (int b = 0; b < 2; ++b)
+        wt[a][b] = ((d.td.k0 + d.td.ks * jd) * d.KH + (p_h ? ah.kidx[1][a] : ah.kidx[0][a])) * d.KW +
+                   (p_w ? aw.kidx[1][b] : aw.kidx[0][b]);
+    f32x4 uu[9];
+#pragma unroll
+    for (int e = 0; e < 4; ++e) {
+      const int ci = ci0 + e;
+      const float* tp = wl + col * g.pr + (half * 4 + e) * g.pc;
+      const bool live = n < s.rows && ci < s.cols;
+      float g2[2][2];
+#pragma unroll
+      for (int a = 0; a < 2; ++a)
+#pragma unroll
+        for (int b = 0; b < 2; ++b) g2[a][b] = live ? tp[wt[a][b]] : 0.f;
+      float u[9];
+      u[0] = g2[0][0];               u[1] = g2[0][0] + g2[0][1];                       u[2] = g2[0][1];
+      u[3] = g2[0][0] + g2[1][0];    u[4] = g2[0][0] + g2[0][1] + g2[1][0] + g2[1][1]; u[5] = g2[0][1] + g2[1][1];
+      u[6] = g2[1][0];               u[7] = g2[1][0] + g2[1][1];                       u[8] = g2[1][1];
+#pragma unroll
+      for (int x = 0; x < 9; ++x) uu[x][e] = u[x];
+    }
+#pragma unroll
+    for (int x = 0; x < 9; ++x) *reinterpret_cast<f32x4*>(up + (((int64_t)pj * 9 + x) * items + q) * 4) = uu[x];
   }
 }
 
@@ -645,7 +738,14 @@
   return true;
 }
 
-int wino22_weights_launch(const rehr_gather_gemm_desc& d, const WinoPlan& plan, hipStream_t stream) {
+int wino22_weights_launch(const rehr_gather_gemm_desc& d, const WinoPlan& plan, hipStream_t stream,
+                          const rehr_weight_src* src) {
+  if (src != nullptr) {
+    const int64_t items = (int64_t)(d.Npad / 32) * plan.kchunks * 256;
+    if (const int mode = wsrc_mode(*src))
+      return wino_transform_launch_lds<w22_weights_lds_kernel>(d, *src, mode, items, plan.nphase * d.td.count, stream, plan.kchunks);
+    return wino_transform_launch_src<w22_weights_src_kernel>(d, *src, items, 8192, stream, plan.kchunks);
+  }
   const int64_t total = (int64_t)plan.nphase * d.td.count * d.Npad * plan.kchunks * 32;
   return wino_transform_launch<w22_weights_kernel>(d, total, 8192, stream, plan.kchunks);
 }
diff --git a/rehrseg_amd/csrc/wino_conv.hip b/rehrseg_amd/csrc/wino_conv.hip
--- a/rehrseg_amd/csrc/wino_conv.hip
+++ b/rehrseg_amd/csrc/wino_conv.hip
@@ -295,6 +295,144 @@
                           (half * 32 + col) * 4 + e;
         up[o] = t[r][0] * G[c][0] + t[r][1] * G[c][1] + t[r][2] * G[c][2];
       }
+  }
+}
+
+__global__ void wino_weights_frag_src_kernel(const rehr_gather_gemm_desc d, const rehr_weight_src s, float* __restrict__ up,
+                                             int kchunks) {
+  const float G[4][3] = {{1.f, 0.f, 0.f}, {.5f, .5f, .5f}, {.5f, -.5f, .5f}, {0.f, 0.f, 1.f}};
+  const int NT = d.Npad / 32;
+  const int64_t items = (int64_t)NT * kchunks * 256;
+  for (int64_t i = (int64_t)blockIdx.x * blockDim.x + threadIdx.x; i < items * d.td.count; i += (int64_t)gridDim.x * blockDim.x) {
+    const int jd = (int)(i / items);
+    const int64_t q = i - jd * items;
+    const int lane = (int)(q & 63), kk = (int)(q >> 6) & 3;
+    const int64_t tc = q >> 8;
+    const int chunk = (int)(tc % kchunks), nt = (int)(tc / kchunks);
+    const int n = nt * 32 + (lane & 31), ci0 = chunk * 32 + kk * 8 + (lane >> 5) * 4;
+    {
+      f32x4 u[16];
+#pragma unroll
+      for (int e = 0; e < 4; ++e) {
+        const int ci = ci0 + e;
+        float g[3][3];
+#pragma unroll
+        for (int jh = 0; jh < 3; ++jh)
+#pragma unroll
+          for (int jw = 0; jw < 3; ++jw) {
+            const int a = d.bh + d.th.off0 + d.th.offs * jh + 1;
+            const int b = d.bw + d.tw.off0 + d.tw.offs * jw + 1;
+            const int wt = ((d.td.k0 + d.td.ks * jd) * d.KH + (d.th.k0 + d.th.ks * jh)) * d.KW + (d.tw.k0 + d.tw.ks * jw);
+            const float v = wsrc_tap(s, wt, n, ci);
+#pragma unroll
+            for (int aa = 0; aa < 3; ++aa)
+#pragma unroll
+              for (int bb = 0; bb < 3; ++bb)
+                if (aa == a && bb == b) g[aa][bb] = v;
+          }
+        float t[4][3];
+#pragma unroll
+        for (int r = 0; r < 4; ++r)
+#pragma unroll
+          for (int b = 0; b < 3; ++b) t[r][b] = G[r][0] * g[0][b] + G[r][1] * g[1][b] + G[r][2] * g[2][b];
+#pragma unroll
+        for (int r = 0; r < 4; ++r)
+#pragma unroll
+          for (int c = 0; c < 4; ++c) u[r * 4 + c][e] = t[r][0] * G[c][0] + t[r][1] * G[c][1] + t[r][2] * G[c][2];
+      }
+#pragma unroll
+      for (int xi = 0; xi < 16; ++xi)
+        *reinterpret_cast<f32x4*>(up + (((int64_t)jd * 16 + xi) * items + q) * 4) = u[xi];
+    }
+  }
+}
+
+__global__ __launch_bounds__(64) void wino_weights_frag_lds_kernel(const rehr_gather_gemm_desc d, const rehr_weight_src s,
+                                                                   float* __restrict__ up, int kchunks, int mode) {
+  extern __shared__ __attribute__((aligned(16))) float wl[];
+  const float G[4][3] = {{1.f, 0.f, 0.f}, {.5f, .5f, .5f}, {.5f, -.5f, .5f}, {0.f, 0.f, 1.f}};
+  const int NT = d.Npad / 32;
+  const int64_t items = (int64_t)NT * kchunks * 256;
+  const int lane = threadIdx.x, col = lane & 31, half = lane >> 5;
+  const int kk = blockIdx.x & 3, tc = blockIdx.x >> 2;
+  const int chunk = tc % kchunks, nt = tc / kchunks;
+  const int64_t q = (int64_t)blockIdx.x * 64 + lane;
+  const int n0 = nt * 32, c0 = chunk * 32 + kk * 8;
+  const WsrcLds g = wsrc_lds(s, mode);
+  wsrc_stage(s, mode, g, n0, c0, lane, wl);
+  __syncthreads();
+  const int n = n0 + col, ci0 = c0 + half * 4;
+  int kh[3], kw[3];
+#pragma unroll
+  for (int aa = 0; aa < 3; ++aa) {
+    kh[aa] = d.th.k0 + d.th.ks * ((aa - 1 - d.bh - d.th.off0) * d.th.offs);
+    kw[aa] = d.tw.k0 + d.tw.ks * ((aa - 1 - d.bw - d.tw.off0) * d.tw.offs);
+  }
+  const int jd_lo = gridDim.y > 1 ? blockIdx.y : 0, jd_hi = gridDim.y > 1 ? blockIdx.y + 1 : d.td.count;
+  for (int jd = jd_lo; jd < jd_hi; ++jd) {
+    f32x4 u[16];
+#pragma unroll
+    for (int e = 0; e < 4; ++e) {
+      const int ci = ci0 + e;
+      const float* tp = wl + col * g.pr + (half * 4 + e) * g.pc;
+      const bool live = n < s.rows && ci < s.cols;
+      float g3[3][3];
+#pragma unroll
+      for (int aa = 0; aa < 3; ++aa)
+#pragma unroll
+        for (int bb = 0; bb < 3; ++bb) {
+          const int wt = ((d.td.k0 + d.td.ks * jd) * d.KH + kh[aa]) * d.KW + kw[bb];
+          g3[aa][bb] = live ? tp[wt] : 0.f;
+        }
+      float t[4][3];
+#pragma unroll
+      for (int r = 0; r < 4; ++r)
+#pragma unroll
+        for (int b = 0; b < 3; ++b) t[r][b] = G[r][0] * g3[0][b] + G[r][1] * g3[1][b] + G[r][2] * g3[2][b];
+#pragma unroll
+      for (int r = 0; r < 4; ++r)
+#pragma unroll
+        for (int c = 0; c < 4; ++c) u[r * 4 + c][e] = t[r][0] * G[c][0] + t[r][1] * G[c][1] + t[r][2] * G[c][2];
+    }
+#pragma unroll
+    for (int xi = 0; xi < 16; ++xi)
+      *reinterpret_cast<f32x4*>(up + (((int64_t)jd * 16 + xi) * items + q) * 4) = u[xi];
+  }
+}
+
+__global__ void wino_weights_src_kernel(const rehr_gather_gemm_desc d, const rehr_weight_src s, float* __restrict__ up) {
+  const float G[4][3] = {{1.f, 0.f, 0.f}, {.5f, .5f, .5f}, {.5f, -.5f, .5f}, {0.f, 0.f, 1.f}};
+  const int64_t per = (int64_t)d.Npad * d.Cin;
+  const int64_t total = (int64_t)d.td.count * per;
+  for (int64_t i = (int64_t)blockIdx.x * blockDim.x + threadIdx.x; i < total; i += (int64_t)gridDim.x * blockDim.x) {
+    const int jd = (int)(i / per);
+    const int64_t nc = i - (int64_t)jd * per;
+    const int n = (int)(nc / d.Cin), ci = (int)(nc - (int64_t)n * d.Cin);
+    float g[3][3];
+#pragma unroll
+    for (int jh = 0; jh < 3; ++jh)
+#pragma unroll
+      for (int jw = 0; jw < 3; ++jw) {
+        const int a = d.bh + d.th.off0 + d.th.offs * jh + 1;
+        const int b = d.bw + d.tw.off0 + d.tw.offs * jw + 1;
+        const int wt = ((d.td.k0 + d.td.ks * jd) * d.KH + (d.th.k0 + d.th.ks * jh)) * d.KW + (d.tw.k0 + d.tw.ks * jw);
+        const float v = wsrc_tap(s, wt, n, ci);
+#pragma unroll
+        for (int aa = 0; aa < 3; ++aa)
+#pragma unroll
+          for (int bb = 0; bb < 3; ++bb)
+            if (aa == a && bb == b) g[aa][bb] = v;
+      }
+    float t[4][3];
+#pragma unroll
+    for (int r = 0; r < 4; ++r)
+#pragma unroll
+      for (int b = 0; b < 3; ++b) t[r][b] = G[r][0] * g[0][b] + G[r][1] * g[1][b] + G[r][2] * g[2][b];
+#pragma unroll
+    for (int r = 0; r < 4; ++r)
+#pragma unroll
+      for (int c = 0; c < 4; ++c)
+        up[((int64_t)jd * 16 + r * 4 + c) * per + nc] = t[r][0] * G[c][0] + t[r][1] * G[c][1] + t[r][2] * G[c][2];
   }
 }
 
@@ -957,7 +1095,16 @@
   return true;
 }
 
-int wino_weights_launch(WinoRoute r, const rehr_gather_gemm_desc& d, const WinoPlan& plan, hipStream_t stream) {
+int wino_weights_launch(WinoRoute r, const rehr_gather_gemm_desc& d, const WinoPlan& plan, hipStream_t stream,
+                        const rehr_weight_src* src) {
+  if (src != nullptr) {
+    if (r == WINO_SMALL)
+      return wino_transform_launch_src<wino_weights_src_kernel>(d, *src, (int64_t)d.td.count * d.Npad * d.Cin, 4096, stream);
+    const int64_t items = (int64_t)(d.Npad / 32) * plan.kchunks * 256;
+    if (const int mode = wsrc_mode(*src))
+      return wino_transform_launch_lds<wino_weights_frag_lds_kernel>(d, *src, mode, items, d.td.count, stream, plan.kchunks);
+    return wino_transform_launch_src<wino_weights_frag_src_kernel>(d, *src, items * d.td.count, 8192, stream, plan.kchunks);
+  }
   if (r == WINO_SMALL)
     return wino_transform_launch<wino_weights_kernel>(d, (int64_t)d.td.count * d.Npad * d.Cin, 4096, stream);
   return wino_transform_launch<wino_weights_frag_kernel>(d, (int64_t)d.td.count * d.Npad * plan.kchunks * 32, 8192, stream,
diff --git a/rehrseg_amd/csrc/wino_shared.h b/rehrseg_amd/csrc/wino_shared.h
--- a/rehrseg_amd/csrc/wino_shared.h
+++ b/rehrseg_amd/csrc/wino_shared.h
@@ -160,14 +160,105 @@
   return REHR_OK;
 }
 
+template <auto KERN, typename... Args>
+static int wino_transform_launch_src(const rehr_gather_gemm_desc& d, const rehr_weight_src& s, int64_t items, int cap,
+                                     hipStream_t stream, Args... args) {
+  if (d.flags & REHR_GG_WS_READY) return REHR_EINVAL;
+  int64_t blocks = (items + 255) / 256;
+  if (blocks > cap) blocks = cap;
+  hipLaunchKernelGGL(KERN, dim3((unsigned)blocks), dim3(256), 0, stream, d, s, d.wino_ws, args...);
+  REHR_LAUNCH_CHECK();
+  return REHR_OK;
+}
+__device__ inline float wsrc_tap(const rehr_weight_src& s, int wt, int n, int ci) {
+  return (n < s.rows && ci < s.cols) ? s.w[(int64_t)wt * s.st + (int64_t)n * s.sn + (int64_t)ci * s.sc] : 0.f;
+}
+
+enum { WSRC_NONE = 0, WSRC_FWD = 1, WSRC_TRANS = 2 };
+constexpr int WSRC_MAX_T = 56;
+inline int wsrc_mode(const rehr_weight_src& s) {
+  if (s.st != 1 || ((uintptr_t)s.w & 15)) return WSRC_NONE;
+  if (s.taps > WSRC_MAX_T) return WSRC_NONE;
+  if (s.sc == s.taps && s.sn % 4 == 0) return WSRC_FWD;
+  if (s.sn == s.taps && s.sc % 4 == 0) return WSRC_TRANS;
+  return WSRC_NONE;
+}
+struct WsrcLds { int T, pr, pc, floats; };
+inline __host__ __device__ WsrcLds wsrc_lds(const rehr_weight_src& s, int mode) {
+  WsrcLds g;
+  if (mode == WSRC_FWD) { g.T = (int)s.sc; g.pc = g.T; g.pr = 8 * g.T + 1; g.floats = 32 * g.pr; }
+  else { g.T = (int)s.sn; g.pr = g.T | 1; g.pc = 32 * g.pr; g.floats = 8 * g.pc; }
+  return g;
+}
+__device__ inline void wsrc_stage(const rehr_weight_src& s, int mode, const WsrcLds& g, int n0, int c0, int lane,
+                                  float* __restrict__ lds) {
+  const int per_sub = g.T;
+  int vr = s.rows - n0; vr = vr > 32 ? 32 : vr;
+  const int vc = c0 < s.cols ? (s.cols - c0 > 8 ? 8 : s.cols - c0) : 0;
+  const int rlen = mode == WSRC_FWD ? vc * per_sub : (vr > 0 ? vr * per_sub : 0);
+  const int vruns = mode == WSRC_FWD ? (vr > 0 ? vr : 0) : vc;
+  const int quads = (rlen + 3) / 4;
+  const int total = vruns * quads;
+  constexpr int U = 28;
+  const float inv_quads = 1.f / (float)(quads > 0 ? quads : 1), inv_sub = 1.f / (float)per_sub;
+  for (int base = 0; base < total; base += 64 * U) {
+    f32x4 q[U];
+#pragma unroll
+    for (int u = 0; u < U; ++u) {
+      const int idx = base + u * 64 + lane;
+      q[u] = f32x4{0.f, 0.f, 0.f, 0.f};
+      if (idx < total) {
+        const int run = (int)(((float)idx + 0.5f) * inv_quads), i0 = (idx - run * quads) * 4;
+        const float* src = mode == WSRC_FWD ? s.w + (int64_t)(n0 + run) * s.sn + (int64_t)c0 * s.sc
+                                            : s.w + (int64_t)(c0 + run) * s.sc + (int64_t)n0 * s.sn;
+        if (i0 + 4 <= rlen) {
+          q[u] = *reinterpret_cast<const f32x4*>(src + i0);
+        } else {
+#pragma unroll
+          for (int k = 0; k < 4; ++k)
+            if (i0 + k < rlen) q[u][k] = src[i0 + k];
+        }
+      }
+    }
+#pragma unroll
+    for (int u = 0; u < U; ++u) {
+      const int idx = base + u * 64 + lane;
+      if (idx < total) {
+        const int run = (int)(((float)idx + 0.5f) * inv_quads), i0 = (idx - run * quads) * 4;
+        int sub = (int)(((float)i0 + 0.5f) * inv_sub), t = i0 - sub * per_sub;
+#pragma unroll
+        for (int k = 0; k < 4; ++k) {
+          if (i0 + k < rlen) lds[mode == WSRC_FWD ? run * g.pr + sub * g.pc + t : run * g.pc + sub * g.pr + t] = q[u][k];
+          if (++t == per_sub) { t = 0; ++sub; }
+        }
+      }
+    }
+  }
+}
+
+template <auto KERN, typename... Args>
+static int wino_transform_launch_lds(const rehr_gather_gemm_desc& d, const rehr_weight_src& s, int mode, int64_t items,
+                                     int outer, hipStream_t stream, Args... args) {
+  if (d.flags & REHR_GG_WS_READY) return REHR_EINVAL;
+  if (items / 64 >= (1ll << 31)) return REHR_ENOSUP;
+  const WsrcLds g = wsrc_lds(s, mode);
+  const int gy = (items / 64 < 1024 && outer <= 65535) ? outer : 1;
+  hipLaunchKernelGGL(KERN, dim3((unsigned)(items / 64), gy), dim3(64), (size_t)g.floats * sizeof(float), stream, d, s,
+                     d.wino_ws, args..., mode);
+  REHR_LAUNCH_CHECK();
+  return REHR_OK;
+}
+
 WinoRoute wino_region_plan(const rehr_gather_gemm_desc& d, WinoPlan& plan);
 bool wino_split_plan(const rehr_gather_gemm_desc* ds, int count, WinoPlan& plan);
-int wino_weights_launch(WinoRoute r, const rehr_gather_gemm_desc& d, const WinoPlan& plan, hipStream_t stream);
+int wino_weights_launch(WinoRoute r, const rehr_gather_gemm_desc& d, const WinoPlan& plan, hipStream_t stream,
+                        const rehr_weight_src* src = nullptr);
 int wino_region_launch(WinoRoute r, const rehr_gather_gemm_desc* ds, int count, const WinoPlan& plan, hipStream_t stream);
 bool wino_flat8_plan(const rehr_gather_gemm_desc& d, WinoPlan& plan);
 int wino_flat8_launch(const rehr_gather_gemm_desc& d, const WinoPlan& plan, hipStream_t stream);
 bool wino22_flat_plan(const rehr_gather_gemm_desc& d, WinoPlan& plan, int parts);
 bool wino22_region_plan(const rehr_gather_gemm_desc& d, WinoPlan& plan);
 bool wino22_flat_multi_plan(const rehr_gather_gemm_desc* ds, int count, WinoPlan& plan);
-int wino22_weights_launch(const rehr_gather_gemm_desc& d, const WinoPlan& plan, hipStream_t stream);
+int wino22_weights_launch(const rehr_gather_gemm_desc& d, const WinoPlan& plan, hipStream_t stream,
+                          const rehr_weight_src* src = nullptr);
 int wino22_launch(WinoRoute r, const rehr_gather_gemm_desc* ds, int count, const WinoPlan& plan, hipStream_t stream);
diff --git a/rehrseg_amd/hip_backend.py b/rehrseg_amd/hip_backend.py
--- a/rehrseg_amd/hip_backend.py
+++ b/rehrseg_amd/hip_backend.py
@@ -241,6 +241,69 @@
         _form_of_panel[id(out)] = f
     _form_ready(f, w)
     return f.out
+
+
+DIRECT_WEIGHT_SOURCE = True
+weight_src_calls = 0
+weight_src_panels = 0
+
+
+class _WeightSrc:
+    __slots__ = ("w", "args", "part", "dtype", "device", "is_cuda")
+
+    def __init__(self, w, args, part):
+        self.w, self.args, self.part = w, args, part
+        self.dtype, self.device, self.is_cuda = torch.float32, w.device, w.is_cuda
+
+    def data_ptr(self):
+        return self.w.data_ptr()
+
+    def panel(self):
+        return pack_weights(self.w, *self.args, part=self.part)
+
+    def src(self):
+        A, _Apad, B, T, transpose = self.args
+        v = self.w if self.part is None else self.w.narrow(*self.part)
+        if v.dim() != 5 or self.w.data_ptr() % 16 or v.data_ptr() % 4:
+            return None
+        rd, cd = (1, 0) if transpose else (0, 1)
+        KD, KH, KW = v.shape[2:]
+        st = v.stride(4)
+        if (v.shape[rd], v.shape[cd], KD * KH * KW) != (A, B, T) or min(v.stride()) < 0:
+            return None
+        if (KH > 1 and v.stride(3) != KW * st) or (KD > 1 and v.stride(2) != KH * KW * st):
+            return None
+        return L.WeightSrc(C.c_void_p(v.data_ptr()), v.stride(rd), v.stride(cd), st, A, B, T, 0)
+
+
+def weight_operand(w, A, Apad, B, T, transpose, dtype=torch.float32, part=None):
+    if dtype != torch.float32 or not (DIRECT_WEIGHT_SOURCE and USE_WINOGRAD) or _keeps_forms(w):
+        return pack_weights(w, A, Apad, B, T, transpose, dtype=dtype, part=part)
+    _chk_dev(w)
+    if w.dtype != torch.float32:
+        raise L.RehrsegHipError("master weights are float32")
+    return _WeightSrc(w, (A, Apad, B, T, transpose), part)
+
+
+def _resolve_weights(descs, n, needs, wp):
+    if not isinstance(wp, _WeightSrc):
+        return None
+    global weight_src_calls, weight_src_panels
+    s = wp.src() if all(needs) else None
+    if s is not None:
+        rc = L.load().rehr_gather_gemm_weight_forms_f32(descs, n, C.byref(s), _stream())
+        if rc == 0:
+            for i in range(n):
+                descs[i].flags |= L.GG_WS_READY
+            weight_src_calls += 1
+            return wp.w
+        if rc != L.ENOSUP:
+            L.check(rc, "rehr_gather_gemm_weight_forms_f32")
+    panel = wp.panel()
+    for i in range(n):
+        descs[i].wp = _ptr(panel)
+    weight_src_panels += 1
+    return panel
 
 
 USE_WINOGRAD = True
@@ -386,6 +449,7 @@
     arr = (L.GatherGemmDesc * 1)(d)
     keep = _attach_ws(arr, 1, [_gg_desc.need], [_gg_desc.sig], args[11])
     with _timed(_gg_family(arr[0]), flops, lambda: _gg_tag(arr[0])):
+        keep = (keep, _resolve_weights(arr, 1, [_gg_desc.need], args[11]))
         L.check(L.load().rehr_gather_gemm_multi_f32(arr, 1, _stream()), "rehr_gather_gemm_f32")
     del keep
 
@@ -406,6 +470,7 @@
     keep = _attach_ws(arr, len(calls), needs, sigs, calls[0][11])
     with _timed(_gg_family(arr[0]) if all(arr[i].wino_ws for i in range(len(calls))) else "gather_gemm", flops,
                 lambda: f"{len(calls)} parts of " + _gg_tag(arr[0])):
+        keep = (keep, _resolve_weights(arr, len(calls), needs, calls[0][11]))
         L.check(L.load().rehr_gather_gemm_multi_f32(arr, len(calls), _stream()), "rehr_gather_gemm_multi_f32")
     del keep
 
diff --git a/rehrseg_amd/lib.py b/rehrseg_amd/lib.py
--- a/rehrseg_amd/lib.py
+++ b/rehrseg_amd/lib.py
@@ -61,6 +61,11 @@
     ]
 
 
+class WeightSrc(C.Structure):
+    _fields_ = [("w", _vp), ("sn", _i64), ("sc", _i64), ("st", _i64), ("rows", _i32), ("cols", _i32),
+                ("taps", _i32), ("reserved", _i32)]
+
+
 class WgradDesc(C.Structure):
     _fields_ = [
         ("l", _vp), ("ldl", _i32), ("Ca", _i32),
@@ -107,6 +112,7 @@
     "rehr_gather_gemm_wino_route": (C.c_int, [_P_GG]),
     "rehr_gather_gemm_f32": (C.c_int, [_P_GG, _vp]),
     "rehr_gather_gemm_multi_f32": (C.c_int, [_P_GG, _i32, _vp]),
+    "rehr_gather_gemm_weight_forms_f32": (C.c_int, [_P_GG, _i32, C.POINTER(WeightSrc), _vp]),
     "rehr_gather_gemm_bf16": (C.c_int, [_P_GG, _vp]),
     "rehr_gather_gemm_multi_bf16": (C.c_int, [_P_GG, _i32, _vp]),
     "rehr_pack_weights_bf16": (C.c_int, [_vp, _vp, _i32, _i32, _i32, _i32, _i32, _vp]),
@@ -215,6 +221,7 @@
     "rehr_last_hip_error": (C.c_char_p, []),
 }
 
+ENOSUP = -2
 _ERR = {-1: "REHR_EINVAL (malformed descriptor)", -2: "REHR_ENOSUP (unsupported shape)",
         -3: "REHR_EHIP (hip launch error)"}
 
diff --git a/rehrseg_amd/ops.py b/rehrseg_amd/ops.py
--- a/rehrseg_amd/ops.py
+++ b/rehrseg_amd/ops.py
@@ -147,11 +147,12 @@
         else:
             w = w.narrow(*part).contiguous()
         shape[part[0]] = part[2]
+    pack = getattr(be, "weight_operand", be.pack_weights)
     if dest_dim == 0:
         A, B = shape[0], shape[1]
-        return be.pack_weights(w, A, pad_rows(A), B, T, False, **kw), pad_rows(A)
+        return pack(w, A, pad_rows(A), B, T, False, **kw), pad_rows(A)
     A, B = shape[1], shape[0]
-    return be.pack_weights(w, A, pad_rows(A), B, T, True, **kw), pad_rows(A)
+    return pack(w, A, pad_rows(A), B, T, True, **kw), pad_rows(A)
 
 
 def _phased_gather(src1, src2, c1, Csrc, wp, Npad, dst, Cdst, K, stride, pad, bias, act, slope, stats, stats_mode):
```
